# LinXueyuanStdio/LaTeX_OCR

Measured on AMD Instinct MI355X. Metric: formula-images/sec training step (batch 64, 128x512), higher is better.
Workload: dtype bf16; 1 GPU; configs[2]: full encoder+attention+decoder training step, batch 64/GPU, 128x512, vocab 500, T=101 (lengths U{30..100}), Adam; global_batch=64, parallelism=dp1

## Files before the change

### include/lxo.h

```cpp
#ifndef LXO_H
#define LXO_H
#include <stddef.h>
#include <stdint.h>
#ifdef __cplusplus
extern "C" {
#endif
#pragma GCC visibility push(default)

#define LXO_F32 0
#define LXO_BF16 1

const char* lxo_last_error(void);
#define LXO_ABI_VERSION 6
int lxo_version(void);
int lxo_shape_size(void);


int lxo_gemm_nt(int dt, int a_f32, int c_f32, int small, const void* A, const void* Bp, void* C,
                int M, int N, int K, int lda, int ldb, int ldc, const float* bias, int act,
                float alpha, int accumulate, void* stream);

int lxo_gemm_tn(int dt, int a_f32, int b_f32, const void* A, const void* B, float* C,
                int M, int I, int J, int lda, int ldb, int ldc, int nsplit, int atomic, void* stream);

// ... 72 lines not shown
                        const int32_t* lengths, float inv_ntok, void* stream);
int lxo_ce_loss_fwd_bwd_dev(const lxo_shape* s, void* ws, const int32_t* formula,
                            const int32_t* lengths, const float* ntok_dev, void* stream);
int lxo_ce_loss_weighted(const lxo_shape* s, void* ws, const int32_t* formula, const int32_t* lengths,
                         const float* w_tok, const float* w_row, float inv_norm, const float* norm_dev, void* stream);
int lxo_ce_loss_smoothed(const lxo_shape* s, void* ws, const int32_t* formula, const int32_t* lengths, float eps,
                         const float* w_tok, const float* w_row, float inv_norm, const float* norm_dev, void* stream);
int lxo_mrt_weights(const float* seq_logp, const float* cost, const int32_t* group_off, int G, int rows, float alpha,
                    float* w_out, float* q_out, float* risk_out, void* stream);
#define LXO_EDIT_MAX_REF 1024
int lxo_edit_distance(const int32_t* hyp, int hyp_block, long long hyp_block_stride, long long hyp_row_stride, long long hyp_tok_stride, int T,
                      const int32_t* hyp_len, const int32_t* ref, int G, int ref_ld, const int32_t* ref_len, const int32_t* ref_of, int per_ref,
                      int pairs, int id_end, int32_t* dist_out, float* cost_out, void* stream);
#define LXO_TEXT_STATS  12
#define LXO_TEXT_CORPUS 14
int lxo_text_stats(const int32_t* hyp, int hyp_block, long long hyp_block_stride, long long hyp_row_stride, long long hyp_tok_stride, int T,
                   const int32_t* hyp_len, const int32_t* ref, int G, int ref_ld, const int32_t* ref_len, const int32_t* ref_of, int per_ref,
                   int pairs, int id_end, int32_t* stats_out, long long* corpus_io, int accumulate, void* stream);
int lxo_mrt_candidates(const int32_t* ids, int B, int max_steps, int n, int steps, const int32_t* ref, int Tr, const int32_t* ref_len,
                       int id_end, int id_pad, int include_reference, int32_t* cand, int32_t* cand_len, float* cost, int32_t* group_off,
                       int32_t* row_image, void* stream);
#define LXO_CONSENSUS_MAX_N 64
int lxo_consensus(const int32_t* ids, long long image_stride, long long draw_stride, long long tok_stride, int B, int n, int T, int id_end,
                  const float* weights, int normalize, int32_t* dist_out, float* risk_out, int32_t* best_out, void* stream);
#define LXO_BLEU_COUNTS 10
int lxo_sentence_bleu(const int32_t* hyp, int hyp_block, long long hyp_block_stride, long long hyp_row_stride, long long hyp_tok_stride, int T,
                      const int32_t* hyp_len, const int32_t* ref, int G, int ref_ld, const int32_t* ref_len, const int32_t* ref_of, int per_ref,
                      int pairs, int id_end, int32_t* counts_out, float* bleu_out, float* cost_out, void* stream);
int lxo_consensus_bleu(const int32_t* ids, long long image_stride, long long draw_stride, long long tok_stride, int B, int n, int T, int id_end,
                       const float* weights, int32_t* match_out, float* cost_out, float* risk_out, int32_t* best_out, void* stream);
#define LXO_COST_EDIT 0
#define LXO_COST_BLEU 1
int lxo_mrt_candidates_cost(const int32_t* ids, int B, int max_steps, int n, int steps, const int32_t* ref, int Tr, const int32_t* ref_len,
                            int id_end, int id_pad, int include_reference, int32_t* cand, int32_t* cand_len, float* cost, int32_t* group_off,
                            int32_t* row_image, int cost_kind, void* stream);
int lxo_score_tokens(const lxo_shape* s, void* ws, const int32_t* formula, const int32_t* lengths,
                     float* logp_out, int32_t* top1_out, float* seq_out, void* stream);
int lxo_score_alternatives(const lxo_shape* s, void* ws, const int32_t* formula, const int32_t* lengths, int k,
                           const uint32_t* allow, int allow_ld, int32_t* ids_out, float* logp_out,
                           int32_t* rank_out, float* entropy_out, void* stream);
int lxo_decoder_train_bwd(const lxo_shape* s, const float* params, const void* wpack, void* ws,
                          const int32_t* formula, float* grads, void* stream);
int lxo_decoder_train_bwd_part(const lxo_shape* s, const float* params, const void* wpack, void* ws,
                               const int32_t* formula, float* grads, int parts, void* stream);

#define LXO_XDEC_BLOCK_BYTES (4096 + (384 << 10))
#define LXO_XDEC_ERR_WORD 512
int lxo_chain_guard(const lxo_shape* s, void* ws, const float* grads, float* scale_io, int have_scale, uint32_t* status_out, void* stream);

#define LXO_GNORM_FLOATS (2 + 1024)
int lxo_global_norm_scale(long long n, const float* grads, float clip, float* scale_out, void* stream);
int lxo_adam_step(long long n, float* params, const float* grads, float* m, float* v,
                  float lr_t, float beta1, float beta2, float eps, const float* scale_dev, void* stream);

int lxo_optimizer_step(int method, long long n, float* params, const float* grads, float* slot, float lr,
                       const float* scale_dev, void* stream);

int lxo_greedy_decode(const lxo_shape* s, const float* params, const void* wpack, void* ws,
                      int id_end, int max_iter, int32_t* ids_out, int* steps_out, void* stream);
int lxo_greedy_decode_attn(const lxo_shape* s, const float* params, const void* wpack, void* ws,
                           int id_end, int max_iter, int32_t* ids_out, float* alpha_out, int* steps_out, void* stream);
int lxo_greedy_decode_scores(const lxo_shape* s, const float* params, const void* wpack, void* ws, int id_end, int max_iter,
                             int32_t* ids_out, float* logp_out, float* alpha_out, int* steps_out, void* stream);
int lxo_greedy_decode_prefix(const lxo_shape* s, const float* params, const void* wpack, void* ws, int id_end, int max_iter,
                             const int32_t* prefix, int prefix_ld, const int32_t* prefix_len,
                             int32_t* ids_out, float* logp_out, float* alpha_out, int* steps_out, void* stream);
int lxo_greedy_decode_constrained(const lxo_shape* s, const float* params, const void* wpack, void* ws, int id_end, int max_iter,
                                  const uint32_t* allow, int allow_ld,
                                  const int32_t* prefix, int prefix_ld, const int32_t* prefix_len,
                                  int32_t* ids_out, float* logp_out, float* alpha_out, int* steps_out, void* stream);
typedef struct lxo_sample_opts { float temperature; int top_k; float top_p; unsigned seed; } lxo_sample_opts;
int lxo_sample_decode(const lxo_shape* s, const float* params, const void* wpack, void* ws, int id_end, int max_iter,
                      const lxo_sample_opts* opts, const uint32_t* allow, int allow_ld,
                      const int32_t* prefix, int prefix_ld, const int32_t* prefix_len,
                      int32_t* ids_out, float* logp_out, float* logq_out, float* alpha_out, int* steps_out, void* stream);
int lxo_sample_tokens(const float* logits, int ld, int rows, int n, int V, int time, const lxo_sample_opts* opts,
                      const uint32_t* allow, int allow_ld, int32_t* ids_out, float* logp_out, float* logq_out, void* stream);
int lxo_decode_begin(const lxo_shape* s, const float* params, const void* wpack, void* ws, void* stream);
int lxo_decode_step(const lxo_shape* s, const float* params, const void* wpack, void* ws, int id_end, int time,
                    int32_t* ids_out, int32_t* parents_out, int32_t* finished_host, int* unfinished_host, void* stream);
int lxo_decode_state_get(const lxo_shape* s, void* ws, int time, float* c, float* h, float* o, void* stream);
int lxo_decode_state_set(const lxo_shape* s, void* ws, int time, const float* c, const float* h, const float* o,
                         const int32_t* ids_prev, void* stream);
int lxo_decode_cell_step(const lxo_shape* s, const float* params, const void* wpack, void* ws, int time, int start_token, void* stream);
int lxo_beam_decode(const lxo_shape* s, const float* params, const void* wpack, void* ws,
                    int id_end, int max_iter, int32_t* ids_out, int32_t* parents_out,
                    int* steps_out, void* stream);
int lxo_beam_decode_attn(const lxo_shape* s, const float* params, const void* wpack, void* ws,
                         int id_end, int max_iter, int32_t* ids_out, int32_t* parents_out, float* alpha_out,
                         int* steps_out, void* stream);
int lxo_beam_decode_scores(const lxo_shape* s, const float* params, const void* wpack, void* ws, int id_end, int max_iter,
                           int32_t* ids_out, int32_t* parents_out, float* scores_out, float* alpha_out, int* steps_out, void* stream);
int lxo_beam_decode_prefix(const lxo_shape* s, const float* params, const void* wpack, void* ws, int id_end, int max_iter,
                           const int32_t* prefix, int prefix_ld, const int32_t* prefix_len,
                           int32_t* ids_out, int32_t* parents_out, float* scores_out, float* alpha_out, int* steps_out, void* stream);
int lxo_beam_decode_constrained(const lxo_shape* s, const float* params, const void* wpack, void* ws, int id_end, int max_iter,
                                const uint32_t* allow, int allow_ld,
                                const int32_t* prefix, int prefix_ld, const int32_t* prefix_len,
                                int32_t* ids_out, int32_t* parents_out, float* scores_out, float* alpha_out, int* steps_out, void* stream);

#define LXO_GRAMMAR_MAX_DEPTH 32
typedef struct lxo_grammar { const int8_t* cls; int n_kinds; int max_depth; int budget; } lxo_grammar;
size_t lxo_grammar_scratch_bytes(int rows, int V);
int lxo_greedy_decode_grammar(const lxo_shape* s, const float* params, const void* wpack, void* ws, int id_end, int max_iter,
                              const uint32_t* allow, int allow_ld, const int32_t* prefix, int prefix_ld, const int32_t* prefix_len,
                              const lxo_grammar* grammar, int32_t* ids_out, float* logp_out, float* alpha_out, int32_t* depth_out,
// ... 28 lines not shown
```

### latex_ocr_amd/_abi.py

```python
import ctypes
import os

c_int, c_ll, c_size, c_float, c_void = ctypes.c_int, ctypes.c_longlong, ctypes.c_size_t, ctypes.c_float, ctypes.c_void_p
P = ctypes.POINTER

LXO_F32, LXO_BF16 = 0, 1
LXO_GNORM_FLOATS = 2 + 1024
LIB_PATH = os.environ.get("LXO_LIB_PATH") or os.path.join(os.path.dirname(os.path.abspath(__file__)), "liblxo.so")


ABI_VERSION = 6
LXO_COMM_ID_BYTES = 128
LXO_I32, LXO_U8 = 2, 3
LXO_XDEC_BLOCK_BYTES, LXO_XDEC_ERR_WORD = 4096 + (384 << 10), 512
LXO_EDIT_MAX_REF = 1024
LXO_CONSENSUS_MAX_N = 64
LXO_TEXT_STATS, LXO_TEXT_CORPUS = 12, 14
LXO_BLEU_COUNTS = 10
LXO_COST_EDIT, LXO_COST_BLEU = 0, 1


class LxoShape(ctypes.Structure):
    _fields_ = [(n, c_int) for n in ("B", "H", "W", "T", "V", "C", "E", "U", "O", "D", "dtype", "beam", "max_steps")] + \
               [("keep_prob", c_float), ("dropout_seed", c_int), ("div_gamma", c_float), ("div_prob", c_float), ("div_seed", c_int),
# ... 11 lines not shown
LXO_GRAMMAR_MAX_DEPTH = 32


def bind(lib):
    S = P(LxoShape)
    sig = {
        "lxo_last_error": (ctypes.c_char_p, []),
        "lxo_version": (c_int, []),
        "lxo_shape_size": (c_int, []),
        "lxo_ws_region_dtype": (c_int, [S, ctypes.c_char_p]),
        "lxo_gemm_nt": (c_int, [c_int] * 4 + [c_void] * 3 + [c_int] * 6 + [c_void, c_int, c_float, c_int, c_void]),
        "lxo_gemm_tn": (c_int, [c_int] * 3 + [c_void] * 3 + [c_int] * 8 + [c_void]),
        "lxo_conv3x3": (c_int, [c_int, c_void, c_void, c_void, c_void] + [c_int] * 9 + [c_void]),
        "lxo_conv3x3_ex": (c_int, [c_int, c_void, c_void, c_void, c_void] + [c_int] * 9 + [c_void, c_int, c_void, c_void, c_void, c_void]),
        "lxo_conv3x3_wgrad": (c_int, [c_int, c_void, c_void, c_void] + [c_int] * 8 + [c_void]),
        "lxo_gemm_slab": (c_int, [c_int, c_void, c_void, c_void] + [c_int] * 6 + [c_ll, c_void]),
        "lxo_attention_fwd": (c_int, [c_int] + [c_void] * 7 + [c_int] * 6 + [c_void]),
        "lxo_timing_enable": (c_int, [c_int]),
        "lxo_timing_count": (c_int, []),
        "lxo_timing_get": (c_int, [c_int, P(ctypes.c_char_p), P(ctypes.c_char_p), P(ctypes.c_double), P(c_float)]),
        "lxo_param_num": (c_int, []),
        "lxo_param_name": (ctypes.c_char_p, [c_int]),
        "lxo_param_name_for": (ctypes.c_char_p, [S, c_int]),
        "lxo_param_total": (c_ll, [S]),
        "lxo_param_info": (c_int, [S, c_int, P(c_ll), P(c_ll)]),
        "lxo_wpack_bytes": (c_size, [S]),
        "lxo_workspace_bytes": (c_size, [S]),
        "lxo_ws_region": (c_int, [S, ctypes.c_char_p, P(c_size), P(c_size)]),
        "lxo_pack_weights": (c_int, [S, c_void, c_void, c_void]),
        "lxo_encoder_fwd": (c_int, [S, c_void, c_void, c_void, c_void, c_void]),
        "lxo_encoder_bwd": (c_int, [S, c_void, c_void, c_void, c_void, c_void, c_int, c_int, c_void]),
        "lxo_encoder_bwd_ready": (c_int, [S, c_void, c_void, c_void, c_void, c_void, c_int, c_int, c_void, c_void]),
        "lxo_train_bwd": (c_int, [S, c_void, c_void, c_void, c_void, c_void, c_void, c_void, c_void]),
        "lxo_set_encoder_side_stream": (c_int, [c_void]),
        "lxo_set_side_stream": (c_int, [c_void]),
        "lxo_decoder_train_fwd": (c_int, [S, c_void, c_void, c_void, c_void, c_void]),
        "lxo_decoder_train_fwd_live": (c_int, [S, c_void, c_void, c_void, c_void, c_void, c_void]),
        "lxo_ce_loss_fwd_bwd": (c_int, [S, c_void, c_void, c_void, c_float, c_void]),
        "lxo_ce_loss_fwd_bwd_dev": (c_int, [S, c_void, c_void, c_void, c_void, c_void]),
        "lxo_ce_loss_weighted": (c_int, [S, c_void, c_void, c_void, c_void, c_void, c_float, c_void, c_void]),
        "lxo_ce_loss_smoothed": (c_int, [S, c_void, c_void, c_void, c_float, c_void, c_void, c_float, c_void, c_void]),
        "lxo_mrt_weights": (c_int, [c_void, c_void, c_void, c_int, c_int, c_float, c_void, c_void, c_void, c_void]),
        "lxo_edit_distance": (c_int, [c_void, c_int, c_ll, c_ll, c_ll, c_int, c_void, c_void, c_int, c_int, c_void, c_void, c_int, c_int, c_int, c_void, c_void, c_void]),
        "lxo_text_stats": (c_int, [c_void, c_int, c_ll, c_ll, c_ll, c_int, c_void, c_void, c_int, c_int, c_void, c_void, c_int, c_int, c_int, c_void, c_void, c_int, c_void]),
        "lxo_mrt_candidates": (c_int, [c_void, c_int, c_int, c_int, c_int, c_void, c_int, c_void, c_int, c_int, c_int, c_void, c_void, c_void, c_void, c_void, c_void]),
        "lxo_sentence_bleu": (c_int, [c_void, c_int, c_ll, c_ll, c_ll, c_int, c_void, c_void, c_int, c_int, c_void, c_void, c_int, c_int, c_int, c_void, c_void, c_void, c_void]),
        "lxo_mrt_candidates_cost": (c_int, [c_void, c_int, c_int, c_int, c_int, c_void, c_int, c_void, c_int, c_int, c_int, c_void, c_void, c_void, c_void, c_void, c_int, c_void]),
        "lxo_consensus_bleu": (c_int, [c_void, c_ll, c_ll, c_ll, c_int, c_int, c_int, c_int, c_void, c_void, c_void, c_void, c_void, c_void]),
        "lxo_consensus": (c_int, [c_void, c_ll, c_ll, c_ll, c_int, c_int, c_int, c_int, c_void, c_int, c_void, c_void, c_void, c_void]),
        "lxo_decoder_train_bwd_part": (c_int, [S, c_void, c_void, c_void, c_void, c_void, c_int, c_void]),
        "lxo_decoder_train_bwd": (c_int, [S, c_void, c_void, c_void, c_void, c_void, c_void]),
        "lxo_global_norm_scale": (c_int, [c_ll, c_void, c_float, c_void, c_void]),
        "lxo_adam_step": (c_int, [c_ll, c_void, c_void, c_void, c_void, c_float, c_float, c_float, c_float, c_void, c_void]),
        "lxo_optimizer_step": (c_int, [c_int, c_ll, c_void, c_void, c_void, c_float, c_void, c_void]),
        "lxo_greedy_decode": (c_int, [S, c_void, c_void, c_void, c_int, c_int, c_void, P(c_int), c_void]),
        "lxo_greedy_decode_attn": (c_int, [S, c_void, c_void, c_void, c_int, c_int, c_void, c_void, P(c_int), c_void]),
        "lxo_decode_begin": (c_int, [S, c_void, c_void, c_void, c_void]),
        "lxo_decode_step": (c_int, [S, c_void, c_void, c_void, c_int, c_int, c_void, c_void, c_void, P(c_int), c_void]),
        "lxo_beam_decode": (c_int, [S, c_void, c_void, c_void, c_int, c_int, c_void, c_void, P(c_int), c_void]),
        "lxo_beam_decode_attn": (c_int, [S, c_void, c_void, c_void, c_int, c_int, c_void, c_void, c_void, P(c_int), c_void]),
        "lxo_greedy_decode_scores": (c_int, [S, c_void, c_void, c_void, c_int, c_int, c_void, c_void, c_void, P(c_int), c_void]),
        "lxo_beam_decode_scores": (c_int, [S, c_void, c_void, c_void, c_int, c_int, c_void, c_void, c_void, c_void, P(c_int), c_void]),
        "lxo_score_tokens": (c_int, [S, c_void, c_void, c_void, c_void, c_void, c_void, c_void]),
        "lxo_score_alternatives": (c_int, [S, c_void, c_void, c_void, c_int, c_void, c_int, c_void, c_void, c_void, c_void, c_void]),
        "lxo_greedy_decode_prefix": (c_int, [S, c_void, c_void, c_void, c_int, c_int, c_void, c_int, c_void, c_void, c_void, c_void, P(c_int), c_void]),
        "lxo_beam_decode_prefix": (c_int, [S, c_void, c_void, c_void, c_int, c_int, c_void, c_int, c_void, c_void, c_void, c_void, c_void, P(c_int), c_void]),
        "lxo_greedy_decode_constrained": (c_int, [S, c_void, c_void, c_void, c_int, c_int, c_void, c_int, c_void, c_int, c_void, c_void, c_void, c_void, P(c_int), c_void]),
        "lxo_beam_decode_constrained": (c_int, [S, c_void, c_void, c_void, c_int, c_int, c_void, c_int, c_void, c_int, c_void, c_void, c_void, c_void, c_void, P(c_int), c_void]),
        "lxo_sample_decode": (c_int, [S, c_void, c_void, c_void, c_int, c_int, P(LxoSampleOpts), c_void, c_int, c_void, c_int, c_void, c_void, c_void, c_void, c_void, P(c_int), c_void]),
        "lxo_sample_tokens": (c_int, [c_void, c_int, c_int, c_int, c_int, c_int, P(LxoSampleOpts), c_void, c_int, c_void, c_void, c_void, c_void]),
        "lxo_grammar_scratch_bytes": (c_size, [c_int, c_int]),
        "lxo_greedy_decode_grammar": (c_int, [S, c_void, c_void, c_void, c_int, c_int, c_void, c_int, c_void, c_int, c_void, P(LxoGrammar), c_void, c_void, c_void, c_void, c_void, P(c_int), c_void]),
        "lxo_beam_decode_grammar": (c_int, [S, c_void, c_void, c_void, c_int, c_int, c_void, c_int, c_void, c_int, c_void, P(LxoGrammar), c_void, c_void, c_void, c_void, c_void, c_void, P(c_int), c_void]),
        "lxo_sample_decode_grammar": (c_int, [S, c_void, c_void, c_void, c_int, c_int, P(LxoSampleOpts), c_void, c_int, c_void, c_int, c_void, P(LxoGrammar), c_void, c_void, c_void, c_void, c_void, c_void, P(c_int), c_void]),
        "lxo_grammar_step": (c_int, [P(LxoGrammar), c_int, c_int, c_int, c_int, c_void, c_void, c_void, c_int, c_int, c_void, c_int, c_void, c_void, c_void, c_void]),
        "lxo_chain_guard": (c_int, [S, c_void, c_void, c_void, c_int, c_void, c_void]),
        "lxo_decode_state_get": (c_int, [S, c_void, c_int, c_void, c_void, c_void, c_void]),
        "lxo_decode_state_set": (c_int, [S, c_void, c_int, c_void, c_void, c_void, c_void, c_void]),
        "lxo_decode_cell_step": (c_int, [S, c_void, c_void, c_void, c_int, c_int, c_void]),
        "lxo_comm_unique_id": (c_int, [c_void]),
        "lxo_comm_init": (c_int, [c_void, c_int, c_int, P(c_void)]),
        "lxo_comm_info": (c_int, [c_void, P(c_int), P(c_int)]),
        "lxo_allreduce_bucket": (c_int, [c_void, c_void, c_ll, c_int, c_void, c_void]),
        "lxo_comm_destroy": (c_int, [c_void]),
        "lxo_comm_last_error": (ctypes.c_char_p, []),
    }
    missing = []
    for name, (res, args) in sig.items():
        try:
            fn = getattr(lib, name)
        except AttributeError:
            missing.append(name)
            continue
        fn.restype, fn.argtypes = res, args
    lib._lxo_missing = missing
    if not missing:
        if lib.lxo_version() != ABI_VERSION or lib.lxo_shape_size() != ctypes.sizeof(LxoShape):
            raise RuntimeError("liblxo ABI mismatch: library version %d / lxo_shape %d bytes, binding version %d / %d bytes"
                               % (lib.lxo_version(), lib.lxo_shape_size(), ABI_VERSION, ctypes.sizeof(LxoShape)))
    return lib


ENTRY_POINTS = ["lxo_last_error", "lxo_version", "lxo_shape_size", "lxo_ws_region_dtype", "lxo_timing_enable", "lxo_timing_count", "lxo_timing_get", "lxo_gemm_nt", "lxo_gemm_tn", "lxo_conv3x3", "lxo_conv3x3_ex", "lxo_conv3x3_wgrad", "lxo_gemm_slab", "lxo_attention_fwd", "lxo_param_num", "lxo_param_name", "lxo_param_name_for",
                "lxo_param_total", "lxo_param_info", "lxo_wpack_bytes", "lxo_workspace_bytes", "lxo_ws_region",
                "lxo_pack_weights", "lxo_encoder_fwd", "lxo_encoder_bwd", "lxo_encoder_bwd_ready", "lxo_train_bwd", "lxo_set_side_stream", "lxo_set_encoder_side_stream", "lxo_decoder_train_fwd", "lxo_decoder_train_fwd_live",
                "lxo_ce_loss_fwd_bwd", "lxo_ce_loss_fwd_bwd_dev", "lxo_ce_loss_weighted", "lxo_ce_loss_smoothed", "lxo_mrt_weights", "lxo_edit_distance", "lxo_text_stats", "lxo_mrt_candidates", "lxo_consensus", "lxo_sentence_bleu", "lxo_consensus_bleu", "lxo_mrt_candidates_cost", "lxo_decoder_train_bwd", "lxo_decoder_train_bwd_part", "lxo_global_norm_scale", "lxo_adam_step", "lxo_optimizer_step",
                "lxo_greedy_decode", "lxo_greedy_decode_attn", "lxo_beam_decode", "lxo_beam_decode_attn", "lxo_greedy_decode_scores", "lxo_beam_decode_scores", "lxo_score_tokens", "lxo_score_alternatives", "lxo_greedy_decode_prefix", "lxo_beam_decode_prefix", "lxo_greedy_decode_constrained", "lxo_beam_decode_constrained", "lxo_sample_decode", "lxo_sample_tokens",
                "lxo_grammar_scratch_bytes", "lxo_greedy_decode_grammar", "lxo_beam_decode_grammar", "lxo_sample_decode_grammar", "lxo_grammar_step", "lxo_decode_begin", "lxo_decode_step",
                "lxo_chain_guard", "lxo_decode_state_get", "lxo_decode_state_set", "lxo_decode_cell_step",
                "lxo_comm_unique_id", "lxo_comm_init", "lxo_comm_info", "lxo_allreduce_bucket", "lxo_comm_destroy", "lxo_comm_last_error"]

_lib = None


def load():
    global _lib
    if _lib is None:
        if not os.path.exists(LIB_PATH):
            raise RuntimeError(
                "latex_ocr_amd: %s is missing. Build it with `python -c 'import __graft_entry__ as g; g.build()'` "
                "(hipcc --offload-arch=gfx950). There is no CPU fallback." % LIB_PATH)
        try:
            import torch
        except ImportError:
            pass
        _lib = bind(ctypes.CDLL(LIB_PATH))
        if _lib._lxo_missing:
            raise RuntimeError("liblxo.so lacks entry points: %s" % _lib._lxo_missing)
    return _lib


def check(lib, rc, what=""):
    if rc != 0:
        raise RuntimeError("%s failed: rc=%d %s" % (what, rc, lib.lxo_last_error().decode()))
```

### latex_ocr_amd/csrc/api.hip

```cpp
#include "lxo.h"
#include "gemm.h"
#include "impl.h"
#include <stdio.h>
#include <string.h>

static thread_local char g_err[256] = "";
static int fail(int code, const char* what) {
    snprintf(g_err, sizeof(g_err), "%s (code %d)", what, code);
    return code < 0 ? code : -code;
}
#define CHECK_LAUNCH(expr, what) do { int rc_ = (expr); if (rc_ != 0) return fail(rc_, what); } while (0)

extern "C" const char* lxo_last_error(void) { return g_err; }
extern "C" int lxo_version(void) { return LXO_ABI_VERSION; }
extern "C" int lxo_shape_size(void) { return (int)sizeof(lxo_shape); }

extern "C" int lxo_gemm_nt(int dt, int a_f32, int c_f32, int small, const void* A, const void* Bp, void* C,
                           int M, int N, int K, int lda, int ldb, int ldc, const float* bias, int act,
                           float alpha, int accumulate, void* stream) {
    GemmNT p; memset(&p, 0, sizeof(p));
    p.A = A; p.Bp = Bp; p.C = C; p.M = M; p.N = N; p.K = K; p.lda = lda; p.ldb = ldb; p.ldc = ldc;
    p.bias = bias; p.act = act; p.alpha = alpha; p.accumulate = accumulate; p.addend_rows = 1;
    CHECK_LAUNCH(lxo_launch_gemm_nt(dt, a_f32, c_f32, small, p, (hipStream_t)stream), "lxo_gemm_nt");
    return 0;
// ... 223 lines not shown
extern "C" int lxo_score_tokens(const lxo_shape* s, void* ws, const int32_t* formula, const int32_t* lengths,
                                float* logp_out, int32_t* top1_out, float* seq_out, void* stream) {
    MAKE_PLAN(P, s);
    if (s->T <= 0) return fail(-1, "T must be positive");
    if (!ws || !formula || !lengths) return fail(-1, "lxo_score_tokens: null workspace, formula or lengths");
    if (!logp_out) return fail(-1, "lxo_score_tokens: null logp_out");
    CHECK_LAUNCH(lxo_impl_score_tokens(P, ws, formula, lengths, logp_out, top1_out, seq_out, (hipStream_t)stream), "lxo_score_tokens");
    return 0;
}
extern "C" int lxo_score_alternatives(const lxo_shape* s, void* ws, const int32_t* formula, const int32_t* lengths, int k,
                                      const uint32_t* allow, int allow_ld, int32_t* ids_out, float* logp_out,
                                      int32_t* rank_out, float* entropy_out, void* stream) {
    MAKE_PLAN(P, s);
    if (s->T <= 0) return fail(-1, "T must be positive");
    if (!ws || !formula || !lengths) return fail(-1, "lxo_score_alternatives: null workspace, formula or lengths");
    if (!ids_out) return fail(-1, "lxo_score_alternatives: null ids_out");
    if (!logp_out) return fail(-1, "lxo_score_alternatives: null logp_out");
    if (k < 1 || k > 16 || k > P.s.V) return fail(-1, "lxo_score_alternatives: k outside 1 .. min(16, V)");
    if (allow && (allow_ld < 0 || (allow_ld != 0 && allow_ld < (P.s.V + 31) / 32))) return fail(-1, "lxo_score_alternatives: allow_ld must be 0 or >= (V + 31) / 32");
    if (!allow && allow_ld != 0) return fail(-1, "lxo_score_alternatives: null allow with allow_ld != 0");
    const DecAllow al = {allow, allow_ld};
    CHECK_LAUNCH(lxo_impl_score_alternatives(P, ws, formula, lengths, k, allow ? &al : nullptr, ids_out, logp_out, rank_out, entropy_out, (hipStream_t)stream),
                 "lxo_score_alternatives");
    return 0;
}
extern "C" int lxo_decoder_train_bwd(const lxo_shape* s, const float* params, const void* wpack, void* ws,
                                     const int32_t* formula, float* grads, void* stream) {
    MAKE_PLAN(P, s);
    CHECK_LAUNCH(lxo_impl_decoder_train_bwd(P, params, wpack, ws, formula, grads, 3, (hipStream_t)stream), "lxo_decoder_train_bwd");
    return 0;
}
extern "C" int lxo_train_bwd(const lxo_shape* s, const float* params, const void* wpack, void* ws, const int32_t* formula, const uint8_t* img,
                            float* grads, void* const* ready_events, void* stream) {
    MAKE_PLAN(P, s);
    CHECK_LAUNCH(lxo_impl_decoder_train_bwd(P, params, wpack, ws, formula, grads, 3, (hipStream_t)stream, true, ready_events ? ready_events[0] : nullptr),
                 "lxo_train_bwd (decoder)");
    CHECK_LAUNCH(lxo_impl_encoder_bwd(P, params, wpack, ws, img, grads, 6, 1, (hipStream_t)stream, ready_events), "lxo_train_bwd (encoder)");
    return 0;
}
extern "C" int lxo_decoder_train_bwd_part(const lxo_shape* s, const float* params, const void* wpack, void* ws,
                                          const int32_t* formula, float* grads, int parts, void* stream) {
    MAKE_PLAN(P, s);
    if (parts < 1 || parts > 3) return fail(-1, "lxo_decoder_train_bwd_part: parts must be 1, 2 or 3");
    CHECK_LAUNCH(lxo_impl_decoder_train_bwd(P, params, wpack, ws, formula, grads, parts, (hipStream_t)stream), "lxo_decoder_train_bwd_part");
    return 0;
}
extern "C" int lxo_global_norm_scale(long long n, const float* grads, float clip, float* scale_out, void* stream) {
    CHECK_LAUNCH(lxo_k_global_norm_scale(n, grads, clip, scale_out + 2, scale_out, (hipStream_t)stream), "lxo_global_norm_scale");
    return 0;
}
extern "C" int lxo_adam_step(long long n, float* params, const float* grads, float* m, float* v,
                             float lr_t, float beta1, float beta2, float eps, const float* scale_dev, void* stream) {
    CHECK_LAUNCH(lxo_k_adam(params, grads, m, v, n, lr_t, beta1, beta2, eps, scale_dev, (hipStream_t)stream), "lxo_adam_step");
    return 0;
}
extern "C" int lxo_greedy_decode(const lxo_shape* s, const float* params, const void* wpack, void* ws,
                                 int id_end, int max_iter, int32_t* ids_out, int* steps_out, void* stream) {
    MAKE_PLAN(P, s);
    const DecodeOuts o = {ids_out, nullptr, nullptr, nullptr, nullptr};
    CHECK_LAUNCH(lxo_impl_greedy_decode(P, params, wpack, ws, id_end, max_iter, o, steps_out, (hipStream_t)stream), "lxo_greedy_decode");
    return 0;
}
extern "C" int lxo_greedy_decode_attn(const lxo_shape* s, const float* params, const void* wpack, void* ws,
                                      int id_end, int max_iter, int32_t* ids_out, float* alpha_out, int* steps_out, void* stream) {
    MAKE_PLAN(P, s);
    const DecodeOuts o = {ids_out, nullptr, nullptr, alpha_out, nullptr};
    CHECK_LAUNCH(lxo_impl_greedy_decode(P, params, wpack, ws, id_end, max_iter, o, steps_out, (hipStream_t)stream), "lxo_greedy_decode_attn");
    return 0;
}
extern "C" int lxo_greedy_decode_scores(const lxo_shape* s, const float* params, const void* wpack, void* ws, int id_end, int max_iter,
                                        int32_t* ids_out, float* logp_out, float* alpha_out, int* steps_out, void* stream) {
    MAKE_PLAN(P, s);
    if (!logp_out) return fail(-1, "lxo_greedy_decode_scores: null logp_out");
    const DecodeOuts o = {ids_out, nullptr, logp_out, alpha_out, nullptr};
    CHECK_LAUNCH(lxo_impl_greedy_decode(P, params, wpack, ws, id_end, max_iter, o, steps_out, (hipStream_t)stream), "lxo_greedy_decode_scores");
    return 0;
}
static bool make_prefix(DecPrefix* pf, const int32_t* prefix, int prefix_ld, const int32_t* prefix_len, int max_iter) {
    *pf = DecPrefix{prefix, prefix_len, prefix_ld, prefix_ld < max_iter ? prefix_ld : max_iter};
    return prefix && prefix_len && prefix_ld >= 1;
}
extern "C" int lxo_greedy_decode_prefix(const lxo_shape* s, const float* params, const void* wpack, void* ws, int id_end, int max_iter,
                                        const int32_t* prefix, int prefix_ld, const int32_t* prefix_len,
                                        int32_t* ids_out, float* logp_out, float* alpha_out, int* steps_out, void* stream) {
    MAKE_PLAN(P, s);
    DecPrefix pf;
    if (!make_prefix(&pf, prefix, prefix_ld, prefix_len, max_iter)) return fail(-1, "lxo_greedy_decode_prefix: null prefix / prefix_len or prefix_ld < 1");
    const DecodeOuts o = {ids_out, nullptr, logp_out, alpha_out, &pf};
    CHECK_LAUNCH(lxo_impl_greedy_decode(P, params, wpack, ws, id_end, max_iter, o, steps_out, (hipStream_t)stream), "lxo_greedy_decode_prefix");
    return 0;
}
static const char* make_constraint(DecAllow* al, DecPrefix* pf, bool* has_prefix, int V, const uint32_t* allow, int allow_ld,
                                   const int32_t* prefix, int prefix_ld, const int32_t* prefix_len, int max_iter) {
    *al = DecAllow{allow, allow_ld};
    if (!allow || allow_ld < 0 || (allow_ld != 0 && allow_ld < (V + 31) / 32)) return "lxo_*_decode_constrained: null allow or 0 < allow_ld < (V + 31) / 32";
    *has_prefix = prefix || prefix_len || prefix_ld != 0;
    if (*has_prefix && !make_prefix(pf, prefix, prefix_ld, prefix_len, max_iter)) return "lxo_*_decode_constrained: a prefix needs prefix, prefix_len and prefix_ld >= 1 (none: all NULL / 0)";
    return nullptr;
}
extern "C" int lxo_greedy_decode_constrained(const lxo_shape* s, const float* params, const void* wpack, void* ws, int id_end, int max_iter,
                                             const uint32_t* allow, int allow_ld, const int32_t* prefix, int prefix_ld, const int32_t* prefix_len,
                                             int32_t* ids_out, float* logp_out, float* alpha_out, int* steps_out, void* stream) {
    MAKE_PLAN(P, s);
    DecAllow al; DecPrefix pf; bool has_prefix = false;
    if (const char* why = make_constraint(&al, &pf, &has_prefix, P.s.V, allow, allow_ld, prefix, prefix_ld, prefix_len, max_iter))
        return fail(-1, why);
// ... 275 lines not shown
```

### latex_ocr_amd/csrc/decoder_kernels.h

```cpp
#pragma once
#include "lxo_common.h"
struct Slabs { const float* p; int n; long long stride; int ld; };
struct Drop { unsigned thr; float inv_keep; unsigned seed; int t, row0, rows_total; };
struct DetScratch { float* p; size_t floats; };
int lxo_k_det_reduce(const float* part, int nslot, long long stride, int N, float* out, hipStream_t st);
int lxo_k_rowmean(int dt, const void* img, float* mean, int B, int R, int C, hipStream_t st);
int lxo_k_embed_gather(int dt, const float* table, const float* start, const int* formula, void* out, int B, int T, int D, int Dp, int V, hipStream_t st);
int lxo_k_embed_rows(int dt, const float* table, const float* start, const int* ids, void* out, int n, int D, int Dp, int V, hipStream_t st);
int lxo_k_embed_table(int dt, const float* table, const float* start, void* out, int V, int D, int Dp, hipStream_t st);
int lxo_k_lstm_fwd(const float* z, Slabs zs, const float* c_prev, float* gates, float* c_out, float* h_out, float* ht_out, int ldh, Drop dr, int B, int U, hipStream_t st);
int lxo_k_lstm_bwd(const float* gates, const float* c_prev, const float* c_cur, Slabs s1, Slabs s3, Slabs s4, int off4,
                   float* dcc, float* dz, Drop dr, int carry_rows, int B, int U, hipStream_t st);
int lxo_k_tanh_bwd(const float* a, int lda, Slabs carry, const float* o, int ldo, float* g, int ldg, void* gb, int ldgb, Drop dr, int carry_rows, int rows, int cols, hipStream_t st);
int lxo_k_slab_reduce(Slabs sl, float* o, int ldo, int rows, int cols, hipStream_t st);
int lxo_k_tanh_finalize(Slabs sl, float* o, int ldo, Drop dr, int rows, int cols, hipStream_t st);
int lxo_k_attn_fwd(int dt, const void* att_img, const void* img, const float* att_h, Slabs ahs, float* att_h_out, const float* beta, float* alpha, float* part,
                   float* ctx, int ldctx, void* ctxb, int ldcb, int nv, int R, int Rp, int E, int C, int beam, int nch, int rev, hipStream_t st, const void* att_exp = nullptr);
int lxo_k_att_exp(const void* att_img, void* att_exp, long long n, hipStream_t st);
int lxo_k_attn_bwd(int dt, const void* att_img, const void* att_exp, const void* img, const float* att_h, const float* beta, const float* alpha,
                   Slabs dcs, int dcoff, float* dctx_out, int lddc, const float* ctx, int ldctx, float* de, float* datth,
                   int nv, int R, int Rp, int E, int C, int nch, int rev, hipStream_t st);
int lxo_k_datt_img(int dt, const void* att_img, const float* att_h, const float* beta, const float* de, void* dout, float* dbeta,
                   int T, int B, int R, int Rp, int E, float* atth_exp, DetScratch det, hipStream_t st);
int lxo_k_add_mean_grad(float* dimg, const float* dmean, int B, int R, int C, hipStream_t st);
int lxo_k_colsum_det(const void* a, int bf16, long long lda, float* out, long long M, int N, DetScratch det, hipStream_t st);
int lxo_k_colsum(const float* a, long long lda, float* out, long long M, int N, DetScratch det, hipStream_t st);
int lxo_k_embed_scatter(const float* demb, const int* formula, float* dtable, float* dstart, int B, int T, int D, int V, int det, hipStream_t st);
int lxo_k_init_bwd(const float* dcc, Slabs dxh, const float* c0, const float* rec0, int ldr, float* dpre, int B, int U, int O, hipStream_t st);
int lxo_k_beam_gather(float* rec, int ldr, int XH, float* cs, int U, const int* parents, int k, float* tmp_rec, float* tmp_cs, int n, void* recb, int ldrb, hipStream_t st);
int lxo_k_tile_rows(const float* src, int lds, float* dst, int ldd, int n, int k, int cols, hipStream_t st);
int lxo_k_global_norm_scale(long long n, const float* g, float clip, float* sumsq_tmp, float* out, hipStream_t st);
int lxo_k_chain_guard(const unsigned* err_fwd, const unsigned* err_bwd, const float* probe, float* scale, int have_scale, unsigned* status, hipStream_t st);
int lxo_k_chain_poison(const unsigned* err_fwd, const unsigned* err_bwd, float* probe, hipStream_t st);
int lxo_k_adam(float* p, const float* g, float* m, float* v, long long n, float lr_t, float b1, float b2, float eps, const float* scale, hipStream_t st);
int lxo_k_simple_opt(float* p, const float* g, float* slot, long long n, float lr, int mode, const float* scale, hipStream_t st);
```

### latex_ocr_amd/csrc/decoder_kernels.hip

```cpp
#include "decoder_kernels.h"
#include "api_util.h"
#include "drop.h"

namespace {


LXO_DEV void load4(const float* p, float (&v)[4]) {
    f32x4 a = *reinterpret_cast<const f32x4*>(p);
    v[0] = a[0]; v[1] = a[1]; v[2] = a[2]; v[3] = a[3];
}
LXO_DEV void load4(const bf16_t* p, float (&v)[4]) {
    u32x2 a = *reinterpret_cast<const u32x2*>(p);
    v[0] = __uint_as_float(a[0] << 16); v[1] = __uint_as_float(a[0] & 0xffff0000u);
    v[2] = __uint_as_float(a[1] << 16); v[3] = __uint_as_float(a[1] & 0xffff0000u);
}
LXO_DEV void store4(float* p, const float (&v)[4]) { f32x4 a = {v[0], v[1], v[2], v[3]}; *reinterpret_cast<f32x4*>(p) = a; }
LXO_DEV void store4(bf16_t* p, const float (&v)[4]) { u32x2 a = {pack_bf2(v[0], v[1]), pack_bf2(v[2], v[3])}; *reinterpret_cast<u32x2*>(p) = a; }

LXO_DEV float slab_sum(const Slabs& sl, long long row, int col) {
    float v = 0.f;
    const float* q = sl.p + row * sl.ld + col;
    for (int s = 0; s < sl.n; ++s) v += q[(long long)s * sl.stride];
    return v;
}

LXO_DEV f32x4 slab_sum4(const Slabs& sl, long long row, int col) {
    f32x4 v = {0.f, 0.f, 0.f, 0.f};
    const float* q = sl.p + row * sl.ld + col;
    for (int s0 = 0; s0 < sl.n; s0 += 8) {
        f32x4 t[8];
#pragma unroll
        for (int j = 0; j < 8; ++j) {
            const f32x4 z = {0.f, 0.f, 0.f, 0.f};
            t[j] = (s0 + j < sl.n) ? *reinterpret_cast<const f32x4*>(q + (long long)(s0 + j) * sl.stride) : z;
        }
#pragma unroll
        for (int j = 0; j < 8; ++j) v += t[j];
    }
    return v;
}

template <typename CT>
__global__ __launch_bounds__(256) void rowmean_kernel(const CT* __restrict__ img, float* __restrict__ mean, int R, int C) {
    __shared__ float red[32][64 + 1];
    const int b = blockIdx.y, c0 = blockIdx.x * 64 + (threadIdx.x & 7) * 8, rg = threadIdx.x >> 3;
    float acc[8];
#pragma unroll
    for (int e = 0; e < 8; ++e) acc[e] = 0.f;
    for (int r = rg; r < R; r += 32) {
        float v[8];
        load8(img + ((long long)b * R + r) * C + c0, v);
#pragma unroll
        for (int e = 0; e < 8; ++e) acc[e] += v[e];
    }
#pragma unroll
// ... 104 lines not shown
    for (int s0 = q; s0 < sl.n; s0 += 32) {
        f32x4 t[8];
#pragma unroll
        for (int j = 0; j < 8; ++j) {
            const f32x4 z = {0.f, 0.f, 0.f, 0.f};
            t[j] = (s0 + 4 * j < sl.n) ? *reinterpret_cast<const f32x4*>(p + (long long)(s0 + 4 * j) * sl.stride) : z;
        }
#pragma unroll
        for (int j = 0; j < 8; ++j) v += t[j];
    }
    return v;
}

__global__ __launch_bounds__(256) void lstm_bwd_kernel(const float* __restrict__ gates, const float* __restrict__ c_prev,
                                                      const float* __restrict__ c_cur, Slabs s1, Slabs s3, Slabs s4, int off4,
                                                      float* __restrict__ dcc, float* __restrict__ dz, Drop dr, int carry_rows,
                                                      int B, int U) {
    __shared__ float ex[64][4][8 + 1];
    const int total = B * (U >> 2);
    const int q = threadIdx.x & 3, ugl = threadIdx.x >> 2;
    for (int base = blockIdx.x * 64; base < total; base += gridDim.x * 64) {
        const int ug = base + ugl;
        const bool ok = ug < total;
        const int b = ok ? ug / (U >> 2) : 0, u = ok ? (ug - b * (U >> 2)) << 2 : 0;
        float gi = 0.f, gj = 0.f, gf = 0.f, go = 0.f, cc = 0.f, cp = 0.f, dci = 0.f;
        if (ok) {
            const float* gr = gates + (long long)b * 4 * U + u + q;
            gi = gr[0]; gj = gr[U]; gf = gr[2 * U]; go = gr[3 * U];
            cc = c_cur[(long long)b * U + u + q]; cp = c_prev[(long long)b * U + u + q]; dci = dcc[(long long)b * U + u + q];
            const f32x4 pm = slab_part4(s1, b, u, q) + slab_part4(s3, b, u, q);
            f32x4 pc = {0.f, 0.f, 0.f, 0.f};
            if (b < carry_rows) pc = slab_part4(s4, b, off4 + u, q);
#pragma unroll
            for (int e = 0; e < 4; ++e) { ex[ugl][q][e] = pm[e]; ex[ugl][q][4 + e] = pc[e]; }
        }
        __syncthreads();
        if (ok) {
            const float dhm = ex[ugl][0][q] + ex[ugl][1][q] + ex[ugl][2][q] + ex[ugl][3][q];
            const float dhc = ex[ugl][0][4 + q] + ex[ugl][1][4 + q] + ex[ugl][2][4 + q] + ex[ugl][3][4 + q];
            const float dh = dhm * drop_scale(dr, 1u, b, u + q, U) + dhc;
            const float tc = tanhf(cc);
            const float dc = dci + dh * go * (1.f - tc * tc);
            float* dzr = dz + (long long)b * 4 * U + u + q;
            dzr[0] = dc * gj * gi * (1.f - gi);
            dzr[U] = dc * gi * (1.f - gj * gj);
            dzr[2 * U] = dc * cp * gf * (1.f - gf);
            dzr[3 * U] = dh * tc * go * (1.f - go);
            dcc[(long long)b * U + u + q] = dc * gf;
        }
        __syncthreads();
    }
}

__global__ __launch_bounds__(256) void tanh_bwd_kernel(const float* __restrict__ a, int lda, Slabs carry,
                                                      const float* __restrict__ o, int ldo, float* __restrict__ g, int ldg,
                                                      bf16_t* __restrict__ gb, int ldgb, Drop dr, int carry_rows, int rows, int cols) {
    const int total = rows * (cols >> 2);
    for (int i = blockIdx.x * 256 + threadIdx.x; i < total; i += gridDim.x * 256) {
        const int r = i / (cols >> 2), c = (i - r * (cols >> 2)) << 2;
        const f32x4 ov = *reinterpret_cast<const f32x4*>(o + (long long)r * ldo + c);
        f32x4 d = *reinterpret_cast<const f32x4*>(a + (long long)r * lda + c);
        if (r < carry_rows) d += slab_sum4(carry, r, c);
        f32x4 out;
#pragma unroll
        for (int e = 0; e < 4; ++e) {
            const float sc = drop_scale(dr, 2u, r, c + e, cols);
            const float th = (dr.thr == 0u) ? ov[e] : ov[e] / dr.inv_keep;
            out[e] = d[e] * sc * (1.f - th * th);
        }
        *reinterpret_cast<f32x4*>(g + (long long)r * ldg + c) = out;
        if (gb) { u32x2 pk = {pack_bf2(out[0], out[1]), pack_bf2(out[2], out[3])}; *reinterpret_cast<u32x2*>(gb + (long long)r * ldgb + c) = pk; }
    }
}
__global__ __launch_bounds__(256) void tanh_finalize_kernel(Slabs sl, float* __restrict__ o, int ldo, Drop dr, int rows, int cols) {
    const int total = rows * (cols >> 2);
    for (int i = blockIdx.x * 256 + threadIdx.x; i < total; i += gridDim.x * 256) {
        const int r = i / (cols >> 2), c = (i - r * (cols >> 2)) << 2;
        const f32x4 v = slab_sum4(sl, r, c);
        f32x4 out;
#pragma unroll
        for (int e = 0; e < 4; ++e) out[e] = tanhf(v[e]) * drop_scale(dr, 2u, r, c + e, cols);
        *reinterpret_cast<f32x4*>(o + (long long)r * ldo + c) = out;
    }
}

constexpr int ATT_W = 8;

template <typename CT> LXO_DEV float tanh_ct(float x);
template <> LXO_DEV float tanh_ct<float>(float x) { return tanhf(x); }
template <> LXO_DEV float tanh_ct<bf16_t>(float x) { return 1.f - 2.f * __builtin_amdgcn_rcpf(__expf(2.f * x) + 1.f); }

template <typename CT, int KCT, int ATT_U>
__global__ __launch_bounds__(512) void attn_fwd_part_kernel(const CT* __restrict__ att_img, const CT* __restrict__ img,
                                                           const float* __restrict__ att_h, Slabs ahs, float* __restrict__ att_h_out,
                                                           const float* __restrict__ beta,
                                                           float* __restrict__ alpha, float* __restrict__ part,
                                                           int R, int Rp, int E, int C, int beam, int nch, int rows_per, int rev) {
    __shared__ float redc[ATT_W][512];
    __shared__ float red[2 * ATT_W];
    const int ch = blockIdx.x, v = blockIdx.y, bi = v / beam;
    const int tid = threadIdx.x, lane = tid & 63, wave = tid >> 6;
    const int r0 = ch * rows_per;
    const int n = min(R, r0 + rows_per) - r0;
    const CT* ai = att_img + ((long long)bi * R + r0) * E;
    const CT* im = img + ((long long)bi * R + r0) * C;
    float* pout = part + ((long long)v * nch + ch) * (C + 2);
    constexpr int KC = KCT;
    float ah[KCT][4], bt[KCT][4];
#pragma unroll
    for (int kc = 0; kc < KCT; ++kc) {
        const int k0 = kc * 256 + lane * 4;
#pragma unroll
        for (int j = 0; j < 4; ++j) { ah[kc][j] = 0.f; bt[kc][j] = 0.f; }
        if (kc < KC && k0 < E) {
            const f32x4 a4 = ahs.n > 0 ? slab_sum4(ahs, v, k0) : *reinterpret_cast<const f32x4*>(att_h + (long long)v * E + k0);
            const f32x4 b4 = *reinterpret_cast<const f32x4*>(beta + k0);
#pragma unroll
            for (int j = 0; j < 4; ++j) { ah[kc][j] = a4[j]; bt[kc][j] = b4[j]; }
            if (ahs.n > 0 && att_h_out && ch == 0 && wave == 0) *reinterpret_cast<f32x4*>(att_h_out + (long long)v * E + k0) = a4;
        }
    }
    const int c0 = lane * 8;
    const bool cok = c0 < C;
    float m = -3.0e38f, l = 0.f, acc[8];
// ... 909 lines not shown
            const int src = b * k + parents[b * k + r];
            v[r] = c < XH ? rec[(long long)src * ldr + c] : cs[(long long)src * U + (c - XH)];
        }
    }
#pragma unroll
    for (int r = 0; r < BP_KMAX; ++r) {
        if (r < k) {
            const int dst = b * k + r;
            if (c < XH) { rec[(long long)dst * ldr + c] = v[r]; if (recb) recb[(long long)dst * ldrb + c] = f2bf(v[r]); }
            else cs[(long long)dst * U + (c - XH)] = v[r];
        }
    }
}
__global__ __launch_bounds__(256) void tile_rows_kernel(const float* __restrict__ src, int lds, float* __restrict__ dst, int ldd, int n, int k, int cols) {
    const long long total = (long long)n * cols;
    for (long long i = (long long)blockIdx.x * 256 + threadIdx.x; i < total; i += (long long)gridDim.x * 256) {
        const int v = (int)(i / cols), c = (int)(i - (long long)v * cols);
        dst[(long long)v * ldd + c] = src[(long long)(v / k) * lds + c];
    }
}

__global__ __launch_bounds__(256) void sumsq_kernel(const float* __restrict__ g, long long n, float* __restrict__ out) {
    __shared__ float red[4];
    float s = 0.f;
    for (long long i = (long long)blockIdx.x * 256 + threadIdx.x; i < n; i += (long long)gridDim.x * 256) s = fmaf(g[i], g[i], s);
    s = wave_sum(s);
    if ((threadIdx.x & 63) == 0) red[threadIdx.x >> 6] = s;
    __syncthreads();
    if (threadIdx.x == 0) out[blockIdx.x] = red[0] + red[1] + red[2] + red[3];
}
__global__ void clip_scale_kernel(const float* __restrict__ sumsq, int nparts, float clip, float* __restrict__ out) {
    float ss = 0.f;
    for (int i = 0; i < nparts; ++i) ss += sumsq[i];
    const float gn = sqrtf(ss);
    out[1] = gn;
    out[0] = clip > 0.f ? clip / fmaxf(gn, clip) : 1.0f;
}
__global__ void chain_guard_kernel(const unsigned* __restrict__ err_fwd, const unsigned* __restrict__ err_bwd, const float* __restrict__ probe,
                                   float* __restrict__ scale, int have_scale, unsigned* __restrict__ status) {
    const unsigned ef = err_fwd ? err_fwd[0] : 0u, eb = err_bwd ? err_bwd[0] : 0u;
    const float pv = probe ? probe[0] : 0.f;
    const bool drop = (ef | eb) != 0u || pv != pv;
    if (status) { status[0] = ef; status[1] = eb; status[2] = drop ? 1u : 0u; }
    scale[0] = drop ? __uint_as_float(0x7fc00000u) : (have_scale ? scale[0] : 1.0f);
}
__global__ void chain_poison_kernel(const unsigned* __restrict__ err_fwd, const unsigned* __restrict__ err_bwd, float* __restrict__ probe) {
    if ((err_fwd && err_fwd[0]) || (err_bwd && err_bwd[0])) probe[0] = __uint_as_float(0x7fc00000u);
}
__global__ __launch_bounds__(256) void adam_kernel(float* __restrict__ p, const float* __restrict__ g, float* __restrict__ m, float* __restrict__ v,
                                                  long long n, float lr_t, float b1, float b2, float eps, const float* __restrict__ scale) {
    const float sc = scale ? scale[0] : 1.0f;
    if (sc != sc) return;
    for (long long i = (long long)blockIdx.x * 256 + threadIdx.x; i < n; i += (long long)gridDim.x * 256) {
        const float gi = g[i] * sc;
        const float mi = b1 * m[i] + (1.f - b1) * gi;
        const float vi = b2 * v[i] + (1.f - b2) * gi * gi;
        m[i] = mi; v[i] = vi;
        p[i] -= lr_t * mi / (sqrtf(vi) + eps);
    }
}

__global__ __launch_bounds__(256) void simple_opt_kernel(float* __restrict__ p, const float* __restrict__ g, float* __restrict__ slot,
                                                        long long n, float lr, int mode, const float* __restrict__ scale) {
    const float sc = scale ? scale[0] : 1.0f;
    if (sc != sc) return;
    for (long long i = (long long)blockIdx.x * 256 + threadIdx.x; i < n; i += (long long)gridDim.x * 256) {
        const float gi = g[i] * sc;
        if (mode == 1) p[i] -= lr * gi;
        else if (mode == 2) { const float a = slot[i] + gi * gi; slot[i] = a; p[i] -= lr * gi / sqrtf(a); }
        else { const float ms = 0.9f * slot[i] + 0.1f * gi * gi; slot[i] = ms; p[i] -= lr * gi / sqrtf(ms + 1e-10f); }
    }
}

inline int grid1(long long items, int per_block = 256, int cap = 2048) {
    long long g = (items + per_block - 1) / per_block;
    return (int)(g < 1 ? 1 : (g > cap ? cap : g));
}
}

#define LAUNCH(kern, grid, ...) hipLaunchKernelGGL(kern, dim3(grid), dim3(256), 0, st, __VA_ARGS__)
#define BYCT(dt, kern, grid, ...) do { if ((dt) == LXO_BF16) LAUNCH((kern<bf16_t>), grid, __VA_ARGS__); else LAUNCH((kern<float>), grid, __VA_ARGS__); } while (0)
#define DONE return (int)hipGetLastError()

int lxo_k_rowmean(int dt, const void* img, float* mean, int B, int R, int C, hipStream_t st) {
    if (C % 64) return -2;
    if (dt == LXO_BF16) LAUNCH((rowmean_kernel<bf16_t>), dim3(C / 64, B), (const bf16_t*)img, mean, R, C);
    else LAUNCH((rowmean_kernel<float>), dim3(C / 64, B), (const float*)img, mean, R, C);
    DONE;
}
int lxo_k_embed_gather(int dt, const float* table, const float* start, const int* formula, void* out, int B, int T, int D, int Dp, int V, hipStream_t st) {
    const int g = grid1((long long)T * B * Dp);
    if (dt == LXO_BF16) LAUNCH((embed_gather_kernel<bf16_t>), g, table, start, formula, (bf16_t*)out, B, T, D, Dp, V);
    else LAUNCH((embed_gather_kernel<float>), g, table, start, formula, (float*)out, B, T, D, Dp, V);
    DONE;
}
int lxo_k_embed_rows(int dt, const float* table, const float* start, const int* ids, void* out, int n, int D, int Dp, int V, hipStream_t st) {
    const int g = grid1((long long)n * Dp);
    if (dt == LXO_BF16) LAUNCH((embed_rows_kernel<bf16_t>), g, table, start, ids, (bf16_t*)out, n, D, Dp, V);
    else LAUNCH((embed_rows_kernel<float>), g, table, start, ids, (float*)out, n, D, Dp, V);
    DONE;
}
int lxo_k_embed_table(int dt, const float* table, const float* start, void* out, int V, int D, int Dp, hipStream_t st) {
    const int g = grid1((long long)(V + 1) * Dp);
    if (dt == LXO_BF16) LAUNCH((embed_table_kernel<bf16_t>), g, table, start, (bf16_t*)out, V, D, Dp);
    else LAUNCH((embed_table_kernel<float>), g, table, start, (float*)out, V, D, Dp);
    DONE;
}
int lxo_k_lstm_fwd(const float* z, Slabs zs, const float* c_prev, float* gates, float* c_out, float* h_out, float* ht_out, int ldh, Drop dr, int B, int U, hipStream_t st) {
    LAUNCH(lstm_fwd_kernel, grid1((long long)B * U), z, zs, c_prev, gates, c_out, h_out, ht_out, ldh, dr, B, U);
    DONE;
}
int lxo_k_lstm_bwd(const float* gates, const float* c_prev, const float* c_cur, Slabs s1, Slabs s3, Slabs s4, int off4,
                   float* dcc, float* dz, Drop dr, int carry_rows, int B, int U, hipStream_t st) {
    LAUNCH(lstm_bwd_kernel, grid1((long long)B * U), gates, c_prev, c_cur, s1, s3, s4, off4, dcc, dz, dr, carry_rows, B, U);
    DONE;
}
int lxo_k_tanh_bwd(const float* a, int lda, Slabs carry, const float* o, int ldo, float* g, int ldg, void* gb, int ldgb, Drop dr, int carry_rows, int rows, int cols, hipStream_t st) {
    LAUNCH(tanh_bwd_kernel, grid1((long long)rows * cols / 4), a, lda, carry, o, ldo, g, ldg, (bf16_t*)gb, ldgb, dr, carry_rows, rows, cols);
    DONE;
}
__global__ __launch_bounds__(256) static void slab_reduce_kernel(Slabs sl, float* __restrict__ o, int ldo, int rows, int cols) {
    const int total = rows * (cols >> 2);
    for (int i = blockIdx.x * 256 + threadIdx.x; i < total; i += gridDim.x * 256) {
        const int r = i / (cols >> 2), c = (i - r * (cols >> 2)) << 2;
        *reinterpret_cast<f32x4*>(o + (long long)r * ldo + c) = slab_sum4(sl, r, c);
    }
}
int lxo_k_slab_reduce(Slabs sl, float* o, int ldo, int rows, int cols, hipStream_t st) {
    LAUNCH(slab_reduce_kernel, grid1((long long)rows * cols / 4), sl, o, ldo, rows, cols);
    DONE;
}
int lxo_k_tanh_finalize(Slabs sl, float* o, int ldo, Drop dr, int rows, int cols, hipStream_t st) {
    LAUNCH(tanh_finalize_kernel, grid1((long long)rows * cols / 4), sl, o, ldo, dr, rows, cols);
    DONE;
}
static int att_u(int rows_per) {
    return (rows_per + 55) / 56 <= (rows_per + 63) / 64 ? 7 : 8;
}
#define ATT_BY_U(K_, CT_, KCT_) do { if (att_u(rows_per) == 8) K_(CT_, KCT_, 8); else K_(CT_, KCT_, 7); } while (0)
#define ATT_BY_CT_E(K_) do { if (dt == LXO_BF16) { if (E <= 256) ATT_BY_U(K_, bf16_t, 1); else ATT_BY_U(K_, bf16_t, 4); } \
                             else { if (E <= 256) ATT_BY_U(K_, float, 1); else ATT_BY_U(K_, float, 4); } } while (0)
int lxo_k_attn_fwd(int dt, const void* att_img, const void* img, const float* att_h, Slabs ahs, float* att_h_out, const float* beta, float* alpha, float* part,
                   float* ctx, int ldctx, void* ctxb, int ldcb, int nv, int R, int Rp, int E, int C, int beam, int nch, int rev, hipStream_t st, const void* att_exp) {
    if (E > 1024 || C > 512 || nch < 1 || nch > 32) return -2;
    const int rows_per = cdiv(R, nch);
    dim3 grid(nch, nv);
    if ((beam == 2 || beam == 3 || beam == 5 || (beam == 1 && att_exp && dt == LXO_BF16)) && ahs.n == 0 && att_h && E <= 256 && C <= 512 && nv % beam == 0) {
        const int nimg = nv / beam;
        int nb = cdiv(512, nimg);
        if (nb > 16) nb = 16;
        const int by_rows = R / 32 > 0 ? R / 32 : 1;
        if (nb > by_rows) nb = by_rows;
        const int need = cdiv(R, 1024);
        if (nb < need) nb = need;
        const int rpb = cdiv(R, nb);
        const dim3 gb(nb, nimg);
#define ABM(CT_, U_, NB_, X_, OCC_, AI_) hipLaunchKernelGGL((attn_fwd_part_beam_kernel<CT_, U_, NB_, X_, OCC_>), gb, dim3(512), 0, st, (const CT_*)(AI_), (const CT_*)img, att_h, beta, alpha, part, R, Rp, E, C, nb, rpb, rev)
        if (dt == LXO_BF16 && att_exp) { if (beam == 1) ABM(bf16_t, 4, 1, true, 4, att_exp); else if (beam == 2) ABM(bf16_t, 4, 2, true, 4, att_exp); else if (beam == 3) ABM(bf16_t, 4, 3, true, 4, att_exp); else ABM(bf16_t, 2, 5, true, 4, att_exp); }
        else if (dt == LXO_BF16) { if (beam == 2) ABM(bf16_t, 4, 2, false, 2, att_img); else if (beam == 3) ABM(bf16_t, 4, 3, false, 2, att_img); else ABM(bf16_t, 4, 5, false, 2, att_img); }
        else { if (beam == 2) ABM(float, 4, 2, false, 2, att_img); else if (beam == 3) ABM(float, 4, 3, false, 2, att_img); else ABM(float, 4, 5, false, 2, att_img); }
#undef ABM
        hipLaunchKernelGGL(attn_fwd_combine_kernel, dim3(4, nv), dim3(256), 0, st, part, alpha, ctx, ldctx, (bf16_t*)ctxb, ldcb, R, Rp, C, nb, rpb);
        DONE;
    }
#define AF(CT_, KCT_, U_) hipLaunchKernelGGL((attn_fwd_part_kernel<CT_, KCT_, U_>), grid, dim3(512), 0, st, (const CT_*)att_img, (const CT_*)img, \
                                             att_h, ahs, att_h_out, beta, alpha, part, R, Rp, E, C, beam, nch, rows_per, rev)
    ATT_BY_CT_E(AF);
// ... 127 lines not shown
```

### latex_ocr_amd/csrc/encoder_kernels.h

```cpp
#pragma once
#include "lxo_common.h"
#include "decoder_kernels.h"
struct PackJob { int kind, K, N, lds, ldd, coff, Kpad, first_block, nblocks; long long src; long long dst; };
struct PackTable { int n; PackJob job[64]; };
int lxo_k_conv1_pool_fwd(int dt, const uint8_t* img, const float* w, const float* b, void* out, int B, int H, int W, hipStream_t s);
int lxo_k_conv1_pool_bwd(int dt, const uint8_t* img, const float* w, const float* b, const void* dout, float* dw, float* db, int B, int H, int W, DetScratch det, hipStream_t s);
int lxo_k_maxpool_fwd(int dt, const void* in, void* out, int B, int H, int W, int C, int ph, int pw, hipStream_t s);
int lxo_k_maxpool_mask_bwd(const unsigned char* mask, const void* dp, void* dy, float* db, int B, int H, int W, int C, int ph, int pw, DetScratch det, hipStream_t s);
int lxo_k_maxpool_relu_bwd(int dt, const void* y, const void* dp, void* dy, float* db, int B, int H, int W, int C, int ph, int pw, hipStream_t s);
int lxo_k_mask_convert(int dt, const float* d, const void* ref, void* out, float* db, long long rows, int C, hipStream_t s);
int lxo_k_timing_signal(float* pos, int Hp, int Wp, int C, hipStream_t s);
int lxo_k_pack_transpose(int dt, const float* src, void* dst, int K, int N, int lds, int ldd, int coff, int Kpad, hipStream_t s);
int lxo_k_pack_copy(int dt, const float* src, void* dst, int R, int Ccols, int lds, int ldd, int Cpad, hipStream_t s);
int lxo_k_pack_conv_dgrad(int dt, const float* w, void* dst, int Cin, int Cout, hipStream_t s);
int lxo_k_pack_batch(int dt, const PackTable& tab, int total_blocks, const float* prm, void* wpk, hipStream_t s);
int lxo_k_im2col_s2(int dt, const void* in, void* cols, int B, int H, int W, int Ho, int Wo, int C, hipStream_t s);
int lxo_k_col2im_s2_relu(int dt, const void* dcols, const void* yref, void* dy, float* db, int B, int H, int W, int Ho, int Wo, int C, hipStream_t s);
int lxo_k_colsum_ct(int dt, const void* a, float* out, long long M, int N, hipStream_t s);
```

### latex_ocr_amd/csrc/encoder_kernels.hip

```cpp
#include "encoder_kernels.h"
#include "switches.h"

namespace {

template <typename CT>
__global__ __launch_bounds__(256) void conv1_pool_fwd_kernel(const uint8_t* __restrict__ img, const float* __restrict__ w,
                                                            const float* __restrict__ bias, CT* __restrict__ out,
                                                            int B, int H, int W, int Hp, int Wp) {
    const int cg = threadIdx.x & 7;
    float wr[9][8], br[8];
#pragma unroll
    for (int t = 0; t < 9; ++t)
#pragma unroll
        for (int e = 0; e < 8; ++e) wr[t][e] = w[t * 64 + cg * 8 + e];
#pragma unroll
    for (int e = 0; e < 8; ++e) br[e] = bias[cg * 8 + e];
    __shared__ float sp[4][68];
    const int pl = threadIdx.x >> 3;
    const int segs_x = (Wp + 31) >> 5, nseg = B * Hp * segs_x;
    for (int seg = blockIdx.x; seg < nseg; seg += gridDim.x) {
        const int row = seg / segs_x, xc = seg - row * segs_x;
        const int b = row / Hp, py = row - b * Hp;
        const int px = xc * 32 + pl;
        const uint8_t* im = img + (long long)b * H * W;
        __syncthreads();
        for (int i = threadIdx.x; i < 4 * 66; i += 256) {
            const int dy = i / 66, dx = i - dy * 66;
            const int y = 2 * py - 1 + dy, x = 64 * xc - 1 + dx;
            sp[dy][dx] = (y >= 0 && y < H && x >= 0 && x < W) ? fmaf((float)im[y * W + x], 0.0078125f, -1.0f) : 0.f;
        }
        __syncthreads();
        if (px >= Wp) continue;
        const int pix = row * Wp + px;
        float patch[4][4];
#pragma unroll
        for (int dy = 0; dy < 4; ++dy) {
            const f32x2 lo = *reinterpret_cast<const f32x2*>(&sp[dy][2 * pl]), hi = *reinterpret_cast<const f32x2*>(&sp[dy][2 * pl + 2]);
            patch[dy][0] = lo[0]; patch[dy][1] = lo[1]; patch[dy][2] = hi[0]; patch[dy][3] = hi[1];
        }
        float best[8];
#pragma unroll
        for (int e = 0; e < 8; ++e) best[e] = -3.0e38f;
#pragma unroll
        for (int qy = 0; qy < 2; ++qy)
#pragma unroll
            for (int qx = 0; qx < 2; ++qx) {
                if (2 * py + qy >= H || 2 * px + qx >= W) continue;
#pragma unroll
                for (int e = 0; e < 8; e += 2) {
                    f32x2 a = {br[e], br[e + 1]};
#pragma unroll
                    for (int kh = 0; kh < 3; ++kh)
#pragma unroll
                        for (int kw = 0; kw < 3; ++kw) {
// ... 565 lines not shown
template <typename CT>
__global__ __launch_bounds__(256) void pack_conv_dgrad_kernel(const float* __restrict__ w, CT* __restrict__ dst, int Cin, int Cout) {
    const long long total = (long long)Cin * 9 * Cout;
    for (long long i = (long long)blockIdx.x * 256 + threadIdx.x; i < total; i += (long long)gridDim.x * 256) {
        const int co = (int)(i % Cout);
        const int tap = (int)((i / Cout) % 9);
        const int ci = (int)(i / ((long long)Cout * 9));
        const int a = tap / 3, b = tap - 3 * a;
        dst[i] = from_f32<CT>(w[((long long)((2 - a) * 3 + (2 - b)) * Cin + ci) * Cout + co]);
    }
}

template <typename CT>
__global__ __launch_bounds__(256) void pack_batch_kernel(PackTable tab, const float* __restrict__ prm, char* __restrict__ wpk) {
    __shared__ float tile[32][33];
    int j = 0;
    while (j + 1 < tab.n && (int)blockIdx.x >= tab.job[j + 1].first_block) ++j;
    const PackJob q = tab.job[j];
    const int lb = blockIdx.x - q.first_block;
    const float* src = prm + q.src;
    CT* dst = reinterpret_cast<CT*>(wpk + q.dst);
    if (q.kind == 0) {
        const int tiles_k = (q.Kpad + 31) / 32;
        const int k0 = (lb % tiles_k) * 32, n0 = (lb / tiles_k) * 32;
        const int tx = threadIdx.x & 31, ty = threadIdx.x >> 5;
        for (int r = ty; r < 32; r += 8) {
            const int k = k0 + r, n = n0 + tx;
            tile[r][tx] = (k < q.K && n < q.N) ? src[(long long)k * q.lds + n] : 0.f;
        }
        __syncthreads();
        for (int r = ty; r < 32; r += 8) {
            const int n = n0 + r, k = k0 + tx;
            if (n < q.N && k < q.Kpad) dst[(long long)n * q.ldd + q.coff + k] = from_f32<CT>(tile[tx][r]);
        }
    } else if (q.kind == 1) {
        const long long total = (long long)q.K * q.Kpad;
        for (long long i = (long long)lb * 256 + threadIdx.x; i < total; i += (long long)q.nblocks * 256) {
            const int c = (int)(i % q.Kpad); const long long r = i / q.Kpad;
            dst[r * q.ldd + c] = from_f32<CT>(c < q.N ? src[r * q.lds + c] : 0.f);
        }
    } else {
        const int Cin = q.K, Cout = q.N;
        const long long total = (long long)Cin * 9 * Cout;
        for (long long i = (long long)lb * 256 + threadIdx.x; i < total; i += (long long)q.nblocks * 256) {
            const int co = (int)(i % Cout);
            const int tap = (int)((i / Cout) % 9);
            const int ci = (int)(i / ((long long)Cout * 9));
            const int a = tap / 3, b = tap - 3 * a;
            dst[i] = from_f32<CT>(src[((long long)((2 - a) * 3 + (2 - b)) * Cin + ci) * Cout + co]);
        }
    }
}


template <typename CT>
__global__ __launch_bounds__(256) void im2col_s2_kernel(const CT* __restrict__ in, CT* __restrict__ cols, int B, int H, int W, int Ho, int Wo, int C) {
    const int c8n = C >> 3;
    const long long total = (long long)B * Ho * Wo * 8 * c8n;
    for (long long i = (long long)blockIdx.x * 256 + threadIdx.x; i < total; i += (long long)gridDim.x * 256) {
        const int c8 = (int)(i % c8n);
        const int tap = (int)((i / c8n) & 7);
        const long long m = i / (8 * c8n);
        const int ox = (int)(m % Wo), oy = (int)((m / Wo) % Ho), b = (int)(m / ((long long)Wo * Ho));
        const int iy = 2 * oy + (tap >> 2), ix = 2 * ox + (tap & 3) - 1;
        float v[8] = {0.f, 0.f, 0.f, 0.f, 0.f, 0.f, 0.f, 0.f};
        if (iy < H && ix >= 0 && ix < W) load8(in + (((long long)b * H + iy) * W + ix) * C + c8 * 8, v);
        store8(cols + (m * 8 + tap) * C + c8 * 8, v);
    }
}
template <typename CT>
__global__ __launch_bounds__(256) void col2im_s2_relu_kernel(const CT* __restrict__ dcols, const CT* __restrict__ yref, CT* __restrict__ dy,
                                                            float* __restrict__ db, int B, int H, int W, int Ho, int Wo, int C, int ppt) {
    const int c8n = C >> 3;
    const long long npix = (long long)B * H * W;
    const long long t = (long long)blockIdx.x * 256 + threadIdx.x;
    const int c8 = (int)(t % c8n);
    const long long p0 = (t / c8n) * ppt;
    if (p0 >= npix) return;
    float cs[8] = {0.f, 0.f, 0.f, 0.f, 0.f, 0.f, 0.f, 0.f};
    const long long p1 = p0 + ppt < npix ? p0 + ppt : npix;
    for (long long p = p0; p < p1; ++p) {
        const int x = (int)(p % W), y = (int)((p / W) % H), b = (int)(p / ((long long)W * H));
        const int oy = y >> 1, kh = y & 1;
        float acc[8] = {0.f, 0.f, 0.f, 0.f, 0.f, 0.f, 0.f, 0.f};
        if (oy < Ho) {
#pragma unroll
            for (int h = 0; h < 2; ++h) {
                const int kw = ((x + 1) & 1) + 2 * h;
                const int ox2 = x + 1 - kw;
                if (ox2 < 0 || (ox2 >> 1) >= Wo) continue;
                float v[8];
                load8(dcols + ((((long long)b * Ho + oy) * Wo + (ox2 >> 1)) * 8 + kh * 4 + kw) * C + c8 * 8, v);
#pragma unroll
                for (int e = 0; e < 8; ++e) acc[e] += v[e];
            }
        }
        float r[8];
        load8(yref + p * C + c8 * 8, r);
#pragma unroll
        for (int e = 0; e < 8; ++e) { acc[e] = r[e] > 0.f ? acc[e] : 0.f; cs[e] += acc[e]; }
        store8(dy + p * C + c8 * 8, acc);
    }
    if (!db) return;
#pragma unroll
    for (int e = 0; e < 8; ++e) atomicAdd(&db[c8 * 8 + e], cs[e]);
}
// ... 98 lines not shown
    else if (ph == 1 && pw == 2) hipLaunchKernelGGL((maxpool_mask_bwd_kernel<1, 2>), grid, dim3(256), 0, s, MB_ARGS);
    else return -2;
#undef MB_ARGS
    if (db_part) return lxo_k_det_reduce(db_part, (int)grid.x, C, C, db, s);
    return (int)hipGetLastError();
}
int lxo_k_maxpool_relu_bwd(int dt, const void* y, const void* dp, void* dy, float* db, int B, int H, int W, int C, int ph, int pw, hipStream_t s) {
    if (C % 8 || C > 512 || 256 % (C / 8)) return -2;
    DISPATCH_CT(dt, pool_bwd_t, y, dp, dy, db, B, H, W, C, ph, pw, s);
    return (int)hipGetLastError();
}
template <typename CT> static void mask_convert_t(const float* d, const void* ref, void* out, float* db, long long rows, int C, hipStream_t s) {
    const int rpb = 256 / (C / 8);
    hipLaunchKernelGGL((mask_convert_kernel<CT>), dim3(grid_for(rows, rpb * 8, 2048)), dim3(256), 0, s,
                       d, (const CT*)ref, (CT*)out, db, rows, C);
}
int lxo_k_mask_convert(int dt, const float* d, const void* ref, void* out, float* db, long long rows, int C, hipStream_t s) {
    if (C % 8 || C > 512 || 256 % (C / 8)) return -2;
    DISPATCH_CT(dt, mask_convert_t, d, ref, out, db, rows, C, s);
    return (int)hipGetLastError();
}
int lxo_k_timing_signal(float* pos, int Hp, int Wp, int C, hipStream_t s) {
    hipLaunchKernelGGL(timing_signal_kernel, dim3(grid_for((long long)Hp * Wp * C, 256, 1024)), dim3(256), 0, s, pos, Hp, Wp, C);
    return (int)hipGetLastError();
}
template <typename CT> static void pack_tr_t(const float* src, void* dst, int K, int N, int lds, int ldd, int coff, int Kpad, hipStream_t s) {
    hipLaunchKernelGGL((pack_transpose_kernel<CT>), dim3(cdiv(Kpad, 32), cdiv(N, 32)), dim3(256), 0, s, src, (CT*)dst, K, N, lds, ldd, coff, Kpad);
}
int lxo_k_pack_transpose(int dt, const float* src, void* dst, int K, int N, int lds, int ldd, int coff, int Kpad, hipStream_t s) {
    DISPATCH_CT(dt, pack_tr_t, src, dst, K, N, lds, ldd, coff, Kpad, s);
    return (int)hipGetLastError();
}
template <typename CT> static void pack_cp_t(const float* src, void* dst, int R, int Ccols, int lds, int ldd, int Cpad, hipStream_t s) {
    hipLaunchKernelGGL((pack_copy_kernel<CT>), dim3(grid_for((long long)R * Cpad, 256, 2048)), dim3(256), 0, s, src, (CT*)dst, R, Ccols, lds, ldd, Cpad);
}
int lxo_k_pack_copy(int dt, const float* src, void* dst, int R, int Ccols, int lds, int ldd, int Cpad, hipStream_t s) {
    DISPATCH_CT(dt, pack_cp_t, src, dst, R, Ccols, lds, ldd, Cpad, s);
    return (int)hipGetLastError();
}
template <typename CT> static void pack_dg_t(const float* w, void* dst, int Cin, int Cout, hipStream_t s) {
    hipLaunchKernelGGL((pack_conv_dgrad_kernel<CT>), dim3(grid_for((long long)Cin * 9 * Cout, 256, 2048)), dim3(256), 0, s, w, (CT*)dst, Cin, Cout);
}
int lxo_k_pack_conv_dgrad(int dt, const float* w, void* dst, int Cin, int Cout, hipStream_t s) {
    DISPATCH_CT(dt, pack_dg_t, w, dst, Cin, Cout, s);
    return (int)hipGetLastError();
}

int lxo_k_pack_batch(int dt, const PackTable& tab, int total_blocks, const float* prm, void* wpk, hipStream_t s) {
    if (tab.n <= 0) return 0;
    if (dt == LXO_BF16) hipLaunchKernelGGL((pack_batch_kernel<bf16_t>), dim3(total_blocks), dim3(256), 0, s, tab, prm, (char*)wpk);
    else hipLaunchKernelGGL((pack_batch_kernel<float>), dim3(total_blocks), dim3(256), 0, s, tab, prm, (char*)wpk);
    return (int)hipGetLastError();
}

template <typename CT> static void im2col_s2_t(const void* in, void* cols, int B, int H, int W, int Ho, int Wo, int C, hipStream_t s) {
    hipLaunchKernelGGL((im2col_s2_kernel<CT>), dim3(grid_for((long long)B * Ho * Wo * C, 256 * 4, 8192)), dim3(256), 0, s,
                       (const CT*)in, (CT*)cols, B, H, W, Ho, Wo, C);
}
int lxo_k_im2col_s2(int dt, const void* in, void* cols, int B, int H, int W, int Ho, int Wo, int C, hipStream_t s) {
    if (C % 8) return -2;
    DISPATCH_CT(dt, im2col_s2_t, in, cols, B, H, W, Ho, Wo, C, s);
    return (int)hipGetLastError();
}
template <typename CT> static void col2im_s2_t(const void* dcols, const void* yref, void* dy, float* db, int B, int H, int W, int Ho, int Wo, int C, hipStream_t s) {
    const int ppt = 32;
    const long long threads = (((long long)B * H * W + ppt - 1) / ppt) * (C / 8);
    hipLaunchKernelGGL((col2im_s2_relu_kernel<CT>), dim3((unsigned)((threads + 255) / 256)), dim3(256), 0, s,
                       (const CT*)dcols, (const CT*)yref, (CT*)dy, db, B, H, W, Ho, Wo, C, ppt);
}
int lxo_k_col2im_s2_relu(int dt, const void* dcols, const void* yref, void* dy, float* db, int B, int H, int W, int Ho, int Wo, int C, hipStream_t s) {
    if (C % 8) return -2;
    DISPATCH_CT(dt, col2im_s2_t, dcols, yref, dy, db, B, H, W, Ho, Wo, C, s);
    return (int)hipGetLastError();
}
template <typename CT> static void colsum_ct_t(const void* a, float* out, long long M, int N, hipStream_t s) {
    const int rpb = 256;
    hipLaunchKernelGGL((colsum_ct_kernel<CT>), dim3((unsigned)((M + rpb - 1) / rpb)), dim3(256), 0, s, (const CT*)a, out, M, N, rpb);
}
int lxo_k_colsum_ct(int dt, const void* a, float* out, long long M, int N, hipStream_t s) {
    if (N % 8 || N > 2048 || 256 % (N / 8)) return -2;
    DISPATCH_CT(dt, colsum_ct_t, a, out, M, N, s);
    return (int)hipGetLastError();
}
```

### latex_ocr_amd/csrc/impl.h

```cpp
#pragma once
#include "plan.h"
struct DecPrefix;
struct DecAllow;
struct DecSample;
const char* lxo_ws_name(int id);
int lxo_impl_pack_weights(const Plan& P, const float* prm, void* wp, hipStream_t st);
int lxo_impl_encoder_fwd(const Plan& P, const float* prm, const void* wp, void* ws, const uint8_t* img, hipStream_t st);
int lxo_impl_encoder_bwd(const Plan& P, const float* prm, const void* wp, void* ws, const uint8_t* img, float* grads,
                         int last_layer, int first_layer, hipStream_t st, void* const* ready = nullptr);
int lxo_impl_decoder_train_fwd(const Plan& P, const float* prm, const void* wp, void* ws, const int* formula, hipStream_t st, const int* lengths = nullptr);
int lxo_impl_ce_loss(const Plan& P, void* ws, const int* formula, const int* lengths, float inv_ntok, const float* ntok_dev, hipStream_t st,
                     const float* w_tok = nullptr, const float* w_row = nullptr, const float* smooth_eps = nullptr);
int lxo_impl_score_tokens(const Plan& P, void* ws, const int* formula, const int* lengths, float* logp_out, int* top1_out, float* seq_out, hipStream_t st);
int lxo_impl_score_alternatives(const Plan& P, void* ws, const int* formula, const int* lengths, int k, const DecAllow* allow, int* ids_out, float* logp_out,
                                int* rank_out, float* ent_out, hipStream_t st);
int lxo_impl_decoder_train_bwd(const Plan& P, const float* prm, const void* wp, void* ws, const int* formula, float* grads, int parts, hipStream_t st,
                               bool defer_join = false, void* ready = nullptr);
struct DecGrammar { const signed char* cls; int n_kinds, max_depth, budget; unsigned* scratch; int* depth; };
struct DecodeOuts { int* ids; int* parents; float* scores; float* alpha; const DecPrefix* prefix; const DecAllow* allow; const DecGrammar* grammar; };
int lxo_impl_greedy_decode(const Plan& P, const float* prm, const void* wp, void* ws, int id_end, int max_iter, const DecodeOuts& out, int* steps_out, hipStream_t st);
int lxo_impl_decode_begin(const Plan& P, const float* prm, const void* wp, void* ws, hipStream_t st);
int lxo_impl_decode_step(const Plan& P, const float* prm, const void* wp, void* ws, int id_end, int time, int* ids_out, int* parents_out, int* finished_out, int* unfinished_host, hipStream_t st);
int lxo_impl_chain_guard(const Plan& P, void* ws, const float* grads, float* scale, int have_scale, unsigned* status, hipStream_t st);
int lxo_impl_decode_state_get(const Plan& P, void* ws, int time, float* c, float* h, float* o, hipStream_t st);
int lxo_impl_decode_state_set(const Plan& P, void* ws, int time, const float* c, const float* h, const float* o, const int* ids_prev, hipStream_t st);
int lxo_impl_decode_cell_step(const Plan& P, const float* prm, const void* wp, void* ws, int time, int start_token, hipStream_t st);
int lxo_impl_beam_decode(const Plan& P, const float* prm, const void* wp, void* ws, int id_end, int max_iter, const DecodeOuts& out, int* steps_out, hipStream_t st);
int lxo_impl_sample_decode(const Plan& P, const float* prm, const void* wp, void* ws, int id_end, int max_iter, const DecSample& opts, const DecodeOuts& out,
                           float* logq_out, int* steps_out, hipStream_t st);
int lxo_impl_set_side_stream(hipStream_t s);
int lxo_impl_set_encoder_side_stream(hipStream_t s);
int lxo_impl_rowenc_fwd(const Plan& P, const float* prm, const void* wp, void* ws, hipStream_t st);
int lxo_impl_rowenc_bwd(const Plan& P, const float* prm, const void* wp, void* ws, float* grads, hipStream_t st);
```

### latex_ocr_amd/csrc/model_decoder.hip

```cpp
#include "plan.h"
#include "impl.h"
#include "gemm.h"
#include "head_kernels.h"
#include "grammar.h"
#include "rstep.h"
#include "xdec.h"
#include "dimg.h"
#include "api_util.h"
#include "switches.h"
#include "timing.h"

namespace {
int nt(const Plan& P, bool a_f32, bool c_f32, bool small, const void* A, int lda, const void* Bp, int ldb, void* C, int ldc,
       int M, int N, int K, const float* bias, int act, bool accumulate, hipStream_t st) {
    GemmNT g; memset(&g, 0, sizeof(g));
    g.A = A; g.Bp = Bp; g.C = C; g.M = M; g.N = N; g.K = K; g.lda = lda; g.ldb = ldb; g.ldc = ldc;
    g.bias = bias; g.act = act; g.alpha = 1.f; g.accumulate = accumulate ? 1 : 0; g.addend_rows = 1;
    if (P.s.dtype == LXO_F32) { a_f32 = true; c_f32 = true; }
    return lxo_launch_gemm_nt(P.s.dtype, a_f32, c_f32, small, g, st);
}
int tn(const Plan& P, bool a_f32, bool b_f32, const void* A, int lda, const void* B, int ldb, float* C, int ldc,
       int M, int I, int J, hipStream_t st, DetScratch det = DetScratch{nullptr, 0}) {
    GemmTN g; memset(&g, 0, sizeof(g));
    g.A = A; g.B = B; g.C = C; g.M = M; g.I = I; g.J = J; g.lda = lda; g.ldb = ldb; g.ldc = ldc;
// ... 36 lines not shown
    }
    return 0;
}
static int fork_side(hipStream_t st) { HIPRC(hipEventRecord(g_ev_fork, st)); HIPRC(hipStreamWaitEvent(g_side, g_ev_fork, 0)); return 0; }
static int join_side(hipStream_t st) { HIPRC(hipEventRecord(g_ev_join, g_side)); HIPRC(hipStreamWaitEvent(st, g_ev_join, 0)); return 0; }

static bool rstep_k_ok(int K, bool bf) {
    if (K % 128) return false;
    const int kq = K / 4;
    auto pow2_16 = [](int n) { return n >= 1 && n <= 16 && (n & (n - 1)) == 0; };
    if (bf && kq % 64 == 0 && pow2_16(kq / 64)) return true;
    return kq % 32 == 0 && pow2_16(kq / 32);
}
struct StepPath {
    enum Kernels { SplitK, Fused };
    Kernels shape, loop;
    bool dual, mirrors, try_chain;
};
static StepPath step_path(const Plan& P, bool training) {
    StepPath p;
    p.shape = P.s.step_kernels == 1 ? StepPath::SplitK : StepPath::Fused;
    const int ks[7] = {P.XH, P.s.U, P.HC, P.s.O, P.s.E, 4 * P.s.U, P.s.C};
    for (int k : ks) if (!rstep_k_ok(k, P.bf) || !rstep_k_ok(k, false)) p.shape = StepPath::SplitK;
    p.dual = training && g_side != nullptr && P.s.B >= 2 && (P.s.B % 2) == 0;
    p.loop = p.dual ? StepPath::SplitK : p.shape;
    p.mirrors = P.bf && p.loop == StepPath::Fused;
    p.try_chain = p.mirrors && P.s.step_kernels == 0;
    return p;
}
static int attn_bwd_chunks(const Plan& P, int nr) { return P.det() ? 1 : P.attn_chunks(nr); }

enum { kChainFwd = 0, kChainBwd = 1 };
static unsigned* chain_block(const Plan& P, void* ws, int which) { return P.ws<unsigned>(ws, W_XSYNC) + which * kXDecBlockWords; }
static unsigned* chain_err(const Plan& P, void* ws, int which) { return P.bf ? chain_block(P, ws, which) + kXDecErrWord : nullptr; }

struct InitProj { size_t woff; int n; ParamId bias, weight; float* x; int ldx; };
struct InitProjs { InitProj p[3]; const InitProj* begin() const { return p; } const InitProj* end() const { return p + 3; } };
static InitProjs init_projs(const Plan& P, float* c, int ldc, float* h, int ldh, float* o, int ldo) {
    const size_t blk = (size_t)P.s.U * P.s.C * P.esz;
    return {{{0, P.s.U, P_BC0, P_WC0, c, ldc}, {blk, P.s.U, P_BH0, P_WH0, h, ldh}, {2 * blk, P.s.O, P_BO0, P_WO0, o, ldo}}};
}

static int attention_prepare(const Plan& P, const StepPath& sp, const float* prm, const void* wp, void* ws, int beam, hipStream_t st) {
    const int B = P.s.B, C = P.s.C, E = P.s.E, U = P.s.U, O = P.s.O;
    RC(nt(P, false, false, false, P.ws<void>(ws, W_IMG), C, P.pk(wp, K_ATT_IMG_T), C, P.ws<void>(ws, W_ATT_IMG), E,
          B * P.R, E, C, nullptr, 0, false, st));
    RC(lxo_k_rowmean(P.s.dtype, P.ws<void>(ws, W_IMG), P.ws<float>(ws, W_MEAN), B, P.R, C, st));
    float* rec0 = P.ws<float>(ws, W_REC);
    const char* wt = (const char*)P.pk(wp, K_INIT_T);
    float* mean = P.ws<float>(ws, W_MEAN);
    const InitProjs state = init_projs(P, P.ws<float>(ws, W_CS), U, rec0 + O, P.REC, rec0, P.REC);
    float* tmp = P.ws<float>(ws, W_BEAM_TMP);
    const InitProjs out = beam <= 1 ? state : init_projs(P, tmp, U, tmp + (size_t)B * U, U, tmp + (size_t)2 * B * U, O);
    for (const InitProj& p : out) {
        if (beam <= 1 && sp.shape == StepPath::Fused) RC(rs_dense(P, mean, C, wt + p.woff, C, p.x, p.ldx, B, p.n, C, prm + P.poff[p.bias], true, false, st));
        else RC(nt(P, true, true, true, mean, C, wt + p.woff, C, p.x, p.ldx, B, p.n, C, prm + P.poff[p.bias], 2, false, st));
    }
    for (int i = 0; i < 3 && beam > 1; ++i)
        RC(lxo_k_tile_rows(out.p[i].x, out.p[i].ldx, state.p[i].x, state.p[i].ldx, B * beam, beam, out.p[i].n, st));
    return 0;
}

struct Step {
    const float *zx, *rec_prev, *cs_prev; float *rec_cur, *cs_cur; const bf16_t* recb_prev; bf16_t* recb_cur;
    float *gates, *atth, *alpha;
    const float* dolog; float *g, *dhc, *de, *datth, *dz; bf16_t *gb, *dzb;
};

static int cell_step(const Plan& P, const float* prm, const void* wp, void* ws, int r0, int nr, int beam, const Step& s, Drop dr, hipStream_t st) {
    const int C = P.s.C, E = P.s.E, U = P.s.U, O = P.s.O;
    const size_t r = (size_t)r0;
    float* s1 = P.ws<float>(ws, W_S_K1) + r * (P.XH / 128) * 4 * U;
    float* s2 = P.ws<float>(ws, W_S_K2) + r * (U / 128) * E;
    float* s4 = P.ws<float>(ws, W_S_K4) + r * (P.HC / 128) * O;
    const char* att_img = (const char*)P.ws<void>(ws, W_ATT_IMG) + (r / beam) * P.R * E * P.esz;
    const char* img = (const char*)P.ws<void>(ws, W_IMG) + (r / beam) * P.R * C * P.esz;
    float* part = P.ws<float>(ws, W_APART) + r * 32 * (C + 2);
    RC(slab(P, s.rec_prev, P.REC, P.pk(wp, K_LSTM_RT), P.ldRT, s1, nr, 4 * U, P.XH, st));
    RC(lxo_k_lstm_fwd(s.zx, view(s1, P.XH, nr, 4 * U), s.cs_prev, s.gates, s.cs_cur, s.rec_cur + O, s.rec_cur + P.OFF_HT, P.REC, dr, nr, U, st));
    RC(slab(P, s.rec_cur + P.OFF_HT, P.REC, P.pk(wp, K_ATT_H_T), P.ldAHT, s2, nr, E, U, st));
    RC(lxo_k_attn_fwd(P.s.dtype, att_img, img, nullptr, view(s2, U, nr, E), s.atth,
                      prm + P.poff[P_BETA], s.alpha, part, s.rec_cur + P.OFF_CTX, P.REC, nullptr, 0, nr, P.R, P.Rp, E, C, beam,
                      P.attn_chunks(nr), 0, st));
    RC(slab(P, s.rec_cur + P.OFF_HT, P.REC, P.pk(wp, K_OW_T), P.ldOWT, s4, nr, O, P.HC, st));
    RC(lxo_k_tanh_finalize(view(s4, P.HC, nr, O), s.rec_cur, P.REC, dr, nr, O, st));
    return 0;
}

static int cell_step_fused(const Plan& P, const float* prm, const void* wp, void* ws, int nr, int beam, const Step& s, Drop dr, hipStream_t st,
                           const int* zx_idx = nullptr, int zx_row = -1, const int* a_par = nullptr) {
    const int C = P.s.C, E = P.s.E, U = P.s.U, O = P.s.O;
    const bool bf = P.bf;
    const char* att_img = (const char*)P.ws<void>(ws, W_ATT_IMG);
    const char* img = (const char*)P.ws<void>(ws, W_IMG);
    float* part = P.ws<float>(ws, W_APART);
    RStep a; memset(&a, 0, sizeof(a));
    a.M = nr; a.U = U; a.O = O; a.dr = dr; a.zx_row = -1;
    RStep k1 = a;
    k1.A = bf ? (const void*)s.recb_prev : (const void*)s.rec_prev; k1.lda = bf ? P.RECB : P.REC;
    k1.W = P.pk(wp, K_LSTM_RT); k1.ldw = P.ldRT; k1.N = 4 * U; k1.K = P.XH; k1.epi = RS_LSTM_FWD;
    k1.zx = s.zx; k1.c_prev = s.cs_prev; k1.gates = s.gates; k1.c_out = s.cs_cur;
    k1.zx_idx = zx_idx; k1.zx_vocab = P.s.V; k1.zx_row = zx_row;
    k1.a_par = a_par; k1.a_k = beam;
    k1.out = s.rec_cur + O; k1.out2 = s.rec_cur + P.OFF_HT; k1.ldo = P.REC;
    if (bf) { k1.outb = s.recb_cur + O; k1.out2b = s.recb_cur + P.OFF_HT; k1.ldob = P.RECB; }
    RC(lxo_launch_rstep(P.s.dtype, bf, k1, st));
    RStep k2 = a;
    k2.A = bf ? (const void*)(s.recb_cur + P.OFF_HT) : (const void*)(s.rec_cur + P.OFF_HT); k2.lda = bf ? P.RECB : P.REC;
    k2.W = P.pk(wp, K_ATT_H_T); k2.ldw = P.ldAHT; k2.N = E; k2.K = U; k2.epi = RS_PLAIN;
    k2.out = s.atth; k2.ldo = E;
// ... 18 lines not shown
    return lxo_k_mirror(P.ws<float>(ws, W_REC) + slot_rows * P.REC, P.REC, P.ws<bf16_t>(ws, W_RECB) + slot_rows * P.RECB, P.RECB, rows, P.XH, st);
}
template <class X>
static void xdec_common(X& x, const Plan& P, const float* prm, const void* wp, void* ws) {
    x.Wrt = (const bf16_t*)P.pk(wp, K_LSTM_RT); x.ldrt = P.ldRT;
    x.Wah = (const bf16_t*)P.pk(wp, K_ATT_H_T); x.ldah = P.ldAHT;
    x.Wow = (const bf16_t*)P.pk(wp, K_OW_T); x.ldow = P.ldOWT;
    x.beta = prm + P.poff[P_BETA];
    x.img = P.ws<bf16_t>(ws, W_IMG);
    x.att_exp = P.att_exp() ? P.ws<bf16_t>(ws, W_ATT_EXP) : nullptr;
    x.rec = P.ws<float>(ws, W_REC); x.recb = P.ws<bf16_t>(ws, W_RECB); x.cs = P.ws<float>(ws, W_CS);
    x.part = P.ws<float>(ws, W_APART); x.sync = chain_block(P, ws, kChainFwd);
    x.B = P.s.B; x.R = P.R; x.REC = P.REC; x.RECB = P.RECB;
}

struct Train {
    const Plan& P; const float* prm; const void* wp; void* ws; hipStream_t st;
    StepPath sp;
    float *zx, *rec, *cs, *gates, *atth, *alpha; bf16_t* recb;
    float *dolog, *g, *dhc, *de, *datth, *dz, *dcc, *dxh; bf16_t *gb, *dzb;
    Step step(int t, int r0 = 0) const {
        const int B = P.s.B, U = P.s.U, O = P.s.O, E = P.s.E;
        const size_t p = (size_t)t * B + r0, c = p + B;
        Step s;
        s.zx = zx + p * 4 * U; s.rec_prev = rec + p * P.REC; s.cs_prev = cs + p * U; s.rec_cur = rec + c * P.REC; s.cs_cur = cs + c * U;
        s.recb_prev = recb ? recb + p * P.RECB : nullptr; s.recb_cur = recb ? recb + c * P.RECB : nullptr;
        s.gates = gates + p * 4 * U; s.atth = atth + p * E; s.alpha = alpha + p * P.Rp;
        s.dolog = dolog + p * O; s.g = g + p * O; s.dhc = dhc + p * P.HC; s.de = de + p * P.Rp; s.datth = datth + p * E; s.dz = dz + p * 4 * U;
        s.gb = gb ? gb + p * P.GBP : nullptr; s.dzb = dzb ? dzb + p * P.DZBP : nullptr;
        return s;
    }
};
static Train train_of(const Plan& P, const float* prm, const void* wp, void* ws, hipStream_t st) {
    Train w = {P, prm, wp, ws, st, step_path(P, true),
               P.ws<float>(ws, W_ZX), P.ws<float>(ws, W_REC), P.ws<float>(ws, W_CS), P.ws<float>(ws, W_GATES), P.ws<float>(ws, W_ATTH),
               P.ws<float>(ws, W_ALPHA), P.bf ? P.ws<bf16_t>(ws, W_RECB) : nullptr,
               P.ws<float>(ws, W_DOLOG), P.ws<float>(ws, W_G), P.ws<float>(ws, W_DHC), P.ws<float>(ws, W_DE), P.ws<float>(ws, W_DATTH),
               P.ws<float>(ws, W_DZ), P.ws<float>(ws, W_DCC), P.ws<float>(ws, W_DXH),
               P.bf ? P.ws<bf16_t>(ws, W_GB) : nullptr, P.bf ? P.ws<bf16_t>(ws, W_DZB) : nullptr};
    return w;
}

static int fwd_setup(const Train& w, const int* formula) {
    const Plan& P = w.P; void* ws = w.ws; hipStream_t st = w.st;
    const int B = P.s.B, T = P.s.T, U = P.s.U, D = P.s.D, V = P.s.V;
    RC(attention_prepare(P, w.sp, w.prm, w.wp, ws, 1, st));
    if (P.att_exp()) RC(lxo_k_att_exp(P.ws<void>(ws, W_ATT_IMG), P.ws<void>(ws, W_ATT_EXP), (long long)B * P.R * P.s.E, st));
    RC(lxo_k_embed_gather(P.s.dtype, w.prm + P.poff[P_EMB], w.prm + P.poff[P_START], formula, P.ws<void>(ws, W_EMB_IN), B, T, D, P.Dp, V, st));
    return nt(P, false, true, false, P.ws<void>(ws, W_EMB_IN), P.Dp, P.pk(w.wp, K_LSTM_XT), P.Dp, w.zx, 4 * U, T * B, 4 * U, P.Dp,
              w.prm + P.poff[P_LSTM_B], 0, false, st);
}
static int fwd_chain(const Train& w, const int* lengths, bool* ran) {
    const Plan& P = w.P; void* ws = w.ws;
    RC(mirror_oh(P, ws, 0, P.s.B, w.st));
    XDecFwd x; memset(&x, 0, sizeof(x));
    xdec_common(x, P, w.prm, w.wp, ws);
    x.att_img = P.ws<bf16_t>(ws, W_ATT_IMG);
    x.zx = w.zx; x.gates = w.gates; x.atth = w.atth; x.alpha = w.alpha;
    x.T = P.s.T; x.Rp = P.Rp;
    x.dr = P.drop(0, 0);
    x.lengths = lengths;
    LxoTimed tm("xdec_fwd", "chain", (double)P.s.T * P.s.B * P.R * (P.s.E + P.s.C) * P.esz, w.st);
    const int rc = lxo_launch_xdec_fwd(x, P.s.U, P.s.O, P.s.C, P.s.E, w.st);
    if (rc == 0) *ran = true;
    else if (rc != -2) return rc < 0 ? rc : -rc;
    return 0;
}
static int fwd_fused_loop(const Train& w) {
    const Plan& P = w.P;
    RC(mirror_oh(P, w.ws, 0, P.s.B, w.st));
    for (int t = 0; t < P.s.T; ++t) RC(cell_step_fused(P, w.prm, w.wp, w.ws, P.s.B, 1, w.step(t), P.drop(t, 0), w.st));
    return 0;
}
static int fwd_splitk_loop(const Train& w) {
    const Plan& P = w.P;
    const int nh = w.sp.dual ? 2 : 1, hb = P.s.B / nh;
    if (w.sp.dual) RC(fork_side(w.st));
    for (int t = 0; t < P.s.T; ++t)
        for (int h = 0; h < nh; ++h)
            RC(cell_step(P, w.prm, w.wp, w.ws, h * hb, hb, 1, w.step(t, h * hb), P.drop(t, h * hb), h ? g_side : w.st));
    if (w.sp.dual) RC(join_side(w.st));
    return 0;
}
static int fwd_logits(const Train& w) {
    const Plan& P = w.P;
    const bool m = w.sp.mirrors;
    return nt(P, !m, true, false, m ? (const void*)w.step(0).recb_cur : (const void*)w.step(0).rec_cur, m ? P.RECB : P.REC, P.pk(w.wp, K_YWO_T), P.s.O,
              P.ws<float>(w.ws, W_LOGITS), P.Vp, P.s.T * P.s.B, P.s.V, P.s.O, nullptr, 0, false, w.st);
}

int lxo_impl_decoder_train_fwd(const Plan& P, const float* prm, const void* wp, void* ws, const int* formula, hipStream_t st, const int* lengths) {
    const Train w = train_of(P, prm, wp, ws, st);
    RC(fwd_setup(w, formula));
    bool chain = false;
    if (w.sp.try_chain) RC(fwd_chain(w, lengths, &chain));
    if (P.bf && !chain) HIPRC(hipMemsetAsync(chain_block(P, ws, kChainFwd), 0, kXDecSyncBytes, st));
    if (w.sp.loop == StepPath::SplitK) RC(fwd_splitk_loop(w));
    else if (!chain) RC(fwd_fused_loop(w));
    return fwd_logits(w);
}

int lxo_impl_ce_loss(const Plan& P, void* ws, const int* formula, const int* lengths, float inv_ntok, const float* ntok_dev, hipStream_t st,
                     const float* w_tok, const float* w_row, const float* smooth_eps) {
    HIPRC(hipMemsetAsync(P.ws<float>(ws, W_LOSS), 0, 64, st));
    const CeWeights wt = {w_tok, w_row};
    const CeSmooth sm = {smooth_eps ? *smooth_eps : 0.f, smooth_eps ? *smooth_eps / (float)P.s.V : 0.f};
    RC(lxo_k_ce_loss(P.s.dtype, P.ws<float>(ws, W_LOGITS), formula, lengths, P.ws<void>(ws, W_DLOGITS), P.ws<float>(ws, W_LOSS),
                     inv_ntok, ntok_dev, chain_err(P, ws, kChainFwd), P.s.B, P.s.T, P.s.V, P.Vp,
                     DetScratch{P.ws<float>(ws, W_DET), P.wbytes[W_DET] / 4}, st,
                     (w_tok || w_row) ? &wt : nullptr, smooth_eps ? &sm : nullptr));
    return 0;
}

int lxo_impl_score_tokens(const Plan& P, void* ws, const int* formula, const int* lengths, float* logp_out, int* top1_out, float* seq_out, hipStream_t st) {
    return lxo_k_score(P.s.dtype, P.ws<float>(ws, W_LOGITS), formula, lengths, logp_out, top1_out, seq_out,
                       chain_err(P, ws, kChainFwd), P.s.B, P.s.T, P.s.V, P.Vp, st);
}

int lxo_impl_score_alternatives(const Plan& P, void* ws, const int* formula, const int* lengths, int k, const DecAllow* allow, int* ids_out, float* logp_out,
                                int* rank_out, float* ent_out, hipStream_t st) {
    return lxo_k_score_alt(P.s.dtype, P.ws<float>(ws, W_LOGITS), formula, lengths, k, allow, ids_out, logp_out, rank_out, ent_out,
                           chain_err(P, ws, kChainFwd), P.s.B, P.s.T, P.s.V, P.Vp, st);
}

hipStream_t lxo_impl_encoder_side_stream();
static thread_local hipEvent_t g_dbw_fork = nullptr, g_dbw_fork2 = nullptr, g_dbw_join = nullptr, g_dbw_init = nullptr;
struct BwdStreams {
    hipStream_t main, side;
    hipStream_t deferred() const { return side ? side : main; }
    int fork() const {
        if (!side) return 0;
        if (!g_dbw_fork) for (hipEvent_t* e : {&g_dbw_fork, &g_dbw_fork2, &g_dbw_join, &g_dbw_init}) HIPRC(hipEventCreateWithFlags(e, hipEventDisableTiming));
        HIPRC(hipEventRecord(g_dbw_fork, main));
        HIPRC(hipStreamWaitEvent(side, g_dbw_fork, 0));
        return 0;
    }
    int dmean_ready() const { if (side) HIPRC(hipEventRecord(g_dbw_init, side)); return 0; }
    int wait_dmean() const { if (side) HIPRC(hipStreamWaitEvent(main, g_dbw_init, 0)); return 0; }
    int datt_img_ready() const { if (side) HIPRC(hipEventRecord(g_dbw_fork2, main)); return 0; }
    int wait_datt_img() const { if (side) HIPRC(hipStreamWaitEvent(side, g_dbw_fork2, 0)); return 0; }
    int join(bool defer) const {
        if (!side || defer) return 0;
        HIPRC(hipEventRecord(g_dbw_join, side));
        HIPRC(hipStreamWaitEvent(main, g_dbw_join, 0));
        return 0;
    }
    int record_ready(void* ready) const {
        if (!ready) return 0;
        if (side) { HIPRC(hipEventRecord(g_dbw_fork, main)); HIPRC(hipStreamWaitEvent(side, g_dbw_fork, 0)); }
        HIPRC(hipEventRecord((hipEvent_t)ready, deferred()));
        return 0;
    }
};

static int bwd_logits(const Train& w, float* grads) {
    const Plan& P = w.P; hipStream_t st = w.st;
    const int B = P.s.B, TB = P.s.T * B, O = P.s.O, V = P.s.V;
    const void* dlog = P.ws<void>(w.ws, W_DLOGITS);
    RC(nt(P, false, true, false, dlog, P.Vp, P.pk(w.wp, K_YWO), P.Vp, w.dolog, O, TB, O, P.Vp, nullptr, 0, false, st));
    if (w.sp.mirrors) RC(tn(P, false, false, w.step(0).recb_cur, P.RECB, dlog, P.Vp, grads + P.poff[P_YWO], V, TB, O, V, st, P.det_scratch(w.ws)));
    else RC(tn(P, true, false, w.step(0).rec_cur, P.REC, dlog, P.Vp, grads + P.poff[P_YWO], V, TB, O, V, st));
    if (P.bf) RC(lxo_k_chain_poison(chain_err(P, w.ws, kChainFwd), nullptr, grads + P.ptotal - 1, st));
    return 0;
}
static int bwd_zero_acc(const Train& w) {
    HIPRC(hipMemsetAsync(w.dcc, 0, (size_t)w.P.s.B * w.P.s.U * 4, w.st));
    HIPRC(hipMemsetAsync(w.datth, 0, (size_t)w.P.s.T * w.P.s.B * w.P.s.E * 4, w.st));
    return 0;
}
static int bwd_last_g(const Train& w) {
    const Plan& P = w.P;
    const Step l = w.step(P.s.T - 1);
    return lxo_k_tanh_bwd(l.dolog, P.s.O, kNoSlabs, l.rec_cur, P.REC, l.g, P.s.O, l.gb, P.GBP, P.drop(P.s.T - 1, 0), 0, P.s.B, P.s.O, w.st);
}
static int bwd_chain(const Train& w, bool* ran) {
    const Plan& P = w.P; void* ws = w.ws; const void* wp = w.wp;
    XDecBwd x; memset(&x, 0, sizeof(x));
    x.Wow = (const bf16_t*)P.pk(wp, K_OW); x.ldow = P.ldOW;
    x.Wah = (const bf16_t*)P.pk(wp, K_ATT_H); x.ldah = P.ldAH;
    x.Wk = (const bf16_t*)P.pk(wp, K_LSTM) + (size_t)P.s.D * P.ldK; x.ldk = P.ldK;
    x.beta = w.prm + P.poff[P_BETA];
    x.att_img = P.ws<bf16_t>(ws, W_ATT_IMG); x.img = P.ws<bf16_t>(ws, W_IMG);
    x.att_exp = P.att_exp() ? P.ws<bf16_t>(ws, W_ATT_EXP) : nullptr;
    x.rec = w.rec; x.REC = P.REC; x.cs = w.cs; x.gates = w.gates; x.atth = w.atth; x.alpha = w.alpha; x.Rp = P.Rp;
    x.dolog = w.dolog; x.gall = w.g; x.gb = w.gb; x.GBP = P.GBP; x.dhc = w.dhc; x.de = w.de; x.datth = w.datth; x.datthb = P.ws<bf16_t>(ws, W_DATTHB);
    x.dz = w.dz; x.dzb = w.dzb; x.DZBP = P.DZBP; x.carry_h = P.ws<float>(ws, W_CARRYH); x.dcc = w.dcc; x.dxh = w.dxh;
    x.part = P.ws<float>(ws, W_APART);
    x.sync = chain_block(P, ws, kChainBwd);
    x.T = P.s.T; x.B = P.s.B; x.R = P.R;
    x.dr = P.drop(0, 0);
    LxoTimed tm("xdec_bwd", "chain", (double)P.s.T * P.s.B * P.R * (P.s.E + P.s.C) * P.esz, w.st);
    const int rc = lxo_launch_xdec_bwd(x, P.s.U, P.s.O, P.s.C, P.s.E, w.st);
    if (rc == 0) *ran = true;
    else if (rc != -2) return rc < 0 ? rc : -rc;
    else { RC(bwd_zero_acc(w)); HIPRC(hipMemsetAsync(x.sync, 0, kXDecSyncBytes, w.st)); }
    return 0;
}
static int bwd_fused_loop(const Train& w) {
    const Plan& P = w.P; void* ws = w.ws; const void* wp = w.wp; hipStream_t st = w.st;
    const int B = P.s.B, T = P.s.T, C = P.s.C, E = P.s.E, U = P.s.U, O = P.s.O;
    const bool bf = P.bf;
    float* carry_h = P.ws<float>(ws, W_CARRYH);
    const int nchb = attn_bwd_chunks(P, B);
    RStep a; memset(&a, 0, sizeof(a));
    a.U = U; a.O = O; a.zx_row = -1; a.M = B;
    for (int t = T - 1; t >= 0; --t) {
        const Step s = w.step(t);
        RStep b1 = a;
        b1.A = bf ? (const void*)s.gb : (const void*)s.g; b1.lda = bf ? P.GBP : O;
        b1.W = P.pk(wp, K_OW); b1.ldw = P.ldOW; b1.N = P.HC; b1.K = O; b1.epi = RS_PLAIN;
        b1.out = s.dhc; b1.ldo = P.HC;
        RC(lxo_launch_rstep(P.s.dtype, bf, b1, st));
        const Slabs dc1 = {s.dhc, 1, 0, P.HC};
        {
        LxoTimed tm("attn_bwd", "part", (double)B * P.R * (E + C) * P.esz, st);
        RC(lxo_k_attn_bwd(P.s.dtype, P.ws<void>(ws, W_ATT_IMG), P.att_exp() ? P.ws<void>(ws, W_ATT_EXP) : nullptr, P.ws<void>(ws, W_IMG), s.atth, w.prm + P.poff[P_BETA],
                          s.alpha, dc1, U, nullptr, P.HC, s.rec_cur + P.OFF_CTX, P.REC,
                          s.de, s.datth, B, P.R, P.Rp, E, C, nchb, att_alternate() ? (t & 1) : 0, st));
        }
        RStep b3 = a;
        b3.A = s.datth; b3.lda = E;
        b3.W = P.pk(wp, K_ATT_H); b3.ldw = P.ldAH; b3.N = U; b3.K = E; b3.epi = RS_LSTM_BWD;
        b3.dhm = s.dhc; b3.lddhm = P.HC; b3.carry_h = carry_h; b3.carry_rows = (t == T - 1) ? 0 : B;
        b3.gates_in = s.gates; b3.c_prev = s.cs_prev; b3.c_cur = s.cs_cur;
        b3.dcc = w.dcc; b3.out = s.dz; b3.outb = s.dzb; b3.ldob = P.DZBP; b3.dr = P.drop(t, 0);
        RC(lxo_launch_rstep(P.s.dtype, 0, b3, st));
        RStep b4 = a;
        b4.A = bf ? (const void*)s.dzb : (const void*)s.dz; b4.lda = bf ? P.DZBP : 4 * U;
        b4.W = (const char*)P.pk(wp, K_LSTM) + (size_t)P.s.D * P.ldK * P.esz; b4.ldw = P.ldK; b4.N = P.XH; b4.K = 4 * U; b4.epi = RS_CARRY;
        if (t == 0) { b4.first = 1; b4.out = w.dxh; b4.ldo = P.XH; }
        else {
            const Step q = w.step(t - 1);
            b4.out = q.g; b4.outb = q.gb; b4.ldob = P.GBP; b4.out2 = carry_h;
            b4.dolog = q.dolog; b4.o_prev = s.rec_prev; b4.ldoprev = P.REC;
            b4.dr = P.drop(t - 1, 0);
        }
        RC(lxo_launch_rstep(P.s.dtype, bf, b4, st));
    }
    return 0;
}
static int bwd_splitk_loop(const Train& w) {
    const Plan& P = w.P; void* ws = w.ws; const void* wp = w.wp;
    const int T = P.s.T, C = P.s.C, E = P.s.E, U = P.s.U, O = P.s.O;
    const int nh = w.sp.dual ? 2 : 1, hb = P.s.B / nh;
    const int nchb = attn_bwd_chunks(P, hb);
// ... 70 lines not shown
    const Plan& P = w.P; hipStream_t sd = s.deferred();
    const int B = P.s.B, T = P.s.T, TB = T * B, U = P.s.U, D = P.s.D;
    float* demb = P.ws<float>(w.ws, W_DEMB);
    if (w.sp.loop == StepPath::Fused) {
        RStep e; memset(&e, 0, sizeof(e));
        e.M = TB; e.N = D; e.K = 4 * U; e.U = U; e.O = P.s.O; e.zx_row = -1; e.epi = RS_PLAIN; e.dr.inv_keep = 1.f;
        e.A = P.bf ? (const void*)w.dzb : (const void*)w.dz; e.lda = P.bf ? P.DZBP : 4 * U;
        e.W = P.pk(w.wp, K_LSTM); e.ldw = P.ldK; e.out = demb; e.ldo = D;
        RC(lxo_launch_rstep(P.s.dtype, P.bf, e, sd));
    } else
        RC(nt(P, true, true, true, w.dz, 4 * U, P.pk(w.wp, K_LSTM), P.ldK, demb, D, TB, D, 4 * U, nullptr, 0, false, w.st));
    return lxo_k_embed_scatter(demb, formula, grads + P.poff[P_EMB], grads + P.poff[P_START], B, T, D, P.s.V, P.det() ? 1 : 0, sd);
}
static int bwd_datt_img(const Train& w, float* grads) {
    const Plan& P = w.P;
    return lxo_k_datt_img(P.s.dtype, P.ws<void>(w.ws, W_ATT_IMG), w.atth, w.prm + P.poff[P_BETA], w.de, P.ws<void>(w.ws, W_DATTIMG), grads + P.poff[P_BETA],
                          P.s.T, P.s.B, P.R, P.Rp, P.s.E, P.wbytes[W_ATTH_EXP] ? P.ws<float>(w.ws, W_ATTH_EXP) : nullptr, P.det_scratch(w.ws), w.st);
}
static int bwd_dimg_masked(const Train& w, float* grads, const BwdStreams& s) {
    const Plan& P = w.P; void* ws = w.ws;
    const int B = P.s.B;
    const DetScratch det = P.det_scratch(ws);
    RC(bwd_datt_img(w, grads));
    RC(s.datt_img_ready());
    RC(s.wait_dmean());
    DimgArgs a; memset(&a, 0, sizeof(a));
    a.alpha = w.alpha; a.ld_alpha = (long long)B * P.Rp; a.Rp = P.Rp;
    a.dctx = w.dhc + P.s.U; a.ld_dctx = (long long)B * P.HC; a.HC = P.HC;
    a.datt = P.ws<bf16_t>(ws, W_DATTIMG); a.W = (const bf16_t*)P.pk(w.wp, K_ATT_IMG); a.ldw = P.s.E;
    a.dmean = P.ws<float>(ws, W_DMEAN); a.T = P.s.T; a.B = B; a.R = P.R; a.C = P.s.C; a.E = P.s.E;
    a.y6 = P.ws<bf16_t>(ws, W_Y6); a.dy6 = P.ws<bf16_t>(ws, W_DIMG); a.db = grads + P.poff[P_CONV6_B];
    if (P.det()) { a.db_part = det.p; a.db_part_floats = det.floats; }
    return lxo_launch_dimg_fused(a, w.st);
}
static int bwd_dimg_plain(const Train& w, float* grads, const BwdStreams& s) {
    const Plan& P = w.P; void* ws = w.ws; hipStream_t st = w.st;
    const int B = P.s.B, C = P.s.C, E = P.s.E;
    float* dimg = P.ws<float>(ws, W_DIMG);
    GemmTN g; memset(&g, 0, sizeof(g));
    g.A = w.alpha; g.B = w.dhc + P.s.U; g.C = dimg; g.M = P.s.T; g.I = P.R; g.J = C;
    g.lda = B * P.Rp; g.ldb = B * P.HC; g.ldc = C;
    g.nsplit = 1; g.nbatch = B; g.strideA = P.Rp; g.strideB = P.HC; g.strideC = (long long)P.R * C; g.atomic = 0;
    RC(lxo_launch_gemm_tn(P.s.dtype, 1, 1, g, st));
    RC(s.wait_dmean());
    RC(lxo_k_add_mean_grad(dimg, P.ws<float>(ws, W_DMEAN), B, P.R, C, st));
    RC(bwd_datt_img(w, grads));
    RC(s.datt_img_ready());
    return nt(P, false, true, false, P.ws<void>(ws, W_DATTIMG), E, P.pk(w.wp, K_ATT_IMG), E, dimg, C, B * P.R, C, E, nullptr, 0, true, st);
}

int lxo_impl_decoder_train_bwd(const Plan& P, const float* prm, const void* wp, void* ws, const int* formula, float* grads,
                               int parts, hipStream_t st, bool defer_join, void* ready) {
    const Train w = train_of(P, prm, wp, ws, st);
    if (parts & 1) RC(bwd_logits(w, grads));
    if (!(parts & 2)) return 0;
    bool chain = false;
    if (!w.sp.try_chain) {
        RC(bwd_zero_acc(w));
        if (P.bf) HIPRC(hipMemsetAsync(chain_block(P, ws, kChainBwd), 0, kXDecSyncBytes, st));
    }
    if (w.sp.loop == StepPath::SplitK) RC(bwd_splitk_loop(w));
    else {
        RC(bwd_last_g(w));
        if (w.sp.try_chain) RC(bwd_chain(w, &chain));
        if (!chain) RC(bwd_fused_loop(w));
    }
    const BwdStreams s = {st, (w.sp.mirrors && !lxo_timer_on()) ? lxo_impl_encoder_side_stream() : nullptr};
    const DetScratch det_s = s.side ? P.det_scratch_side(ws) : P.det_scratch(ws);
    RC(s.fork());
    RC(bwd_init_states(w, grads, s, det_s));
    RC(bwd_weight_grads(w, grads, chain, s, det_s));
    RC(P.dimg_masked() ? bwd_dimg_masked(w, grads, s) : bwd_dimg_plain(w, grads, s));
    RC(bwd_embedding(w, formula, grads, BwdStreams{st, nullptr}));
    RC(s.wait_datt_img());
    RC(tn(P, false, false, P.ws<void>(ws, W_IMG), P.s.C, P.ws<void>(ws, W_DATTIMG), P.s.E, grads + P.poff[P_ATT_IMG], P.s.E, P.s.B * P.R, P.s.C, P.s.E,
          s.deferred(), det_s));
    RC(s.join(defer_join));
    if (chain) RC(lxo_k_chain_poison(nullptr, chain_err(P, ws, kChainBwd), grads + P.ptotal - 1, st));
    return s.record_ready(ready);
}

struct Dec {
    int k, nv;
    bool beam;
    int *flags, *finished;
    int *ids_step, *par_step;
    float *logp, *tmp;
    float *rec, *cs; bf16_t* recb;
    float *logits, *alpha;
    StepPath path;
    bool fused() const { return path.shape == StepPath::Fused; }
};
static Dec dec_of(const Plan& P, void* ws, int k, bool beam) {
    Dec d;
    d.k = k; d.nv = P.s.B * k; d.beam = beam;
    d.flags = P.ws<int>(ws, W_DEC_FLAGS); d.finished = d.flags + 64;
    d.ids_step = P.ws<int>(ws, W_DEC_IDS); d.par_step = P.ws<int>(ws, W_BEAM_PAR);
    d.logp = P.ws<float>(ws, W_BEAM_LP); d.tmp = P.ws<float>(ws, W_BEAM_TMP);
    d.rec = P.ws<float>(ws, W_REC); d.cs = P.ws<float>(ws, W_CS);
    d.logits = P.ws<float>(ws, W_DEC_LOGITS); d.alpha = P.ws<float>(ws, W_ALPHA);
    d.path = step_path(P, false);
    d.recb = d.path.mirrors ? P.ws<bf16_t>(ws, W_RECB) : nullptr;
    return d;
}
static int decode_token_table(const Plan& P, const float* prm, const void* wp, void* ws, hipStream_t st) {
    const int U = P.s.U, D = P.s.D, V = P.s.V;
    RC(lxo_k_embed_table(P.s.dtype, prm + P.poff[P_EMB], prm + P.poff[P_START], P.ws<void>(ws, W_DEC_TXE), V, D, P.Dp, st));
    RC(nt(P, false, true, false, P.ws<void>(ws, W_DEC_TXE), P.Dp, P.pk(wp, K_LSTM_XT), P.Dp, P.ws<float>(ws, W_DEC_TX), 4 * U, V + 1, 4 * U, P.Dp,
          prm + P.poff[P_LSTM_B], 0, false, st));
    return 0;
}
static int decode_common_step(const Plan& P, const float* prm, const void* wp, void* ws, const Dec& d, int time, const int* ids_prev, hipStream_t st, const int* a_par = nullptr) {
    const int U = P.s.U, O = P.s.O, D = P.s.D, V = P.s.V, nv = d.nv;
    const size_t cur = (size_t)((time + 1) & 1) * nv, prev = (size_t)(time & 1) * nv;
    Step s; memset(&s, 0, sizeof(s));
    s.rec_prev = d.rec + prev * P.REC; s.cs_prev = d.cs + prev * U; s.rec_cur = d.rec + cur * P.REC; s.cs_cur = d.cs + cur * U;
    if (d.recb) { s.recb_prev = d.recb + prev * P.RECB; s.recb_cur = d.recb + cur * P.RECB; }
    s.atth = P.ws<float>(ws, W_ATTH); s.alpha = d.alpha;
// ... 279 lines not shown
```

### latex_ocr_amd/csrc/model_encoder.hip

```cpp
#include "impl.h"
#include "gemm.h"
#include "encoder_kernels.h"
#include "decoder_kernels.h"
#include "api_util.h"
#include "timing.h"

int lxo_impl_pack_weights(const Plan& P, const float* prm, void* wp, hipStream_t st) {
    const int dt = P.s.dtype, C = P.s.C, E = P.s.E, U = P.s.U, O = P.s.O, D = P.s.D, V = P.s.V;
    PackTable tab; memset(&tab, 0, sizeof(tab));
    int blocks = 0;
    auto add = [&](int kind, long long src, size_t dst, int K, int N, int lds, int ldd, int coff, int Kpad) {
        PackJob& j = tab.job[tab.n++];
        j.kind = kind; j.K = K; j.N = N; j.lds = lds; j.ldd = ldd; j.coff = coff; j.Kpad = Kpad; j.src = src; j.dst = (long long)dst;
        if (kind == 0) j.nblocks = cdiv(Kpad, 32) * cdiv(N, 32);
        else if (kind == 1) { long long t = cdivl((long long)K * Kpad, 256 * 4); j.nblocks = (int)(t < 1 ? 1 : (t > 512 ? 512 : t)); }
        else { long long t = cdivl((long long)K * 9 * N, 256 * 4); j.nblocks = (int)(t < 1 ? 1 : (t > 512 ? 512 : t)); }
        j.first_block = blocks; blocks += j.nblocks;
    };
    auto tr = [&](long long src, size_t dst, int K, int N, int ldd, int coff, int Kpad) { add(0, src, dst, K, N, N, ldd, coff, Kpad); };
    auto cp = [&](long long src, size_t dst, int R, int Ccols, int ldd, int Cpad) { add(1, src, dst, R, Ccols, Ccols, ldd, 0, Cpad); };
    for (int l = 1; l < 6; ++l) {
        const int ci = P.convCin[l], co = P.convCout[l];
        tr(P.poff[P.convW[l]], P.koff[K_CONV2_F + l - 1], 9 * ci, co, 9 * ci, 0, 9 * ci);
        add(2, P.poff[P.convW[l]], P.koff[K_CONV2_D + l - 1], ci, co, 0, 0, 0, 0);
    }
    if (P.cnn) {
        tr(P.poff[P_CONVS_W], P.koff[K_CONVS_F], 8 * C, C, 8 * C, 0, 8 * C);
        cp(P.poff[P_CONVS_W], P.koff[K_CONVS_D], 8 * C, C, C, C);
    }
    tr(P.poff[P_ATT_IMG], P.koff[K_ATT_IMG_T], C, E, C, 0, C);
    cp(P.poff[P_ATT_IMG], P.koff[K_ATT_IMG], C, E, E, E);
    {
        const int pid[3] = {P_WC0, P_WH0, P_WO0};
        const int nout[3] = {U, U, O};
        size_t offT = 0, offN = 0;
        for (int i = 0; i < 3; ++i) {
            tr(P.poff[pid[i]], P.koff[K_INIT_T] + offT, C, nout[i], C, 0, C);
            cp(P.poff[pid[i]], P.koff[K_INIT] + offN, C, nout[i], nout[i], nout[i]);
            offT += (size_t)nout[i] * C * P.esz; offN += (size_t)C * nout[i] * P.esz;
        }
    }
    const long long K = P.poff[P_LSTM_K];
    tr(K, P.koff[K_LSTM_XT], D, 4 * U, P.Dp, 0, P.Dp);
    tr(K + (long long)D * 4 * U, P.koff[K_LSTM_RT], P.XH, 4 * U, P.ldRT, 0, P.XH);
    cp(K, P.koff[K_LSTM], D + P.XH, 4 * U, P.ldK, 4 * U);
    tr(P.poff[P_ATT_H], P.koff[K_ATT_H_T], U, E, P.ldAHT, 0, U);
    cp(P.poff[P_ATT_H], P.koff[K_ATT_H], U, E, P.ldAH, E);
    tr(P.poff[P_OWH], P.koff[K_OW_T], U, O, P.ldOWT, 0, U);
    tr(P.poff[P_OWC], P.koff[K_OW_T], C, O, P.ldOWT, U, C);
    cp(P.poff[P_OWH], P.koff[K_OW], U, O, P.ldOW, O);
    cp(P.poff[P_OWC], P.koff[K_OW] + (size_t)U * P.ldOW * P.esz, C, O, P.ldOW, O);
    tr(P.poff[P_YWO], P.koff[K_YWO_T], O, V, O, 0, O);
    cp(P.poff[P_YWO], P.koff[K_YWO], O, V, P.Vp, P.Vp);
    if (P.rnn) {
        const int Ur = P.Ur;
        for (int d = 0; d < 2; ++d) {
            const long long k = P.poff[P_ROWF_K + 2 * d];
            tr(k, P.koff[K_ROWX_T + d], C, 4 * Ur, C, 0, C);
            cp(k, P.koff[K_ROWX + d], C, 4 * Ur, 4 * Ur, 4 * Ur);
            tr(k + (long long)C * 4 * Ur, P.koff[K_ROWH_T + d], Ur, 4 * Ur, Ur, 0, Ur);
            cp(k + (long long)C * 4 * Ur, P.koff[K_ROWH + d], Ur, 4 * Ur, 4 * Ur, 4 * Ur);
        }
    }
    return lxo_k_pack_batch(dt, tab, blocks, prm, wp, st);
}

static const char* conv_name(int Cin, int Cout, bool valid) {
    if (valid) return "conv6";
    if (Cin == 64) return "conv2";
    if (Cin == 128) return "conv3";
    return Cin == Cout ? "conv4" : "conv5";
}
static int conv_fwd(const Plan& P, const void* in, const void* wpk, const float* bias, void* out,
                    int H, int W, int Cin, int Cout, bool valid, const float* addend, int addend_rows,
                    void* out_pre, hipStream_t st) {
    GemmNT g; memset(&g, 0, sizeof(g));
    g.A = in; g.Bp = wpk; g.C = out;
    g.conv = 1; g.H = H; g.W = W; g.Cin = Cin;
    g.Ho = valid ? H - 2 : H; g.Wo = valid ? W - 2 : W; g.pad = valid ? 0 : 1;
    g.M = P.Be * g.Ho * g.Wo; g.N = Cout; g.K = 9 * Cin;
    g.lda = Cin; g.ldb = 9 * Cin; g.ldc = Cout;
    g.bias = bias; g.act = 1; g.alpha = 1.f;
    g.addend = addend; g.addend_rows = addend_rows > 0 ? addend_rows : 1; g.out_pre = out_pre;
    LxoTimed tm("conv_fwd", conv_name(Cin, Cout, valid), 2.0 * g.M * g.N * g.K, st);
    return lxo_launch_gemm_nt(P.s.dtype, 0, 0, 0, g, st);
}
static int conv_fwd_pool(const Plan& P, const void* in, const void* wpk, const float* bias, int H, int W, int Cin, int Cout,
                         void* pooled, void* mask, int ph, int pw, hipStream_t st) {
    GemmNT g; memset(&g, 0, sizeof(g));
    g.A = in; g.Bp = wpk; g.C = nullptr;
    g.conv = 1; g.H = H; g.W = W; g.Cin = Cin; g.Ho = H; g.Wo = W; g.pad = 1;
    g.M = P.Be * H * W; g.N = Cout; g.K = 9 * Cin;
    g.lda = Cin; g.ldb = 9 * Cin; g.ldc = Cout;
    g.bias = bias; g.act = 1; g.alpha = 1.f; g.addend_rows = 1;
    g.pool_out = pooled; g.pool_mask = (unsigned char*)mask; g.pool_h = ph; g.pool_w = pw;
    LxoTimed tm("conv_fwd", conv_name(Cin, Cout, false), 2.0 * g.M * g.N * g.K, st);
    return lxo_launch_gemm_nt(P.s.dtype, 0, 0, 0, g, st);
}
static int conv_dgrad(const Plan& P, const void* dout, const void* wd, void* din, int Hout, int Wout, int Cout,
                      int Hin, int Win, int Cin, bool valid, const void* relu_ref, float* colsum, DetScratch det, hipStream_t st) {
    GemmNT g; memset(&g, 0, sizeof(g));
    g.A = dout; g.Bp = wd; g.C = din;
    g.conv = 1; g.H = Hout; g.W = Wout; g.Cin = Cout;
    g.Ho = Hin; g.Wo = Win; g.pad = valid ? 2 : 1;
    g.M = P.Be * Hin * Win; g.N = Cin; g.K = 9 * Cout;
    g.lda = Cout; g.ldb = 9 * Cout; g.ldc = Cin;
    g.act = 0; g.alpha = 1.f; g.addend_rows = 1;
    g.relu_ref = relu_ref; g.ldr = Cin; g.colsum = colsum;
    if (P.det() && colsum) { g.colsum_part = det.p; g.colsum_part_floats = det.floats; }
    LxoTimed tm("conv_dgrad", conv_name(Cin, Cout, valid), 2.0 * P.Be * Hout * Wout * 9.0 * Cin * Cout, st);
    return lxo_launch_gemm_nt(P.s.dtype, 0, 0, 0, g, st);
}
static int conv_wgrad(const Plan& P, const void* in, const void* dout, float* dw, int H, int W, int Cin, int Cout,
                      bool valid, DetScratch det, hipStream_t st) {
    GemmTN g; memset(&g, 0, sizeof(g));
    g.A = in; g.B = dout; g.C = dw;
    g.conv = 1; g.H = H; g.W = W; g.Cin = Cin;
// ... 197 lines not shown
```

### latex_ocr_amd/csrc/rstep.h

```cpp
#pragma once
#include "lxo_common.h"
#include "decoder_kernels.h"

enum RStepEpi {
    RS_PLAIN = 0,
    RS_TANH_O = 1,
    RS_LSTM_FWD = 2,
    RS_LSTM_BWD = 3,
    RS_CARRY = 4,
};

struct RStep {
    const void* A; int lda;
    const void* W; int ldw;
    int M, N, K, epi;
    int U, O;
    float* out; int ldo;
    bf16_t* outb; int ldob;
    float* out2; bf16_t* out2b;
    const float* zx; const float* c_prev; float* gates; float* c_out;
    const int* a_par; int a_k;
    const int* zx_idx; int zx_vocab, zx_row;
    const float* dhm; int lddhm; const float* carry_h; const float* gates_in; const float* c_cur; float* dcc; int carry_rows;
    const float* bias; int accumulate;
    const float* dolog; const float* o_prev; int ldoprev; int first;
    Drop dr;
    unsigned long long* dbg;
};

int lxo_launch_rstep(int dt, int a_bf16, const RStep& p, hipStream_t st);
#include "lxo_debug.h"
int lxo_k_mirror(const float* src, int lds, void* dst, int ldd, int rows, int cols, hipStream_t st);
```

### latex_ocr_amd/csrc/rstep.hip

```cpp
#include "rstep.h"
#include "drop.h"
#include "api_util.h"
#include "switches.h"

namespace {

typedef __attribute__((ext_vector_type(4))) float v4f;

LXO_DEV v4f mfma16_bf16(u32x4 a, u32x4 b, v4f c) {
    return __builtin_amdgcn_mfma_f32_16x16x32_bf16(__builtin_bit_cast(bf16x8_t, a), __builtin_bit_cast(bf16x8_t, b), c, 0, 0, 0);
}

template <bool FAST> LXO_DEV float tanh_e(float x) {
    if constexpr (FAST) return 1.f - 2.f * __builtin_amdgcn_rcpf(__builtin_amdgcn_exp2f(x * 2.8853900817779268f) + 1.f);
    else return tanhf(x);
}
template <bool FAST> LXO_DEV float sigm_e(float x) {
    if constexpr (FAST) return __builtin_amdgcn_rcpf(1.f + __builtin_amdgcn_exp2f(x * -1.4426950408889634f));
    else return sigmoidf_(x);
}

LXO_DEV u32x4 frag8(const bf16_t* p) { return *reinterpret_cast<const u32x4*>(p); }
LXO_DEV u32x4 frag8(const float* p) {
    const f32x4 a = *reinterpret_cast<const f32x4*>(p), b = *reinterpret_cast<const f32x4*>(p + 4);
// ... 120 lines not shown
                    acc[rb] = mfma16_bf16(*reinterpret_cast<const u32x4*>(&As[(rb * 16 + r) * PITCH + s * 32 + g * 8]), bw, acc[rb]);
            } else {
                const f32x4 bw = *reinterpret_cast<const f32x4*>(&Ws[r * PITCH + s * 16 + g * 4]);
                f32x4 aw[RB];
#pragma unroll
                for (int rb = 0; rb < RB; ++rb) aw[rb] = *reinterpret_cast<const f32x4*>(&As[(rb * 16 + r) * PITCH + s * 16 + g * 4]);
#pragma unroll
                for (int e = 0; e < 4; ++e)
#pragma unroll
                    for (int rb = 0; rb < RB; ++rb)
                        acc[rb] = __builtin_amdgcn_mfma_f32_16x16x4f32(aw[rb][e], bw[e], acc[rb], 0, 0, 0);
            }
        }
        __builtin_amdgcn_wave_barrier();
        if (c == 0) STAMP(3);
    }
#undef ISSUE
    STAMP(4);
#pragma unroll
    for (int rb = 0; rb < RB; ++rb)
#pragma unroll
        for (int i = 0; i < 4; ++i) red[wave][rb * 16 + g * 4 + i][r] = acc[rb][i];
    __syncthreads();
    STAMP(5);
    if (!mok) return;

    if constexpr (EPI == RS_LSTM_FWD) {
        const int U = p.U, u = blockIdx.x * 4 + part;
        float a[4];
#pragma unroll
        for (int q = 0; q < 4; ++q) {
            const float z = pz[q] + red[0][row][q * 4 + part] + red[1][row][q * 4 + part] + red[2][row][q * 4 + part] + red[3][row][q * 4 + part];
            a[q] = (q == 1) ? tanh_e<BF>(z) : sigm_e<BF>(q == 2 ? z + 1.0f : z);
        }
        const float c = a[2] * pcp + a[0] * a[1];
        const float h = a[3] * tanh_e<BF>(c);
        const float ht = h * drop_scale(p.dr, 1u, m, u, U);
        if (p.gates) {
#pragma unroll
            for (int q = 0; q < 4; ++q) p.gates[(long long)m * 4 * U + q * U + u] = a[q];
        }
        p.c_out[(long long)m * U + u] = c;
        p.out[(long long)m * p.ldo + u] = h;
        p.out2[(long long)m * p.ldo + u] = ht;
        if (p.outb) { p.outb[(long long)m * p.ldob + u] = f2bf(h); p.out2b[(long long)m * p.ldob + u] = f2bf(ht); }
        STAMP(6);
        return;
    } else {
        if (n >= p.N) return;
        float v[4];
#pragma unroll
        for (int e = 0; e < 4; ++e) v[e] = red[0][row][part * 4 + e] + red[1][row][part * 4 + e] + red[2][row][part * 4 + e] + red[3][row][part * 4 + e];
        if constexpr (EPI == RS_PLAIN || EPI == RS_TANH_O) {
            if (p.bias) { float b4[4]; ld4(p.bias + n, b4); for (int e = 0; e < 4; ++e) v[e] += b4[e]; }
            if (p.accumulate) { float o4[4]; ld4(p.out + (long long)m * p.ldo + n, o4); for (int e = 0; e < 4; ++e) v[e] += o4[e]; }
        }
        if constexpr (EPI == RS_PLAIN) {
            st4(p.out + (long long)m * p.ldo + n, v);
            if (p.outb) st4b(p.outb + (long long)m * p.ldob + n, v);
        } else if constexpr (EPI == RS_TANH_O) {
#pragma unroll
            for (int e = 0; e < 4; ++e) v[e] = tanh_e<BF>(v[e]) * drop_scale(p.dr, 2u, m, n + e, p.N);
            st4(p.out + (long long)m * p.ldo + n, v);
            if (p.outb) st4b(p.outb + (long long)m * p.ldob + n, v);
        } else if constexpr (EPI == RS_LSTM_BWD) {
            const int U = p.U;
            float dzi[4], dzj[4], dzf[4], dzo[4], dcn[4];
#pragma unroll
            for (int e = 0; e < 4; ++e) {
                const float dh = (e0[e] + v[e]) * drop_scale(p.dr, 1u, m, n + e, U) + e1[e];
                const float tc = tanh_e<BF>(e6[e]);
                const float dc = e8[e] + dh * e5[e] * (1.f - tc * tc);
                dzi[e] = dc * e3[e] * e2[e] * (1.f - e2[e]);
                dzj[e] = dc * e2[e] * (1.f - e3[e] * e3[e]);
                dzf[e] = dc * e7[e] * e4[e] * (1.f - e4[e]);
                dzo[e] = dh * tc * e5[e] * (1.f - e5[e]);
                dcn[e] = dc * e4[e];
            }
            float* dzr = p.out + (long long)m * 4 * U + n;
            st4(dzr, dzi); st4(dzr + U, dzj); st4(dzr + 2 * U, dzf); st4(dzr + 3 * U, dzo);
            if (p.outb) {
                bf16_t* db = p.outb + (long long)m * p.ldob + n;
                st4b(db, dzi); st4b(db + U, dzj); st4b(db + 2 * U, dzf); st4b(db + 3 * U, dzo);
            }
            st4(p.dcc + (long long)m * U + n, dcn);
        } else if constexpr (EPI == RS_CARRY) {
            const int O = p.O;
            if (p.first) { st4(p.out + (long long)m * p.ldo + n, v); STAMP(6); return; }
            if (n < O) {
#pragma unroll
                for (int e = 0; e < 4; ++e) {
                    const float sc = drop_scale(p.dr, 2u, m, n + e, O);
                    const float th = (p.dr.thr == 0u) ? e1[e] : e1[e] / p.dr.inv_keep;
                    v[e] = (e0[e] + v[e]) * sc * (1.f - th * th);
                }
                st4(p.out + (long long)m * O + n, v);
                if (p.outb) st4b(p.outb + (long long)m * p.ldob + n, v);
            } else {
                st4(p.out2 + (long long)m * p.U + (n - O), v);
            }
        }
        STAMP(6);
    }
}

template <typename AT, typename WT, int EPI, int MT, int KC>
// ... 6 lines not shown
    case 8: hipLaunchKernelGGL((rstep_kernel<AT, WT, EPI, MT, KC, 8, 4>), grid, dim3(256), 0, st, p.A, p.W, p.lda, p.ldw, p.M, p.N, p.K, p.U, p.a_par, p.a_k > 0 ? p.a_k : 1, p); break;
    case 16: hipLaunchKernelGGL((rstep_kernel<AT, WT, EPI, MT, KC, 16, 4>), grid, dim3(256), 0, st, p.A, p.W, p.lda, p.ldw, p.M, p.N, p.K, p.U, p.a_par, p.a_k > 0 ? p.a_k : 1, p); break;
    default: return -2;
    }
    return (int)hipGetLastError();
}
template <typename AT, typename WT, int EPI>
int launch_ch(const RStep& p, hipStream_t st) {
    constexpr bool BF = is_bf16<WT>::value;
    constexpr int K0 = (BF && sizeof(AT) == 2) ? 64 : 32;
    constexpr int KMIN = BF ? 32 : 16;
    const int kq = p.K / 4;
    const int ncol = EPI == RS_LSTM_FWD ? p.U / 4 : cdiv(p.N, 16);
    const bool half = ((long long)ncol * cdiv(p.M, 64) <= 128 && p.M > 32) || (p.M > 64 && p.M <= 512);
    const bool quarter = lxo_switch(SW_RSTEP_MT16) && (long long)ncol * cdiv(p.M, 32) <= 128 && p.M > 16;
    if (kq % K0 == 0) {
        if (quarter) return launch_nch<AT, WT, EPI, 16, K0>(p, dim3(ncol, cdiv(p.M, 16)), st);
        if (half) return launch_nch<AT, WT, EPI, 32, K0>(p, dim3(ncol, cdiv(p.M, 32)), st);
        return launch_nch<AT, WT, EPI, 64, K0>(p, dim3(ncol, cdiv(p.M, 64)), st);
    }
    if constexpr (K0 / 2 >= KMIN) {
        if (kq % (K0 / 2) == 0) return launch_nch<AT, WT, EPI, 64, K0 / 2>(p, dim3(ncol, cdiv(p.M, 64)), st);
    }
    return -2;
}

template <int EPI>
int launch_epi(int dt, bool a_bf16, const RStep& p, hipStream_t st) {
    if (dt == LXO_F32) return launch_ch<float, float, EPI>(p, st);
    return a_bf16 ? launch_ch<bf16_t, bf16_t, EPI>(p, st) : launch_ch<float, bf16_t, EPI>(p, st);
}

__global__ __launch_bounds__(256) void mirror_kernel(const float* __restrict__ src, int lds, bf16_t* __restrict__ dst, int ldd, int rows, int cols) {
    const int total = rows * (cols >> 2);
    for (int i = blockIdx.x * 256 + threadIdx.x; i < total; i += gridDim.x * 256) {
        const int r = i / (cols >> 2), c = (i - r * (cols >> 2)) << 2;
        float v[4];
        ld4(src + (long long)r * lds + c, v);
        st4b(dst + (long long)r * ldd + c, v);
    }
}

}

static thread_local unsigned long long* g_dbg = nullptr;
static thread_local int g_dbg_epi = -1;
extern "C" int lxo_rstep_debug(unsigned long long* buf, int epi) { g_dbg = buf; g_dbg_epi = epi; return 0; }
int lxo_launch_rstep(int dt, int a_bf16, const RStep& p0, hipStream_t st) {
    RStep p = p0;
    p.dbg = (g_dbg && p.epi == g_dbg_epi) ? g_dbg : nullptr;
    if (p.M <= 0 || p.N <= 0) return 0;
    if (p.K % 128 != 0 || p.lda % 8 != 0 || p.ldw % 8 != 0 || p.N % 4 != 0) return -2;
    if (p.epi == RS_LSTM_FWD && (p.U % 4 != 0 || p.N != 4 * p.U)) return -2;
    switch (p.epi) {
    case RS_PLAIN: return launch_epi<RS_PLAIN>(dt, a_bf16 != 0, p, st);
    case RS_TANH_O: return launch_epi<RS_TANH_O>(dt, a_bf16 != 0, p, st);
    case RS_LSTM_FWD: return launch_epi<RS_LSTM_FWD>(dt, a_bf16 != 0, p, st);
    case RS_LSTM_BWD: return launch_epi<RS_LSTM_BWD>(dt, a_bf16 != 0, p, st);
    case RS_CARRY: return launch_epi<RS_CARRY>(dt, a_bf16 != 0, p, st);
    default: return -2;
    }
}

int lxo_k_mirror(const float* src, int lds, void* dst, int ldd, int rows, int cols, hipStream_t st) {
    if (rows <= 0 || cols <= 0) return 0;
    if (cols % 4 != 0 || lds % 4 != 0 || ldd % 4 != 0) return -2;
    int g = cdiv(rows * (cols >> 2), 256);
    if (g > 1024) g = 1024;
    hipLaunchKernelGGL(mirror_kernel, dim3(g), dim3(256), 0, st, src, lds, (bf16_t*)dst, ldd, rows, cols);
    return (int)hipGetLastError();
}
```

### latex_ocr_amd/csrc/xdec.h

```cpp
#pragma once
#include "lxo.h"
#include "lxo_common.h"
#include "decoder_kernels.h"
#include "lxo_debug.h"

struct XDecFwd {
    const bf16_t* Wrt; int ldrt;
    const bf16_t* Wah; int ldah;
    const bf16_t* Wow; int ldow;
    const float* beta;
    const bf16_t* att_img;
    const bf16_t* att_exp;
    const bf16_t* img;
    const float* zx;
    float* rec; bf16_t* recb;
    float* cs;
    float* gates;
    float* atth;
    float* alpha;
    float* part;
    unsigned* sync;
    int T, B, R, Rp, REC, RECB;
    Drop dr;
    unsigned long long* dbg;
    const int* lengths;
};

int lxo_launch_xdec_fwd(const XDecFwd& p, int U, int O, int C, int E, hipStream_t st);

struct XDecDec {
    const bf16_t* Wrt; int ldrt; const bf16_t* Wah; int ldah; const bf16_t* Wow; int ldow;
    const bf16_t* Wyo; int ldyo;
    const float* beta;
    const bf16_t* att_exp;
    const bf16_t* img;
    const float* tx;
    float* rec; bf16_t* recb;
    float* cs;
    float* part;
    unsigned* sync;
    int* ids_step;
    int* ids_out;
    int* finished;
    int* unfinished;
    int* stop;
    int B, R, REC, RECB, V, id_end, t0, nsteps, max_steps;
    float* logp_out;
    const int* prefix;
    const int* prefix_len;
    int prefix_ld, prefix_lim;
    const unsigned* allow;
    int allow_ld;
};
int lxo_launch_xdec_dec(const XDecDec& p, int U, int O, int C, int E, hipStream_t st);

struct XDecBwd {
    const bf16_t* Wow; int ldow;
    const bf16_t* Wah; int ldah;
    const bf16_t* Wk; int ldk;
    const float* beta;
    const bf16_t* att_img; const bf16_t* att_exp; const bf16_t* img;
    const float* rec; int REC;
    const float* cs; const float* gates; const float* atth; const float* alpha; int Rp;
    const float* dolog;
    float* gall; bf16_t* gb; int GBP;
    float* dhc;
    float* de;
    float* datth;
    bf16_t* datthb;
    float* dz; bf16_t* dzb; int DZBP;
    float* carry_h;
    float* dcc;
    float* dxh;
    float* part;
    unsigned* sync;
    int T, B, R;
    Drop dr;
    unsigned long long* dbg;
};
int lxo_launch_xdec_bwd(const XDecBwd& p, int U, int O, int C, int E, hipStream_t st);
constexpr size_t kXDecSyncBytes = 4096, kXDecLLBytes = 384u << 10, kXDecBlockBytes = kXDecSyncBytes + kXDecLLBytes;
constexpr size_t kXDecBlockWords = kXDecBlockBytes / 4;
constexpr size_t kXDecErrWord = 8 * 64;
constexpr size_t kXDecTicketBytes = kXDecErrWord * 4;
static_assert(kXDecErrWord == LXO_XDEC_ERR_WORD, "include/lxo.h names the error word for the callers");
constexpr size_t kLLFwdHt = 0, kLLFwdAh = 128u << 10, kLLFwdO = 256u << 10;
constexpr size_t kLLBwdGb = 0, kLLBwdDctx = 128u << 10;
```

### latex_ocr_amd/csrc/xdec.hip

```cpp
#include "xdec.h"
#include "drop.h"
#include "api_util.h"
#include "switches.h"

#ifdef LXO_HIPSIM
int lxo_launch_xdec_fwd(const XDecFwd&, int, int, int, int, hipStream_t) { return -2; }
int lxo_launch_xdec_bwd(const XDecBwd&, int, int, int, int, hipStream_t) { return -2; }
int lxo_launch_xdec_dec(const XDecDec&, int, int, int, int, hipStream_t) { return -2; }
extern "C" int lxo_xdec_debug(unsigned long long*) { return 0; }
extern "C" int lxo_xdec_debug_bwd(unsigned long long*) { return 0; }
#else

HIP_DYNAMIC_SHARED(char, xdec_dyn_lds)

namespace {
constexpr int XU = 512, XO = 512, XC = 512, XE = 256;
constexpr int XXH = XO + XU, XHC = XU + XC;
constexpr int OFF_H = XO, OFF_HT = XO + XU, OFF_CTX = XO + 2 * XU;
constexpr int XW = 8;
#ifndef LXO_XDEC_LLMASK
#define LXO_XDEC_LLMASK 15
#endif
constexpr int kLL = LXO_XDEC_LLMASK;
#ifndef LXO_XDEC_LLMASK_B
#define LXO_XDEC_LLMASK_B 7
#endif
constexpr int kLLB = LXO_XDEC_LLMASK_B;

#ifndef LXO_XDEC_PF
#define LXO_XDEC_PF 0
#endif
constexpr int kPF = LXO_XDEC_PF;
#ifndef LXO_XDEC_PFB
#define LXO_XDEC_PFB 0
#endif
constexpr int kPFB = LXO_XDEC_PFB;

constexpr int PST = XC + 4;
constexpr int PLW = 264;
static_assert(PLW * 2 <= XC + 16, "plan.hip sizes att_part with C + 16 floats per partial");
constexpr int SCMAX = 2432;

typedef __attribute__((ext_vector_type(4))) float v4f;
LXO_DEV v4f mfma16(u32x4 a, u32x4 b, v4f c) {
    return __builtin_amdgcn_mfma_f32_16x16x32_bf16(__builtin_bit_cast(bf16x8_t, a), __builtin_bit_cast(bf16x8_t, b), c, 0, 0, 0);
}
LXO_DEV float tanh_x(float x) { return 1.f - 2.f * __builtin_amdgcn_rcpf(__builtin_amdgcn_exp2f(x * 2.8853900817779268f) + 1.f); }
LXO_DEV float sigm_x(float x) { return __builtin_amdgcn_rcpf(1.f + __builtin_amdgcn_exp2f(x * -1.4426950408889634f)); }

typedef __amdgpu_buffer_rsrc_t rsrc_t;
LXO_DEV rsrc_t make_rsrc(const void* base, unsigned bytes) { return __builtin_amdgcn_make_buffer_rsrc(const_cast<void*>(base), 0, (int)bytes, 0x00020000); }
LXO_DEV u32x4 l2_load16(rsrc_t r, unsigned byte_off) { return __builtin_amdgcn_raw_buffer_load_b128(r, (int)byte_off, 0, 16); }
LXO_DEV float l2_load4(rsrc_t r, unsigned byte_off) { return __uint_as_float(__builtin_amdgcn_raw_buffer_load_b32(r, (int)byte_off, 0, 16)); }

LXO_DEV void xbar(unsigned* flags, int rank, unsigned ph, unsigned* err, int* s_dead) {
    asm volatile("s_waitcnt vmcnt(0)" ::: "memory");
    __syncthreads();
    const int tid = threadIdx.x;
    if (tid < 64) {
        if (tid == 0) *reinterpret_cast<volatile unsigned*>(flags + rank) = ph;
// ... 1335 lines not shown
            if (tid < NB * 32) {
                float v = 0.f;
#pragma unroll
                for (int w = 0; w < XW; ++w) v += red[w][e4r][e4c];
                const int bb = b0 + e4r, n = n0 + e4c;
                if (t == 0) p.dxh[(long long)bb * XXH + n] = v;
                else if (n < XO) {
                    Drop dq = dr; dq.t = t - 1;
                    const float sc = drop_scale(dq, 2u, bb, n, XO);
                    const float th = (dq.thr == 0u) ? qo : qo / dq.inv_keep;
                    const float g = (qd + v) * sc * (1.f - th * th);
                    p.gall[(sp - B + bb) * XO + n] = g;
                    const bf16_t gbv = f2bf(g);
                    p.gb[(sp - B + bb) * p.GBP + n] = gbv;
                    if (kLLB & 1) {
                        const unsigned mine = (unsigned)gbv, other = (unsigned)__shfl_xor((int)mine, 1);
                        if (!(e4c & 1)) { const u32x2 wv = {mine | (other << 16), (unsigned)t}; *reinterpret_cast<u32x2*>(ll_gb + ((bb * 256 + (n >> 1)) * 2)) = wv; }
                    }
                } else p.carry_h[(long long)bb * XU + (n - XO)] = v;
            }
        }
        XSTAMP(T - 1 - t, 7);
        if (kLLB & 1) __syncthreads();
        else xbar(xsync, rank, ++ph, err, &s_dead);
        XSTAMP(T - 1 - t, 8);
    }
    if (tid < NB * 16) p.dcc[(long long)(b0 + e3r) * XU + u0 + e3u] = cst[e3r][e3u];
}

template <int NB>
int launch_bwd_nb(const XDecBwd& p, hipStream_t st) {
    return p.att_exp ? xdec_launch<xdec_bwd_kernel<NB, 4, true>>(p, st) : xdec_launch<xdec_bwd_kernel<NB, 4, false>>(p, st);
}
}

static int xdec_gate(LxoSwitch own, int U, int O, int C, int E, int B, int R, int rows_max) {
    if (!lxo_switch(SW_XDEC) || !lxo_switch(own)) return 0;
    if (U != XU || O != XO || C != XC || E != XE) return 0;
    if (B % 8 != 0 || B > 64) return 0;
    const int nb = B / 8;
    if (nb != 1 && nb != 2 && nb != 4 && nb != 8) return 0;
    const int nq = 32 / nb, rows_per = (R + nq - 1) / nq;
    if (rows_per > rows_max || rows_per < 1) return 0;
    static int dev_ok = -1;
    if (dev_ok < 0) {
        int dev = 0; hipDeviceProp_t pr;
        dev_ok = (hipGetDevice(&dev) == hipSuccess && hipGetDeviceProperties(&pr, dev) == hipSuccess && pr.multiProcessorCount == 256) ? 1 : 0;
    }
    return dev_ok ? nb : 0;
}

static thread_local unsigned long long* g_xdbg = nullptr;
extern "C" int lxo_xdec_debug(unsigned long long* buf) { g_xdbg = buf; return 0; }
int lxo_launch_xdec_fwd(const XDecFwd& p0, int U, int O, int C, int E, hipStream_t st) {
    XDecFwd p = p0;
    p.dbg = g_xdbg;
    const int nb = xdec_gate(SW_XDEC, U, O, C, E, p.B, p.R, SCMAX);
    if (!nb || p.T < 1) return -2;
    if ((long long)p.B * p.RECB * 2 >= (1LL << 31) || p.ldrt % 8 || p.ldah % 8 || p.ldow % 8 || p.RECB % 8) return -2;
    HIPRC(hipMemsetAsync(p.sync, 0, kXDecBlockBytes, st));
    if (kLL & 4) HIPRC(hipMemsetAsync(p.part, 0, (size_t)p.B * (32 / nb) * PLW * 8, st));

    switch (nb) {
    case 1: return launch_nb<1>(p, st);
    case 2: return launch_nb<2>(p, st);
    case 4: return launch_nb<4>(p, st);
    default: return launch_nb<8>(p, st);
    }
}
int lxo_launch_xdec_dec(const XDecDec& p, int U, int O, int C, int E, hipStream_t st) {
    const int nb = xdec_gate(SW_XDEC_DEC, U, O, C, E, p.B, p.R, 1 << 30);
    if (!nb || p.nsteps < 1 || p.nsteps > 16 || p.V < 1 || p.V > 512 || !p.stop) return -2;
    if ((long long)p.B * p.RECB * 2 >= (1LL << 31) || p.ldrt % 8 || p.ldah % 8 || p.ldow % 8 || p.ldyo % 8 || p.RECB % 8 || !p.att_exp) return -2;
    HIPRC(hipMemsetAsync(p.sync, 0, 8 * 64 * 4, st));
    HIPRC(hipMemsetAsync(p.sync + 8 * 64 + 1, 0, kXDecBlockBytes - (8 * 64 + 1) * 4, st));
    HIPRC(hipMemsetAsync(p.sync + kXDecBlockBytes / 4 + kXDecSyncBytes / 4, 0, (size_t)p.B * 32 * 8 * (p.logp_out ? (p.prefix ? 3 : 2) : 1), st));
    if (kLL & 4) HIPRC(hipMemsetAsync(p.part, 0, (size_t)p.B * (32 / nb) * PLW * 8, st));
    switch (nb) {
    case 1: return launch_dec_nb<1>(p, st);
    case 2: return launch_dec_nb<2>(p, st);
    case 4: return launch_dec_nb<4>(p, st);
    default: return launch_dec_nb<8>(p, st);
    }
}
static thread_local unsigned long long* g_xdbg_b = nullptr;
extern "C" int lxo_xdec_debug_bwd(unsigned long long* buf) { g_xdbg_b = buf; return 0; }
int lxo_launch_xdec_bwd(const XDecBwd& p0, int U, int O, int C, int E, hipStream_t st) {
    XDecBwd p = p0;
    p.dbg = g_xdbg_b;
    const int nb = xdec_gate(SW_XDEC_BWD, U, O, C, E, p.B, p.R, SCMAX);
    if (!nb || p.T < 1) return -2;
    if (p.ldow % 8 || p.ldah % 8 || p.ldk % 8 || p.GBP % 8 || p.DZBP % 8 || p.REC % 4 || (long long)p.B * p.DZBP * 2 >= (1LL << 31)) return -2;
    HIPRC(hipMemsetAsync(p.sync, 0, kXDecBlockBytes, st));
    if (kLLB & 4) HIPRC(hipMemsetAsync(p.part, 0, (size_t)p.B * (32 / nb) * XE * 4, st));
    switch (nb) {
    case 1: return launch_bwd_nb<1>(p, st);
    case 2: return launch_bwd_nb<2>(p, st);
    case 4: return launch_bwd_nb<4>(p, st);
    default: return launch_bwd_nb<8>(p, st);
    }
}
#endif
```

### latex_ocr_amd/engine.py

```python
import ctypes
import math
import os
from collections import OrderedDict, namedtuple

import numpy as np
import torch

from . import _abi
from .model import params as PP


Alternatives = namedtuple("Alternatives", ["ids", "logp", "rank", "entropy"])


def _p(t):
    return ctypes.c_void_p(t.data_ptr()) if t is not None else ctypes.c_void_p(0)


def _cost_kind(what, cost):
    if not isinstance(cost, str) or cost not in ("edit", "bleu"):
        raise ValueError("%s: cost must be \"edit\" or \"bleu\", got %r" % (what, cost))
    return _abi.LXO_COST_BLEU if cost == "bleu" else _abi.LXO_COST_EDIT


# ... 449 lines not shown
                                                  hi, lo, st), "encoder_bwd")
                comm(*rng)
        else:
            self._ck(self.lib.lxo_encoder_bwd(self.sref(), _p(self.params), _p(self.wpack), _p(self.ws), _p(self._img), _p(self.grads),
                                              6, 1, st), "encoder_bwd")

    def _enc_ready_events(self):
        if getattr(self, "_enc_ready", None) is None:
            cur = torch.cuda.current_stream(self.device)
            evs = [None] * 7
            for lo in [0] + [lo for (hi, lo), _ in self.enc_buckets]:
                evs[lo] = torch.cuda.Event()
                evs[lo].record(cur)
            self._enc_ready = evs
        return self._enc_ready

    METHODS = {"adam": 0, "sgd": 1, "adagrad": 2, "rmsprop": 3}

    def set_optimizer(self, lr_method):
        m = lr_method.lower()
        if m not in self.METHODS:
            raise NotImplementedError("Unknown method {}".format(lr_method))
        self.method = self.METHODS[m]
        if self.method == 2:
            self.adam_v.fill_(0.1)
        elif self.method == 3:
            self.adam_v.fill_(1.0)

    def optimizer_step(self, lr, clip=-1.0, beta1=0.9, beta2=0.999, eps=1e-8, guard=False, dp=False):
        st = self._stream()
        possible = self._chains_possible() or (dp and self.dtype == _abi.LXO_BF16 and self.device.type == "cuda")
        guard = guard and possible and self.ws is not None and self.shape is not None
        if getattr(self, "method", 0) != 0:
            scale = None
            if clip is not None and clip > 0:
                self._ck(self.lib.lxo_global_norm_scale(self.n_params, _p(self.grads), ctypes.c_float(clip), _p(self.scale), st), "clip")
                scale = self.scale
            if guard:
                self._chain_health_post(scale is not None, dp)
                scale = self.scale
            self._ck(self.lib.lxo_optimizer_step(self.method, self.n_params, _p(self.params), _p(self.grads), _p(self.adam_v),
                                                 ctypes.c_float(float(lr)), _p(scale), st), "optimizer_step")
            self.pack()
            return
        self.adam_t += 1
        lr_t = float(lr) * math.sqrt(1.0 - beta2 ** self.adam_t) / (1.0 - beta1 ** self.adam_t)
        scale = None
        if clip is not None and clip > 0:
            self._ck(self.lib.lxo_global_norm_scale(self.n_params, _p(self.grads), ctypes.c_float(clip), _p(self.scale), st), "clip")
            scale = self.scale
        if guard:
            self._chain_health_post(scale is not None, dp)
            scale = self.scale
        self._ck(self.lib.lxo_adam_step(self.n_params, _p(self.params), _p(self.grads), _p(self.adam_m), _p(self.adam_v),
                                        ctypes.c_float(lr_t), ctypes.c_float(beta1), ctypes.c_float(beta2), ctypes.c_float(eps),
                                        _p(scale), st), "adam")
        self.pack()

    def train_step(self, img, formula, lengths, lr, clip=-1.0, dist=None, sync_loss=True, dropout=1.0, dropout_seed=None,
                   weights=None, row_weights=None, norm=None, label_smoothing=0.0):
        eps = self._check_smoothing("train_step", label_smoothing)
        weighted = weights is not None or row_weights is not None
        if weighted:
            weights, row_weights = self._check_weights("train_step", weights, row_weights, int(img.shape[0]), int(formula.shape[1]))
        if norm is not None and not (math.isfinite(float(norm)) and float(norm) != 0.0):
            raise ValueError("train_step: norm must be a finite non-zero number, got %r" % (norm,))
        wkw = dict(weights=weights, row_weights=row_weights) if weighted else {}
        if eps > 0.0:
            wkw["label_smoothing"] = eps
        drop = None
        if dropout is not None and 0.0 < float(dropout) < 1.0:
            self.drop_step = getattr(self, "drop_step", 0) + 1
            world, rank = (dist.world, dist.rank) if dist is not None else (1, 0)
            drop = (float(dropout), dropout_seed if dropout_seed is not None else self.drop_step * world + rank)
        n_local = int(np.asarray(lengths).sum()) if not isinstance(lengths, torch.Tensor) else int(lengths.sum().item())
        if self._health_ring is not None and dist is None:
            self._chain_health_poll()
        if dist is not None and norm is None:
            ntok, ev = dist.sum_count_async(n_local)
            self.forward(img, formula, dropout=drop, before_decoder=ev, lengths=lengths)
            stats = self.loss(lengths, ntok_dev=ntok, ntok_event=ev, _bound=True, **wkw)
        else:
            self.forward(img, formula, dropout=drop, lengths=lengths)
            stats = self.loss(lengths, 1.0 / (float(n_local) if norm is None else float(norm)), _bound=True, **wkw)
        self.backward(comm=dist.reduce_range_fn(self.grads) if dist is not None else None)
        if dist is not None:
            dist.finish()
        self.optimizer_step(lr, clip, guard=True, dp=dist is not None)
        if not sync_loss:
            return None
        if dist is not None:
            s = stats.clone()
            dist.all_reduce(s)
            s = s.cpu().numpy()
        else:
            s = stats.cpu().numpy()
        if (self._health_ring is not None and self._chain_health_poll(wait=True) and getattr(self, "_last_dropped_seq", -1) == self._health_i
                and dist is None and not getattr(self, "_redoing", False)):
            self._redoing = True
            try:
                return self.train_step(img, formula, lengths, lr, clip=clip, dist=None, sync_loss=True, dropout=dropout,
                                       dropout_seed=drop[1] if drop is not None else None, norm=norm, **wkw)
            finally:
                self._redoing = False
        self.last_ce = float(s[3 if len(s) == 4 else 0]) / max(float(s[1]), 1.0)
        return float(s[0]) / (float(s[1]) if norm is None else float(norm))

    def mrt_grads(self, img, cand, cand_lengths, group_sizes, cost, alpha, dropout=None):
        cand_h = cand.detach().cpu().numpy() if isinstance(cand, torch.Tensor) else np.asarray(cand)
        ln = np.ascontiguousarray(np.asarray(cand_lengths), dtype=np.int64).reshape(-1)
# ... 765 lines not shown
```

Before: 9133 img/s.

## Fuse Adam update with weight repacking and fold xdec memsets into chain-arm kernel

```diff
diff --git a/include/lxo.h b/include/lxo.h
--- a/include/lxo.h
+++ b/include/lxo.h
@@ -148,6 +148,8 @@
 int lxo_global_norm_scale(long long n, const float* grads, float clip, float* scale_out, void* stream);
 int lxo_adam_step(long long n, float* params, const float* grads, float* m, float* v,
                   float lr_t, float beta1, float beta2, float eps, const float* scale_dev, void* stream);
+int lxo_adam_pack_step(const lxo_shape* s, float* params, const float* grads, float* m, float* v, void* wpack,
+                       float lr_t, float beta1, float beta2, float eps, const float* scale_dev, void* stream);
 
 int lxo_optimizer_step(int method, long long n, float* params, const float* grads, float* slot, float lr,
                        const float* scale_dev, void* stream);
diff --git a/latex_ocr_amd/_abi.py b/latex_ocr_amd/_abi.py
--- a/latex_ocr_amd/_abi.py
+++ b/latex_ocr_amd/_abi.py
@@ -87,6 +87,7 @@
         "lxo_decoder_train_bwd": (c_int, [S, c_void, c_void, c_void, c_void, c_void, c_void]),
         "lxo_global_norm_scale": (c_int, [c_ll, c_void, c_float, c_void, c_void]),
         "lxo_adam_step": (c_int, [c_ll, c_void, c_void, c_void, c_void, c_float, c_float, c_float, c_float, c_void, c_void]),
+        "lxo_adam_pack_step": (c_int, [S, c_void, c_void, c_void, c_void, c_void, c_float, c_float, c_float, c_float, c_void, c_void]),
         "lxo_optimizer_step": (c_int, [c_int, c_ll, c_void, c_void, c_void, c_float, c_void, c_void]),
         "lxo_greedy_decode": (c_int, [S, c_void, c_void, c_void, c_int, c_int, c_void, P(c_int), c_void]),
         "lxo_greedy_decode_attn": (c_int, [S, c_void, c_void, c_void, c_int, c_int, c_void, c_void, P(c_int), c_void]),
@@ -139,7 +140,7 @@
 ENTRY_POINTS = ["lxo_last_error", "lxo_version", "lxo_shape_size", "lxo_ws_region_dtype", "lxo_timing_enable", "lxo_timing_count", "lxo_timing_get", "lxo_gemm_nt", "lxo_gemm_tn", "lxo_conv3x3", "lxo_conv3x3_ex", "lxo_conv3x3_wgrad", "lxo_gemm_slab", "lxo_attention_fwd", "lxo_param_num", "lxo_param_name", "lxo_param_name_for",
                 "lxo_param_total", "lxo_param_info", "lxo_wpack_bytes", "lxo_workspace_bytes", "lxo_ws_region",
                 "lxo_pack_weights", "lxo_encoder_fwd", "lxo_encoder_bwd", "lxo_encoder_bwd_ready", "lxo_train_bwd", "lxo_set_side_stream", "lxo_set_encoder_side_stream", "lxo_decoder_train_fwd", "lxo_decoder_train_fwd_live",
-                "lxo_ce_loss_fwd_bwd", "lxo_ce_loss_fwd_bwd_dev", "lxo_ce_loss_weighted", "lxo_ce_loss_smoothed", "lxo_mrt_weights", "lxo_edit_distance", "lxo_text_stats", "lxo_mrt_candidates", "lxo_consensus", "lxo_sentence_bleu", "lxo_consensus_bleu", "lxo_mrt_candidates_cost", "lxo_decoder_train_bwd", "lxo_decoder_train_bwd_part", "lxo_global_norm_scale", "lxo_adam_step", "lxo_optimizer_step",
+                "lxo_ce_loss_fwd_bwd", "lxo_ce_loss_fwd_bwd_dev", "lxo_ce_loss_weighted", "lxo_ce_loss_smoothed", "lxo_mrt_weights", "lxo_edit_distance", "lxo_text_stats", "lxo_mrt_candidates", "lxo_consensus", "lxo_sentence_bleu", "lxo_consensus_bleu", "lxo_mrt_candidates_cost", "lxo_decoder_train_bwd", "lxo_decoder_train_bwd_part", "lxo_global_norm_scale", "lxo_adam_step", "lxo_adam_pack_step", "lxo_optimizer_step",
                 "lxo_greedy_decode", "lxo_greedy_decode_attn", "lxo_beam_decode", "lxo_beam_decode_attn", "lxo_greedy_decode_scores", "lxo_beam_decode_scores", "lxo_score_tokens", "lxo_score_alternatives", "lxo_greedy_decode_prefix", "lxo_beam_decode_prefix", "lxo_greedy_decode_constrained", "lxo_beam_decode_constrained", "lxo_sample_decode", "lxo_sample_tokens",
                 "lxo_grammar_scratch_bytes", "lxo_greedy_decode_grammar", "lxo_beam_decode_grammar", "lxo_sample_decode_grammar", "lxo_grammar_step", "lxo_decode_begin", "lxo_decode_step",
                 "lxo_chain_guard", "lxo_decode_state_get", "lxo_decode_state_set", "lxo_decode_cell_step",
diff --git a/latex_ocr_amd/csrc/adam_update.h b/latex_ocr_amd/csrc/adam_update.h
--- /dev/null
+++ b/latex_ocr_amd/csrc/adam_update.h
@@ -0,0 +1,13 @@
+#pragma once
+#include "lxo_common.h"
+
+__device__ __forceinline__ float adam_update(float* __restrict__ p, const float* __restrict__ g, float* __restrict__ m, float* __restrict__ v,
+                                             long long i, float sc, float lr_t, float b1, float b2, float eps) {
+    const float gi = g[i] * sc;
+    const float mi = b1 * m[i] + (1.f - b1) * gi;
+    const float vi = b2 * v[i] + (1.f - b2) * gi * gi;
+    m[i] = mi; v[i] = vi;
+    const float pi = p[i] - lr_t * mi / (sqrtf(vi) + eps);
+    p[i] = pi;
+    return pi;
+}
diff --git a/latex_ocr_amd/csrc/api.hip b/latex_ocr_amd/csrc/api.hip
--- a/latex_ocr_amd/csrc/api.hip
+++ b/latex_ocr_amd/csrc/api.hip
@@ -299,6 +299,12 @@
 extern "C" int lxo_adam_step(long long n, float* params, const float* grads, float* m, float* v,
                              float lr_t, float beta1, float beta2, float eps, const float* scale_dev, void* stream) {
     CHECK_LAUNCH(lxo_k_adam(params, grads, m, v, n, lr_t, beta1, beta2, eps, scale_dev, (hipStream_t)stream), "lxo_adam_step");
+    return 0;
+}
+extern "C" int lxo_adam_pack_step(const lxo_shape* s, float* params, const float* grads, float* m, float* v, void* wpack,
+                                  float lr_t, float beta1, float beta2, float eps, const float* scale_dev, void* stream) {
+    MAKE_PLAN(P, s);
+    CHECK_LAUNCH(lxo_impl_adam_pack(P, params, grads, m, v, wpack, lr_t, beta1, beta2, eps, scale_dev, (hipStream_t)stream), "lxo_adam_pack_step");
     return 0;
 }
 extern "C" int lxo_greedy_decode(const lxo_shape* s, const float* params, const void* wpack, void* ws,
diff --git a/latex_ocr_amd/csrc/decoder_kernels.h b/latex_ocr_amd/csrc/decoder_kernels.h
--- a/latex_ocr_amd/csrc/decoder_kernels.h
+++ b/latex_ocr_amd/csrc/decoder_kernels.h
@@ -12,6 +12,9 @@
 int lxo_k_lstm_bwd(const float* gates, const float* c_prev, const float* c_cur, Slabs s1, Slabs s3, Slabs s4, int off4,
                    float* dcc, float* dz, Drop dr, int carry_rows, int B, int U, hipStream_t st);
 int lxo_k_tanh_bwd(const float* a, int lda, Slabs carry, const float* o, int ldo, float* g, int ldg, void* gb, int ldgb, Drop dr, int carry_rows, int rows, int cols, hipStream_t st);
+struct ChainArm { int kind; const float* a; int lda; const float* o; int ldo; float* g; int ldg; bf16_t* gb; int ldgb; Drop dr; int rows, cols;
+                  const unsigned* poison_err; float* probe; };
+int lxo_k_chain_arm(void* z0, size_t bytes0, void* z1, size_t bytes1, const ChainArm& w, hipStream_t st);
 int lxo_k_slab_reduce(Slabs sl, float* o, int ldo, int rows, int cols, hipStream_t st);
 int lxo_k_tanh_finalize(Slabs sl, float* o, int ldo, Drop dr, int rows, int cols, hipStream_t st);
 int lxo_k_attn_fwd(int dt, const void* att_img, const void* img, const float* att_h, Slabs ahs, float* att_h_out, const float* beta, float* alpha, float* part,
diff --git a/latex_ocr_amd/csrc/decoder_kernels.hip b/latex_ocr_amd/csrc/decoder_kernels.hip
--- a/latex_ocr_amd/csrc/decoder_kernels.hip
+++ b/latex_ocr_amd/csrc/decoder_kernels.hip
@@ -1,6 +1,7 @@
 #include "decoder_kernels.h"
 #include "api_util.h"
 #include "drop.h"
+#include "adam_update.h"
 
 namespace {
 
@@ -211,24 +212,45 @@
     }
 }
 
+LXO_DEV void tanh_bwd_item(int i, const float* __restrict__ a, int lda, const Slabs& carry, const float* __restrict__ o, int ldo, float* __restrict__ g, int ldg,
+                           bf16_t* __restrict__ gb, int ldgb, const Drop& dr, int carry_rows, int cols) {
+    const int r = i / (cols >> 2), c = (i - r * (cols >> 2)) << 2;
+    const f32x4 ov = *reinterpret_cast<const f32x4*>(o + (long long)r * ldo + c);
+    f32x4 d = *reinterpret_cast<const f32x4*>(a + (long long)r * lda + c);
+    if (r < carry_rows) d += slab_sum4(carry, r, c);
+    f32x4 out;
+#pragma unroll
+    for (int e = 0; e < 4; ++e) {
+        const float sc = drop_scale(dr, 2u, r, c + e, cols);
+        const float th = (dr.thr == 0u) ? ov[e] : ov[e] / dr.inv_keep;
+        out[e] = d[e] * sc * (1.f - th * th);
+    }
+    *reinterpret_cast<f32x4*>(g + (long long)r * ldg + c) = out;
+    if (gb) { u32x2 pk = {pack_bf2(out[0], out[1]), pack_bf2(out[2], out[3])}; *reinterpret_cast<u32x2*>(gb + (long long)r * ldgb + c) = pk; }
+}
 __global__ __launch_bounds__(256) void tanh_bwd_kernel(const float* __restrict__ a, int lda, Slabs carry,
                                                       const float* __restrict__ o, int ldo, float* __restrict__ g, int ldg,
                                                       bf16_t* __restrict__ gb, int ldgb, Drop dr, int carry_rows, int rows, int cols) {
     const int total = rows * (cols >> 2);
-    for (int i = blockIdx.x * 256 + threadIdx.x; i < total; i += gridDim.x * 256) {
-        const int r = i / (cols >> 2), c = (i - r * (cols >> 2)) << 2;
-        const f32x4 ov = *reinterpret_cast<const f32x4*>(o + (long long)r * ldo + c);
-        f32x4 d = *reinterpret_cast<const f32x4*>(a + (long long)r * lda + c);
-        if (r < carry_rows) d += slab_sum4(carry, r, c);
-        f32x4 out;
-#pragma unroll
-        for (int e = 0; e < 4; ++e) {
-            const float sc = drop_scale(dr, 2u, r, c + e, cols);
-            const float th = (dr.thr == 0u) ? ov[e] : ov[e] / dr.inv_keep;
-            out[e] = d[e] * sc * (1.f - th * th);
-        }
-        *reinterpret_cast<f32x4*>(g + (long long)r * ldg + c) = out;
-        if (gb) { u32x2 pk = {pack_bf2(out[0], out[1]), pack_bf2(out[2], out[3])}; *reinterpret_cast<u32x2*>(gb + (long long)r * ldgb + c) = pk; }
+    for (int i = blockIdx.x * 256 + threadIdx.x; i < total; i += gridDim.x * 256) tanh_bwd_item(i, a, lda, carry, o, ldo, g, ldg, gb, ldgb, dr, carry_rows, cols);
+}
+__global__ __launch_bounds__(256) void chain_arm_kernel(u32x2* __restrict__ z0, int n0, u32x2* __restrict__ z1, int n1, ChainArm w) {
+    const int t = blockIdx.x * 256 + threadIdx.x, nt = gridDim.x * 256;
+    const u32x2 zero = {0u, 0u};
+    for (int i = t; i < n0; i += nt) z0[i] = zero;
+    for (int i = t; i < n1; i += nt) z1[i] = zero;
+    if (t == 0 && w.probe && w.poison_err[0]) w.probe[0] = __uint_as_float(0x7fc00000u);
+    const int total = w.rows * (w.cols >> 2);
+    if (w.kind == 1) {
+        for (int i = t; i < total; i += nt) {
+            const int r = i / (w.cols >> 2), c = (i - r * (w.cols >> 2)) << 2;
+            const f32x4 v = *reinterpret_cast<const f32x4*>(w.a + (long long)r * w.lda + c);
+            const u32x2 pk = {pack_bf2(v[0], v[1]), pack_bf2(v[2], v[3])};
+            *reinterpret_cast<u32x2*>(w.gb + (long long)r * w.ldgb + c) = pk;
+        }
+    } else if (w.kind == 2) {
+        const Slabs none = {nullptr, 0, 0, 0};
+        for (int i = t; i < total; i += nt) tanh_bwd_item(i, w.a, w.lda, none, w.o, w.ldo, w.g, w.ldg, w.gb, w.ldgb, w.dr, 0, w.cols);
     }
 }
 __global__ __launch_bounds__(256) void tanh_finalize_kernel(Slabs sl, float* __restrict__ o, int ldo, Drop dr, int rows, int cols) {
@@ -1244,11 +1266,7 @@
     const float sc = scale ? scale[0] : 1.0f;
     if (sc != sc) return;
     for (long long i = (long long)blockIdx.x * 256 + threadIdx.x; i < n; i += (long long)gridDim.x * 256) {
-        const float gi = g[i] * sc;
-        const float mi = b1 * m[i] + (1.f - b1) * gi;
-        const float vi = b2 * v[i] + (1.f - b2) * gi * gi;
-        m[i] = mi; v[i] = vi;
-        p[i] -= lr_t * mi / (sqrtf(vi) + eps);
+        adam_update(p, g, m, v, i, sc, lr_t, b1, b2, eps);
     }
 }
 
@@ -1305,6 +1323,14 @@
 int lxo_k_lstm_bwd(const float* gates, const float* c_prev, const float* c_cur, Slabs s1, Slabs s3, Slabs s4, int off4,
                    float* dcc, float* dz, Drop dr, int carry_rows, int B, int U, hipStream_t st) {
     LAUNCH(lstm_bwd_kernel, grid1((long long)B * U), gates, c_prev, c_cur, s1, s3, s4, off4, dcc, dz, dr, carry_rows, B, U);
+    DONE;
+}
+int lxo_k_chain_arm(void* z0, size_t bytes0, void* z1, size_t bytes1, const ChainArm& w, hipStream_t st) {
+    if (bytes0 % 8 || bytes1 % 8 || ((bytes0 | bytes1) >> 33) != 0 || w.cols % 4 || w.lda % 4 || w.ldgb % 4 || (w.kind == 2 && (w.ldo % 4 || w.ldg % 4))) return -2;
+    long long items = (long long)w.rows * w.cols / 4;
+    if ((long long)(bytes0 / 8) > items) items = (long long)(bytes0 / 8);
+    if ((long long)(bytes1 / 8) > items) items = (long long)(bytes1 / 8);
+    LAUNCH(chain_arm_kernel, grid1(items, 256, 256), (u32x2*)z0, (int)(bytes0 / 8), (u32x2*)z1, (int)(bytes1 / 8), w);
     DONE;
 }
 int lxo_k_tanh_bwd(const float* a, int lda, Slabs carry, const float* o, int ldo, float* g, int ldg, void* gb, int ldgb, Drop dr, int carry_rows, int rows, int cols, hipStream_t st) {
diff --git a/latex_ocr_amd/csrc/encoder_kernels.h b/latex_ocr_amd/csrc/encoder_kernels.h
--- a/latex_ocr_amd/csrc/encoder_kernels.h
+++ b/latex_ocr_amd/csrc/encoder_kernels.h
@@ -3,6 +3,8 @@
 #include "decoder_kernels.h"
 struct PackJob { int kind, K, N, lds, ldd, coff, Kpad, first_block, nblocks; long long src; long long dst; };
 struct PackTable { int n; PackJob job[64]; };
+struct AdamPackJob { int kind, K, N, ldd, coff, Kpad, first_block, nblocks, kind2, ldd2, Cpad2, Cin; long long src, dst, dst2, count; };
+struct AdamPackTable { int n; AdamPackJob job[48]; };
 int lxo_k_conv1_pool_fwd(int dt, const uint8_t* img, const float* w, const float* b, void* out, int B, int H, int W, hipStream_t s);
 int lxo_k_conv1_pool_bwd(int dt, const uint8_t* img, const float* w, const float* b, const void* dout, float* dw, float* db, int B, int H, int W, DetScratch det, hipStream_t s);
 int lxo_k_maxpool_fwd(int dt, const void* in, void* out, int B, int H, int W, int C, int ph, int pw, hipStream_t s);
@@ -14,6 +16,8 @@
 int lxo_k_pack_copy(int dt, const float* src, void* dst, int R, int Ccols, int lds, int ldd, int Cpad, hipStream_t s);
 int lxo_k_pack_conv_dgrad(int dt, const float* w, void* dst, int Cin, int Cout, hipStream_t s);
 int lxo_k_pack_batch(int dt, const PackTable& tab, int total_blocks, const float* prm, void* wpk, hipStream_t s);
+int lxo_k_adam_pack(int dt, const AdamPackTable& tab, int total_blocks, float* prm, const float* g, float* m, float* v, void* wpk,
+                    float lr_t, float b1, float b2, float eps, const float* scale, hipStream_t s);
 int lxo_k_im2col_s2(int dt, const void* in, void* cols, int B, int H, int W, int Ho, int Wo, int C, hipStream_t s);
 int lxo_k_col2im_s2_relu(int dt, const void* dcols, const void* yref, void* dy, float* db, int B, int H, int W, int Ho, int Wo, int C, hipStream_t s);
 int lxo_k_colsum_ct(int dt, const void* a, float* out, long long M, int N, hipStream_t s);
diff --git a/latex_ocr_amd/csrc/encoder_kernels.hip b/latex_ocr_amd/csrc/encoder_kernels.hip
--- a/latex_ocr_amd/csrc/encoder_kernels.hip
+++ b/latex_ocr_amd/csrc/encoder_kernels.hip
@@ -1,5 +1,6 @@
 #include "encoder_kernels.h"
 #include "switches.h"
+#include "adam_update.h"
 
 namespace {
 
@@ -671,6 +672,52 @@
     }
 }
 
+template <typename CT>
+__global__ __launch_bounds__(256) void adam_pack_kernel(AdamPackTable tab, float* __restrict__ prm, const float* __restrict__ g, float* __restrict__ m,
+                                                       float* __restrict__ v, char* __restrict__ wpk, float lr_t, float b1, float b2, float eps,
+                                                       const float* __restrict__ scale) {
+    __shared__ float tile[32][33];
+    const float sc = scale ? scale[0] : 1.0f;
+    const bool upd = sc == sc;
+    int j = 0;
+    while (j + 1 < tab.n && (int)blockIdx.x >= tab.job[j + 1].first_block) ++j;
+    const AdamPackJob q = tab.job[j];
+    const int lb = blockIdx.x - q.first_block;
+    if (q.kind == 3) {
+        if (!upd) return;
+        for (long long i = (long long)lb * 256 + threadIdx.x; i < q.count; i += (long long)q.nblocks * 256) adam_update(prm, g, m, v, q.src + i, sc, lr_t, b1, b2, eps);
+        return;
+    }
+    CT* dst = reinterpret_cast<CT*>(wpk + q.dst);
+    CT* dst2 = reinterpret_cast<CT*>(wpk + q.dst2);
+    const int tiles_k = (q.Kpad + 31) / 32;
+    const int k0 = (lb % tiles_k) * 32, n0 = (lb / tiles_k) * 32;
+    const int tx = threadIdx.x & 31, ty = threadIdx.x >> 5;
+    for (int r = ty; r < 32; r += 8) {
+        const int k = k0 + r, n = n0 + tx;
+        float x = 0.f;
+        if (k < q.K && n < q.N) {
+            const long long i = q.src + (long long)k * q.N + n;
+            x = upd ? adam_update(prm, g, m, v, i, sc, lr_t, b1, b2, eps) : prm[i];
+        }
+        tile[r][tx] = x;
+        if (k < q.K) {
+            if (q.kind2 == 1) {
+                if (n < q.Cpad2) dst2[(long long)k * q.ldd2 + n] = from_f32<CT>(x);
+                if (n0 + 32 >= q.N) for (int c = n + 32; c < q.Cpad2; c += 32) dst2[(long long)k * q.ldd2 + c] = from_f32<CT>(0.f);
+            } else if (q.kind2 == 2 && n < q.N) {
+                const int tap = k / q.Cin, ci = k - tap * q.Cin;
+                dst2[((long long)ci * 9 + (8 - tap)) * q.N + n] = from_f32<CT>(x);
+            }
+        }
+    }
+    __syncthreads();
+    for (int r = ty; r < 32; r += 8) {
+        const int n = n0 + r, k = k0 + tx;
+        if (n < q.N && k < q.Kpad) dst[(long long)n * q.ldd + q.coff + k] = from_f32<CT>(tile[tx][r]);
+    }
+}
+
 
 template <typename CT>
 __global__ __launch_bounds__(256) void im2col_s2_kernel(const CT* __restrict__ in, CT* __restrict__ cols, int B, int H, int W, int Ho, int Wo, int C) {
@@ -875,6 +922,14 @@
     else hipLaunchKernelGGL((pack_batch_kernel<float>), dim3(total_blocks), dim3(256), 0, s, tab, prm, (char*)wpk);
     return (int)hipGetLastError();
 }
+static_assert(sizeof(AdamPackTable) + 64 <= 4096, "adam_pack_kernel's arguments must fit the 4 KB kernel-argument segment");
+int lxo_k_adam_pack(int dt, const AdamPackTable& tab, int total_blocks, float* prm, const float* g, float* m, float* v, void* wpk,
+                    float lr_t, float b1, float b2, float eps, const float* scale, hipStream_t s) {
+    if (tab.n <= 0) return 0;
+    if (dt == LXO_BF16) hipLaunchKernelGGL((adam_pack_kernel<bf16_t>), dim3(total_blocks), dim3(256), 0, s, tab, prm, g, m, v, (char*)wpk, lr_t, b1, b2, eps, scale);
+    else hipLaunchKernelGGL((adam_pack_kernel<float>), dim3(total_blocks), dim3(256), 0, s, tab, prm, g, m, v, (char*)wpk, lr_t, b1, b2, eps, scale);
+    return (int)hipGetLastError();
+}
 
 template <typename CT> static void im2col_s2_t(const void* in, void* cols, int B, int H, int W, int Ho, int Wo, int C, hipStream_t s) {
     hipLaunchKernelGGL((im2col_s2_kernel<CT>), dim3(grid_for((long long)B * Ho * Wo * C, 256 * 4, 8192)), dim3(256), 0, s,
diff --git a/latex_ocr_amd/csrc/impl.h b/latex_ocr_amd/csrc/impl.h
--- a/latex_ocr_amd/csrc/impl.h
+++ b/latex_ocr_amd/csrc/impl.h
@@ -5,6 +5,8 @@
 struct DecSample;
 const char* lxo_ws_name(int id);
 int lxo_impl_pack_weights(const Plan& P, const float* prm, void* wp, hipStream_t st);
+int lxo_impl_adam_pack(const Plan& P, float* prm, const float* grads, float* m, float* v, void* wp,
+                       float lr_t, float b1, float b2, float eps, const float* scale, hipStream_t st);
 int lxo_impl_encoder_fwd(const Plan& P, const float* prm, const void* wp, void* ws, const uint8_t* img, hipStream_t st);
 int lxo_impl_encoder_bwd(const Plan& P, const float* prm, const void* wp, void* ws, const uint8_t* img, float* grads,
                          int last_layer, int first_layer, hipStream_t st, void* const* ready = nullptr);
diff --git a/latex_ocr_amd/csrc/model_decoder.hip b/latex_ocr_amd/csrc/model_decoder.hip
--- a/latex_ocr_amd/csrc/model_decoder.hip
+++ b/latex_ocr_amd/csrc/model_decoder.hip
@@ -112,10 +112,23 @@
     const InitProjs state = init_projs(P, P.ws<float>(ws, W_CS), U, rec0 + O, P.REC, rec0, P.REC);
     float* tmp = P.ws<float>(ws, W_BEAM_TMP);
     const InitProjs out = beam <= 1 ? state : init_projs(P, tmp, U, tmp + (size_t)B * U, U, tmp + (size_t)2 * B * U, O);
-    for (const InitProj& p : out) {
-        if (beam <= 1 && sp.shape == StepPath::Fused) RC(rs_dense(P, mean, C, wt + p.woff, C, p.x, p.ldx, B, p.n, C, prm + P.poff[p.bias], true, false, st));
-        else RC(nt(P, true, true, true, mean, C, wt + p.woff, C, p.x, p.ldx, B, p.n, C, prm + P.poff[p.bias], 2, false, st));
-    }
+    if (beam <= 1 && sp.shape == StepPath::Fused) {
+        RStep a; memset(&a, 0, sizeof(a));
+        a.M = B; a.N = 2 * U + O; a.K = C; a.U = U; a.O = O; a.zx_row = -1; a.epi = RS_TANH_O; a.dr.inv_keep = 1.f;
+        a.A = mean; a.lda = C; a.W = wt; a.ldw = C;
+        a.nseg = 3;
+        int n0 = 0;
+        for (int i = 0; i < 3; ++i) {
+            const InitProj& p = out.p[i];
+            a.seg[i].out = p.x; a.seg[i].ldo = p.ldx; a.seg[i].bias = prm + P.poff[p.bias]; a.seg[i].n0 = n0;
+            n0 += p.n;
+        }
+        const int rc = lxo_launch_rstep(P.s.dtype, 0, a, st);
+        if (rc != -2) return rc < 0 ? rc : -rc;
+        for (const InitProj& p : out) RC(rs_dense(P, mean, C, wt + p.woff, C, p.x, p.ldx, B, p.n, C, prm + P.poff[p.bias], true, false, st));
+        return 0;
+    }
+    for (const InitProj& p : out) RC(nt(P, true, true, true, mean, C, wt + p.woff, C, p.x, p.ldx, B, p.n, C, prm + P.poff[p.bias], 2, false, st));
     for (int i = 0; i < 3 && beam > 1; ++i)
         RC(lxo_k_tile_rows(out.p[i].x, out.p[i].ldx, state.p[i].x, state.p[i].ldx, B * beam, beam, out.p[i].n, st));
     return 0;
@@ -240,7 +253,6 @@
 }
 static int fwd_chain(const Train& w, const int* lengths, bool* ran) {
     const Plan& P = w.P; void* ws = w.ws;
-    RC(mirror_oh(P, ws, 0, P.s.B, w.st));
     XDecFwd x; memset(&x, 0, sizeof(x));
     xdec_common(x, P, w.prm, w.wp, ws);
     x.att_img = P.ws<bf16_t>(ws, W_ATT_IMG);
@@ -249,7 +261,9 @@
     x.dr = P.drop(0, 0);
     x.lengths = lengths;
     LxoTimed tm("xdec_fwd", "chain", (double)P.s.T * P.s.B * P.R * (P.s.E + P.s.C) * P.esz, w.st);
-    const int rc = lxo_launch_xdec_fwd(x, P.s.U, P.s.O, P.s.C, P.s.E, w.st);
+    ChainArm arm; memset(&arm, 0, sizeof(arm));
+    arm.kind = 1; arm.a = w.rec; arm.lda = P.REC; arm.gb = w.recb; arm.ldgb = P.RECB; arm.rows = P.s.B; arm.cols = P.XH;
+    const int rc = lxo_launch_xdec_fwd(x, P.s.U, P.s.O, P.s.C, P.s.E, w.st, &arm);
     if (rc == 0) *ran = true;
     else if (rc != -2) return rc < 0 ? rc : -rc;
     return 0;
@@ -341,14 +355,14 @@
     }
 };
 
-static int bwd_logits(const Train& w, float* grads) {
+static int bwd_logits(const Train& w, float* grads, bool poison) {
     const Plan& P = w.P; hipStream_t st = w.st;
     const int B = P.s.B, TB = P.s.T * B, O = P.s.O, V = P.s.V;
     const void* dlog = P.ws<void>(w.ws, W_DLOGITS);
     RC(nt(P, false, true, false, dlog, P.Vp, P.pk(w.wp, K_YWO), P.Vp, w.dolog, O, TB, O, P.Vp, nullptr, 0, false, st));
     if (w.sp.mirrors) RC(tn(P, false, false, w.step(0).recb_cur, P.RECB, dlog, P.Vp, grads + P.poff[P_YWO], V, TB, O, V, st, P.det_scratch(w.ws)));
     else RC(tn(P, true, false, w.step(0).rec_cur, P.REC, dlog, P.Vp, grads + P.poff[P_YWO], V, TB, O, V, st));
-    if (P.bf) RC(lxo_k_chain_poison(chain_err(P, w.ws, kChainFwd), nullptr, grads + P.ptotal - 1, st));
+    if (P.bf && poison) RC(lxo_k_chain_poison(chain_err(P, w.ws, kChainFwd), nullptr, grads + P.ptotal - 1, st));
     return 0;
 }
 static int bwd_zero_acc(const Train& w) {
@@ -361,7 +375,7 @@
     const Step l = w.step(P.s.T - 1);
     return lxo_k_tanh_bwd(l.dolog, P.s.O, kNoSlabs, l.rec_cur, P.REC, l.g, P.s.O, l.gb, P.GBP, P.drop(P.s.T - 1, 0), 0, P.s.B, P.s.O, w.st);
 }
-static int bwd_chain(const Train& w, bool* ran) {
+static int bwd_chain(const Train& w, bool* ran, float* probe) {
     const Plan& P = w.P; void* ws = w.ws; const void* wp = w.wp;
     XDecBwd x; memset(&x, 0, sizeof(x));
     x.Wow = (const bf16_t*)P.pk(wp, K_OW); x.ldow = P.ldOW;
@@ -378,7 +392,12 @@
     x.T = P.s.T; x.B = P.s.B; x.R = P.R;
     x.dr = P.drop(0, 0);
     LxoTimed tm("xdec_bwd", "chain", (double)P.s.T * P.s.B * P.R * (P.s.E + P.s.C) * P.esz, w.st);
-    const int rc = lxo_launch_xdec_bwd(x, P.s.U, P.s.O, P.s.C, P.s.E, w.st);
+    const Step l = w.step(P.s.T - 1);
+    ChainArm arm; memset(&arm, 0, sizeof(arm));
+    arm.kind = 2; arm.a = l.dolog; arm.lda = P.s.O; arm.o = l.rec_cur; arm.ldo = P.REC; arm.g = l.g; arm.ldg = P.s.O; arm.gb = l.gb; arm.ldgb = P.GBP;
+    arm.dr = P.drop(P.s.T - 1, 0); arm.rows = P.s.B; arm.cols = P.s.O;
+    if (probe) { arm.poison_err = chain_err(P, ws, kChainFwd); arm.probe = probe; }
+    const int rc = lxo_launch_xdec_bwd(x, P.s.U, P.s.O, P.s.C, P.s.E, w.st, &arm);
     if (rc == 0) *ran = true;
     else if (rc != -2) return rc < 0 ? rc : -rc;
     else { RC(bwd_zero_acc(w)); HIPRC(hipMemsetAsync(x.sync, 0, kXDecSyncBytes, w.st)); }
@@ -555,7 +574,8 @@
 int lxo_impl_decoder_train_bwd(const Plan& P, const float* prm, const void* wp, void* ws, const int* formula, float* grads,
                                int parts, hipStream_t st, bool defer_join, void* ready) {
     const Train w = train_of(P, prm, wp, ws, st);
-    if (parts & 1) RC(bwd_logits(w, grads));
+    const bool fold = (parts & 3) == 3 && w.sp.try_chain;
+    if (parts & 1) RC(bwd_logits(w, grads, !fold));
     if (!(parts & 2)) return 0;
     bool chain = false;
     if (!w.sp.try_chain) {
@@ -564,9 +584,9 @@
     }
     if (w.sp.loop == StepPath::SplitK) RC(bwd_splitk_loop(w));
     else {
-        RC(bwd_last_g(w));
-        if (w.sp.try_chain) RC(bwd_chain(w, &chain));
-        if (!chain) RC(bwd_fused_loop(w));
+        if (w.sp.try_chain) RC(bwd_chain(w, &chain, fold ? grads + P.ptotal - 1 : nullptr));
+        if (fold && !chain) RC(lxo_k_chain_poison(chain_err(P, ws, kChainFwd), nullptr, grads + P.ptotal - 1, st));
+        if (!chain) { RC(bwd_last_g(w)); RC(bwd_fused_loop(w)); }
     }
     const BwdStreams s = {st, (w.sp.mirrors && !lxo_timer_on()) ? lxo_impl_encoder_side_stream() : nullptr};
     const DetScratch det_s = s.side ? P.det_scratch_side(ws) : P.det_scratch(ws);
diff --git a/latex_ocr_amd/csrc/model_encoder.hip b/latex_ocr_amd/csrc/model_encoder.hip
--- a/latex_ocr_amd/csrc/model_encoder.hip
+++ b/latex_ocr_amd/csrc/model_encoder.hip
@@ -5,9 +5,9 @@
 #include "api_util.h"
 #include "timing.h"
 
-int lxo_impl_pack_weights(const Plan& P, const float* prm, void* wp, hipStream_t st) {
-    const int dt = P.s.dtype, C = P.s.C, E = P.s.E, U = P.s.U, O = P.s.O, D = P.s.D, V = P.s.V;
-    PackTable tab; memset(&tab, 0, sizeof(tab));
+static int pack_table(const Plan& P, PackTable& tab) {
+    const int C = P.s.C, E = P.s.E, U = P.s.U, O = P.s.O, D = P.s.D, V = P.s.V;
+    memset(&tab, 0, sizeof(tab));
     int blocks = 0;
     auto add = [&](int kind, long long src, size_t dst, int K, int N, int lds, int ldd, int coff, int Kpad) {
         PackJob& j = tab.job[tab.n++];
@@ -62,7 +62,61 @@
             cp(k + (long long)C * 4 * Ur, P.koff[K_ROWH + d], Ur, 4 * Ur, 4 * Ur, 4 * Ur);
         }
     }
-    return lxo_k_pack_batch(dt, tab, blocks, prm, wp, st);
+    return blocks;
+}
+int lxo_impl_pack_weights(const Plan& P, const float* prm, void* wp, hipStream_t st) {
+    PackTable tab;
+    const int blocks = pack_table(P, tab);
+    return lxo_k_pack_batch(P.s.dtype, tab, blocks, prm, wp, st);
+}
+int lxo_impl_adam_pack(const Plan& P, float* prm, const float* grads, float* m, float* v, void* wp,
+                       float lr_t, float b1, float b2, float eps, const float* scale, hipStream_t st) {
+    PackTable src; pack_table(P, src);
+    AdamPackTable tab; memset(&tab, 0, sizeof(tab));
+    const int cap = (int)(sizeof(tab.job) / sizeof(tab.job[0]));
+    long long rows_done[64] = {0};
+    int order[64], nt = 0;
+    for (int i = 0; i < src.n; ++i) if (src.job[i].kind == 0) {
+        if (src.job[i].lds != src.job[i].N) return -1;
+        int k = nt++;
+        for (; k > 0 && src.job[order[k - 1]].src > src.job[i].src; --k) order[k] = order[k - 1];
+        order[k] = i;
+    }
+    int blocks = 0;
+    auto plain = [&](long long from, long long to) {
+        if (to <= from) return 0;
+        if (tab.n >= cap) return -1;
+        AdamPackJob& j = tab.job[tab.n++];
+        j.kind = 3; j.src = from; j.count = to - from;
+        j.nblocks = (int)cdivl(j.count, 256 * 4); j.first_block = blocks; blocks += j.nblocks;
+        return 0;
+    };
+    long long at = 0;
+    for (int o = 0; o < nt; ++o) {
+        const PackJob& t = src.job[order[o]];
+        const long long end = t.src + (long long)t.K * t.N;
+        if (t.src < at) return -1;
+        RC(plain(at, t.src));
+        if (tab.n >= cap) return -1;
+        AdamPackJob& j = tab.job[tab.n++];
+        j.kind = 0; j.K = t.K; j.N = t.N; j.ldd = t.ldd; j.coff = t.coff; j.Kpad = t.Kpad; j.src = t.src; j.dst = t.dst;
+        j.nblocks = t.nblocks; j.first_block = blocks; blocks += j.nblocks;
+        for (int i = 0; i < src.n; ++i) {
+            const PackJob& c = src.job[i];
+            if (c.kind == 1 && c.N == t.N && c.lds == c.N && t.src >= c.src && end <= c.src + (long long)c.K * c.N && (t.src - c.src) % c.N == 0) {
+                j.kind2 = 1; j.ldd2 = c.ldd; j.Cpad2 = c.Kpad;
+                j.dst2 = c.dst + (t.src - c.src) / c.N * c.ldd * (long long)P.esz;
+                rows_done[i] += t.K;
+            } else if (c.kind == 2 && c.src == t.src && c.N == t.N && t.K == 9 * c.K) {
+                j.kind2 = 2; j.Cin = c.K; j.dst2 = c.dst;
+                rows_done[i] += c.K;
+            }
+        }
+        at = end;
+    }
+    RC(plain(at, P.ptotal));
+    for (int i = 0; i < src.n; ++i) if (src.job[i].kind != 0 && rows_done[i] != src.job[i].K) return -1;
+    return lxo_k_adam_pack(P.s.dtype, tab, blocks, prm, grads, m, v, wp, lr_t, b1, b2, eps, scale, st);
 }
 
 static const char* conv_name(int Cin, int Cout, bool valid) {
diff --git a/latex_ocr_amd/csrc/rstep.h b/latex_ocr_amd/csrc/rstep.h
--- a/latex_ocr_amd/csrc/rstep.h
+++ b/latex_ocr_amd/csrc/rstep.h
@@ -23,6 +23,7 @@
     const int* zx_idx; int zx_vocab, zx_row;
     const float* dhm; int lddhm; const float* carry_h; const float* gates_in; const float* c_cur; float* dcc; int carry_rows;
     const float* bias; int accumulate;
+    int nseg; struct Seg { float* out; const float* bias; int ldo, n0; } seg[3];
     const float* dolog; const float* o_prev; int ldoprev; int first;
     Drop dr;
     unsigned long long* dbg;
diff --git a/latex_ocr_amd/csrc/rstep.hip b/latex_ocr_amd/csrc/rstep.hip
--- a/latex_ocr_amd/csrc/rstep.hip
+++ b/latex_ocr_amd/csrc/rstep.hip
@@ -196,6 +196,19 @@
 #pragma unroll
         for (int e = 0; e < 4; ++e) v[e] = red[0][row][part * 4 + e] + red[1][row][part * 4 + e] + red[2][row][part * 4 + e] + red[3][row][part * 4 + e];
         if constexpr (EPI == RS_PLAIN || EPI == RS_TANH_O) {
+            if (p.nseg > 0) {
+                int sg = 0;
+                while (sg + 1 < p.nseg && n >= p.seg[sg + 1].n0) ++sg;
+                const int nl = n - p.seg[sg].n0;
+                if (p.seg[sg].bias) { float b4[4]; ld4(p.seg[sg].bias + nl, b4); for (int e = 0; e < 4; ++e) v[e] += b4[e]; }
+                if constexpr (EPI == RS_TANH_O) {
+#pragma unroll
+                    for (int e = 0; e < 4; ++e) v[e] = tanh_e<BF>(v[e]);
+                }
+                st4(p.seg[sg].out + (long long)m * p.seg[sg].ldo + nl, v);
+                STAMP(6);
+                return;
+            }
             if (p.bias) { float b4[4]; ld4(p.bias + n, b4); for (int e = 0; e < 4; ++e) v[e] += b4[e]; }
             if (p.accumulate) { float o4[4]; ld4(p.out + (long long)m * p.ldo + n, o4); for (int e = 0; e < 4; ++e) v[e] += o4[e]; }
         }
@@ -308,6 +321,10 @@
     if (p.M <= 0 || p.N <= 0) return 0;
     if (p.K % 128 != 0 || p.lda % 8 != 0 || p.ldw % 8 != 0 || p.N % 4 != 0) return -2;
     if (p.epi == RS_LSTM_FWD && (p.U % 4 != 0 || p.N != 4 * p.U)) return -2;
+    if (p.nseg) {
+        if (p.nseg < 0 || p.nseg > 3 || (p.epi != RS_PLAIN && p.epi != RS_TANH_O) || p.dr.thr != 0u || p.outb || p.accumulate || p.seg[0].n0 != 0) return -2;
+        for (int i = 0; i < p.nseg; ++i) if (p.seg[i].n0 % 16 || p.seg[i].ldo % 4 || (i && p.seg[i].n0 <= p.seg[i - 1].n0) || p.seg[i].n0 >= p.N) return -2;
+    }
     switch (p.epi) {
     case RS_PLAIN: return launch_epi<RS_PLAIN>(dt, a_bf16 != 0, p, st);
     case RS_TANH_O: return launch_epi<RS_TANH_O>(dt, a_bf16 != 0, p, st);
diff --git a/latex_ocr_amd/csrc/xdec.h b/latex_ocr_amd/csrc/xdec.h
--- a/latex_ocr_amd/csrc/xdec.h
+++ b/latex_ocr_amd/csrc/xdec.h
@@ -26,7 +26,7 @@
     const int* lengths;
 };
 
-int lxo_launch_xdec_fwd(const XDecFwd& p, int U, int O, int C, int E, hipStream_t st);
+int lxo_launch_xdec_fwd(const XDecFwd& p, int U, int O, int C, int E, hipStream_t st, const ChainArm* arm = nullptr);
 
 struct XDecDec {
     const bf16_t* Wrt; int ldrt; const bf16_t* Wah; int ldah; const bf16_t* Wow; int ldow;
@@ -78,7 +78,7 @@
     Drop dr;
     unsigned long long* dbg;
 };
-int lxo_launch_xdec_bwd(const XDecBwd& p, int U, int O, int C, int E, hipStream_t st);
+int lxo_launch_xdec_bwd(const XDecBwd& p, int U, int O, int C, int E, hipStream_t st, const ChainArm* arm = nullptr);
 constexpr size_t kXDecSyncBytes = 4096, kXDecLLBytes = 384u << 10, kXDecBlockBytes = kXDecSyncBytes + kXDecLLBytes;
 constexpr size_t kXDecBlockWords = kXDecBlockBytes / 4;
 constexpr size_t kXDecErrWord = 8 * 64;
diff --git a/latex_ocr_amd/csrc/xdec.hip b/latex_ocr_amd/csrc/xdec.hip
--- a/latex_ocr_amd/csrc/xdec.hip
+++ b/latex_ocr_amd/csrc/xdec.hip
@@ -4,8 +4,8 @@
 #include "switches.h"
 
 #ifdef LXO_HIPSIM
-int lxo_launch_xdec_fwd(const XDecFwd&, int, int, int, int, hipStream_t) { return -2; }
-int lxo_launch_xdec_bwd(const XDecBwd&, int, int, int, int, hipStream_t) { return -2; }
+int lxo_launch_xdec_fwd(const XDecFwd&, int, int, int, int, hipStream_t, const ChainArm*) { return -2; }
+int lxo_launch_xdec_bwd(const XDecBwd&, int, int, int, int, hipStream_t, const ChainArm*) { return -2; }
 int lxo_launch_xdec_dec(const XDecDec&, int, int, int, int, hipStream_t) { return -2; }
 extern "C" int lxo_xdec_debug(unsigned long long*) { return 0; }
 extern "C" int lxo_xdec_debug_bwd(unsigned long long*) { return 0; }
@@ -1447,14 +1447,22 @@
 
 static thread_local unsigned long long* g_xdbg = nullptr;
 extern "C" int lxo_xdec_debug(unsigned long long* buf) { g_xdbg = buf; return 0; }
-int lxo_launch_xdec_fwd(const XDecFwd& p0, int U, int O, int C, int E, hipStream_t st) {
+static int xdec_arm(void* sync, void* part, size_t part_bytes, const ChainArm* arm, hipStream_t st) {
+    if (arm) {
+        const int rc = lxo_k_chain_arm(sync, kXDecBlockBytes, part_bytes ? part : nullptr, part_bytes, *arm, st);
+        return rc == -2 ? -1 : rc;
+    }
+    HIPRC(hipMemsetAsync(sync, 0, kXDecBlockBytes, st));
+    if (part_bytes) HIPRC(hipMemsetAsync(part, 0, part_bytes, st));
+    return 0;
+}
+int lxo_launch_xdec_fwd(const XDecFwd& p0, int U, int O, int C, int E, hipStream_t st, const ChainArm* arm) {
     XDecFwd p = p0;
     p.dbg = g_xdbg;
     const int nb = xdec_gate(SW_XDEC, U, O, C, E, p.B, p.R, SCMAX);
     if (!nb || p.T < 1) return -2;
     if ((long long)p.B * p.RECB * 2 >= (1LL << 31) || p.ldrt % 8 || p.ldah % 8 || p.ldow % 8 || p.RECB % 8) return -2;
-    HIPRC(hipMemsetAsync(p.sync, 0, kXDecBlockBytes, st));
-    if (kLL & 4) HIPRC(hipMemsetAsync(p.part, 0, (size_t)p.B * (32 / nb) * PLW * 8, st));
+    RC(xdec_arm(p.sync, p.part, (kLL & 4) ? (size_t)p.B * (32 / nb) * PLW * 8 : 0, arm, st));
 
     switch (nb) {
     case 1: return launch_nb<1>(p, st);
@@ -1480,14 +1488,13 @@
 }
 static thread_local unsigned long long* g_xdbg_b = nullptr;
 extern "C" int lxo_xdec_debug_bwd(unsigned long long* buf) { g_xdbg_b = buf; return 0; }
-int lxo_launch_xdec_bwd(const XDecBwd& p0, int U, int O, int C, int E, hipStream_t st) {
+int lxo_launch_xdec_bwd(const XDecBwd& p0, int U, int O, int C, int E, hipStream_t st, const ChainArm* arm) {
     XDecBwd p = p0;
     p.dbg = g_xdbg_b;
     const int nb = xdec_gate(SW_XDEC_BWD, U, O, C, E, p.B, p.R, SCMAX);
     if (!nb || p.T < 1) return -2;
     if (p.ldow % 8 || p.ldah % 8 || p.ldk % 8 || p.GBP % 8 || p.DZBP % 8 || p.REC % 4 || (long long)p.B * p.DZBP * 2 >= (1LL << 31)) return -2;
-    HIPRC(hipMemsetAsync(p.sync, 0, kXDecBlockBytes, st));
-    if (kLLB & 4) HIPRC(hipMemsetAsync(p.part, 0, (size_t)p.B * (32 / nb) * XE * 4, st));
+    RC(xdec_arm(p.sync, p.part, (kLLB & 4) ? (size_t)p.B * (32 / nb) * XE * 4 : 0, arm, st));
     switch (nb) {
     case 1: return launch_bwd_nb<1>(p, st);
     case 2: return launch_bwd_nb<2>(p, st);
diff --git a/latex_ocr_amd/engine.py b/latex_ocr_amd/engine.py
--- a/latex_ocr_amd/engine.py
+++ b/latex_ocr_amd/engine.py
@@ -525,10 +525,10 @@
         if guard:
             self._chain_health_post(scale is not None, dp)
             scale = self.scale
-        self._ck(self.lib.lxo_adam_step(self.n_params, _p(self.params), _p(self.grads), _p(self.adam_m), _p(self.adam_v),
-                                        ctypes.c_float(lr_t), ctypes.c_float(beta1), ctypes.c_float(beta2), ctypes.c_float(eps),
-                                        _p(scale), st), "adam")
-        self.pack()
+        shape = self.shape if self.shape is not None else self._shape(1, 32, 32, 1)
+        self._ck(self.lib.lxo_adam_pack_step(ctypes.byref(shape), _p(self.params), _p(self.grads), _p(self.adam_m), _p(self.adam_v), _p(self.wpack),
+                                             ctypes.c_float(lr_t), ctypes.c_float(beta1), ctypes.c_float(beta2), ctypes.c_float(eps),
+                                             _p(scale), st), "adam_pack")
 
     def train_step(self, img, formula, lengths, lr, clip=-1.0, dist=None, sync_loss=True, dropout=1.0, dropout_seed=None,
                    weights=None, row_weights=None, norm=None, label_smoothing=0.0):
```

Result: no change. 9132 img/s (median of 2 runs) (-0.0%).
